# wen-yuan-zhang/MaterialRefGS

Hardware: AMD Instinct MI355X
Metric: full-render fwd+bwd views/sec at 800x800/300k surfels; grad max-rel-err vs ref (higher is better)
Workload: dtype f32; 1 GPU; C3 shell scene through render_surfel: P=300000, 800x800, S=8 + deferred BRDF shading, fwd+bwd; P=300000, H=800, W=800, S=8, sh_degree=3, num_rendered=1153468, cameras_cycled=2, parallelism=single GPU, glue_epilogue=True

## Files before the change

include/mrgs.h:

```cpp
#ifndef MRGS_H_INCLUDED
#define MRGS_H_INCLUDED

#include <stddef.h>
#include <stdint.h>

#ifdef __cplusplus
extern "C" {
#endif

#define MRGS_MAX_FEATURES 24
#define MRGS_TILE 16
#define MRGS_NUM_OTHERS 7

enum {
    MRGS_OK = 0,
    MRGS_E_BAD_ARG = 1,
    MRGS_E_TOO_MANY_FEATURES = 2,
    MRGS_E_NEED_COLORS = 3,
    MRGS_E_HIP = 4,
    MRGS_E_WORKSPACE = 5,
    MRGS_E_UNSUPPORTED = 6,
    MRGS_E_INTERNAL = 7
};

typedef struct MrgsRasterConfig {
    uint32_t struct_size;
    int32_t P;
    int32_t S;
    int32_t D;
    int32_t M;
    int32_t H, W;
    float tanfovx, tanfovy;
    float scale_modifier;
    int32_t prefiltered;
    int32_t debug;
} MrgsRasterConfig;

typedef struct MrgsRasterInputs {
    uint64_t struct_size;
    const float* bg;
    const float* means3D;
    const float* shs;
    const float* colors_precomp;
    const float* features;
    const float* opacities;
    const float* scales;
    const float* rotations;
    const float* transMat_precomp;
    const float* viewmatrix;
    const float* projmatrix;
    const float* campos;
    uint32_t* work_hint;
    const float* shs_rest;
    void* bwd_grad_ws;
    uint32_t hint_flags;
    uint32_t features_live;
} MrgsRasterInputs;
#define MRGS_HINT_REUSE_ORDER 1u
#define MRGS_HINT_VISIBLE_BYTES 2u

size_t mrgs_geom_bytes(int32_t P, int32_t H, int32_t W);
size_t mrgs_img_bytes(int32_t H, int32_t W);
size_t mrgs_binning_bytes(int64_t num_rendered);
size_t mrgs_work_hint_bytes(int32_t H, int32_t W);

int mrgs_rasterize_forward_geom(const MrgsRasterConfig* cfg, const MrgsRasterInputs* in, void* geom_ws, size_t geom_bytes,
                                int32_t* radii, int64_t* num_rendered_host, void* stream);

int mrgs_rasterize_forward_render(const MrgsRasterConfig* cfg, const MrgsRasterInputs* in, void* geom_ws, void* binning_ws,
                                  size_t binning_bytes, void* img_ws, int64_t num_rendered, float* out_color,
                                  float* out_feature, float* out_others, void* stream);

int mrgs_rasterize_forward(const MrgsRasterConfig* cfg, const MrgsRasterInputs* in, void* geom_ws, size_t geom_bytes,
                           void* binning_ws, size_t binning_bytes, int64_t capacity_pairs, void* img_ws, int32_t* radii,
                           float* out_color, float* out_feature, float* out_others, int64_t* num_rendered_host, void* stream);

typedef struct MrgsRasterTicket {
    int32_t device, slot;
    uint64_t seq;
    int64_t capacity_pairs;
} MrgsRasterTicket;
int mrgs_rasterize_forward_begin(const MrgsRasterConfig* cfg, const MrgsRasterInputs* in, void* geom_ws, size_t geom_bytes,
                                 void* binning_ws, size_t binning_bytes, int64_t capacity_pairs, void* img_ws, int32_t* radii,
                                 float* out_color, float* out_feature, float* out_others, MrgsRasterTicket* ticket, void* stream);
int mrgs_rasterize_forward_finish(const MrgsRasterTicket* ticket, int64_t* num_rendered_host);

typedef struct MrgsRasterGrads {
    uint64_t struct_size;
    float* dL_dmeans2D;
    float* dL_dcolors;
    float* dL_dfeatures;
    float* dL_dopacity;
    float* dL_dmeans3D;
    float* dL_dtransMat;
    float* dL_dsh;
    float* dL_dscales;
    float* dL_drotations;
    float* dL_dsh_rest;
    const struct MrgsSurfelParams* glue_params;
    const struct MrgsSurfelGrads* glue_grads;
} MrgsRasterGrads;

size_t mrgs_grad_bytes(int32_t P, int32_t S);
int mrgs_rasterize_backward(const MrgsRasterConfig* cfg, const MrgsRasterInputs* in, const int32_t* radii, const void* geom_ws,
                            const void* binning_ws, const void* img_ws, int64_t num_rendered, const float* dL_dout_color,
                            const float* dL_dout_feature, const float* dL_dout_others, void* grad_ws,
                            const MrgsRasterGrads* grads, void* stream);

int mrgs_rasterize_backward_blend(const MrgsRasterConfig* cfg, const MrgsRasterInputs* in, const int32_t* radii, const void* geom_ws,
                                  const void* binning_ws, const void* img_ws, int64_t num_rendered, const float* dL_dout_color,
                                  const float* dL_dout_feature, const float* dL_dout_others, void* grad_ws, float* dL_dRGB_masked,
                                  void* stream);
int mrgs_rasterize_backward_finish(const MrgsRasterConfig* cfg, const MrgsRasterInputs* in, const int32_t* radii, const void* geom_ws,
                                   const void* grad_ws, const MrgsRasterGrads* grads, void* stream);

int mrgs_mark_visible(int32_t P, const float* means3D, const float* viewmatrix, const float* projmatrix, uint8_t* present,
                      void* stream);

#define MRGS_MAX_MIPS 8
typedef struct MrgsEnvMips {
    int32_t n_levels;
    int32_t res[MRGS_MAX_MIPS];
    const float* tex[MRGS_MAX_MIPS];
    float* grad[MRGS_MAX_MIPS];
    int32_t grad_copies[MRGS_MAX_MIPS];
    float min_roughness, max_roughness;
} MrgsEnvMips;

int mrgs_envmap_lookup_forward(const MrgsEnvMips* mips, int64_t N, const float* dirs, const float* roughness, float* out, void* stream);
int mrgs_envmap_lookup_backward(const MrgsEnvMips* mips, int64_t N, const float* dirs, const float* roughness, const float* g_out,
                                float* g_dirs , float* g_roughness , void* stream);

typedef struct MrgsStridedMap { const float* ptr; int64_t stride_h, stride_w, stride_c; } MrgsStridedMap;
typedef struct MrgsShadeFrame {
    int32_t H, W;
    float Kinv[9];
    const float* R;
    const float* T;
    MrgsStridedMap albedo;
    MrgsStridedMap normal;
    MrgsStridedMap alpha;
// ... 335 lines not shown
```

materialrefgs_amd/_lib.py:

```python
import ctypes
import os
import subprocess

import torch

_CSRC = os.path.join(os.path.dirname(os.path.abspath(__file__)), "csrc")
LIB_PATH = os.environ.get("MRGS_LIB") or os.path.join(_CSRC, "libmrgs.so")

c_int32, c_int64, c_float, c_void_p, c_size_t = ctypes.c_int32, ctypes.c_int64, ctypes.c_float, ctypes.c_void_p, ctypes.c_size_t


class _Sized(ctypes.Structure):

    def __init__(self, *args, **kw):
        super().__init__(ctypes.sizeof(type(self)), *args, **kw)


class MrgsRasterConfig(_Sized):
    _fields_ = [("struct_size", ctypes.c_uint32), ("P", c_int32), ("S", c_int32), ("D", c_int32), ("M", c_int32), ("H", c_int32), ("W", c_int32),
                ("tanfovx", c_float), ("tanfovy", c_float), ("scale_modifier", c_float), ("prefiltered", c_int32),
                ("debug", c_int32)]


class MrgsRasterInputs(_Sized):
    _fields_ = [("struct_size", ctypes.c_uint64)] + [(n, c_void_p) for n in ("bg", "means3D", "shs", "colors_precomp", "features", "opacities", "scales",
                                        "rotations", "transMat_precomp", "viewmatrix", "projmatrix", "campos", "work_hint", "shs_rest",
                                        "bwd_grad_ws")] + [("hint_flags", ctypes.c_uint32), ("features_live", ctypes.c_uint32)]


MRGS_HINT_REUSE_ORDER = 1
MRGS_HINT_VISIBLE_BYTES = 2


class MrgsRasterGrads(_Sized):
    _fields_ = [("struct_size", ctypes.c_uint64)] + [(n, c_void_p) for n in ("dL_dmeans2D", "dL_dcolors", "dL_dfeatures", "dL_dopacity", "dL_dmeans3D",
                                        "dL_dtransMat", "dL_dsh", "dL_dscales", "dL_drotations", "dL_dsh_rest",
                                        "glue_params", "glue_grads")]


MRGS_MAX_MIPS = 8


class MrgsEnvMips(ctypes.Structure):
    _fields_ = [("n_levels", c_int32), ("res", c_int32 * MRGS_MAX_MIPS), ("tex", c_void_p * MRGS_MAX_MIPS),
                ("grad", c_void_p * MRGS_MAX_MIPS), ("grad_copies", c_int32 * MRGS_MAX_MIPS), ("min_roughness", c_float), ("max_roughness", c_float)]


class MrgsStridedMap(ctypes.Structure):
    _fields_ = [("ptr", c_void_p), ("stride_h", c_int64), ("stride_w", c_int64), ("stride_c", c_int64)]


class MrgsShadeFrame(ctypes.Structure):
    _fields_ = [("H", c_int32), ("W", c_int32), ("Kinv", c_float * 9), ("R", c_void_p), ("T", c_void_p),
                ("albedo", MrgsStridedMap), ("normal", MrgsStridedMap), ("alpha", MrgsStridedMap), ("refl", MrgsStridedMap),
                ("roughness", MrgsStridedMap), ("lut", c_void_p), ("lut_res", c_int32)]


class MrgsRasterTicket(ctypes.Structure):
    _fields_ = [("device", c_int32), ("slot", c_int32), ("seq", ctypes.c_uint64), ("capacity_pairs", c_int64)]


class MrgsSpmvDesc(ctypes.Structure):
    _fields_ = [("nrows", c_int32), ("lanes_per_row", c_int32), ("col_bytes", c_int32), ("val_bytes", c_int32), ("row_ptr", c_void_p),
                ("col", c_void_p), ("val", c_void_p), ("row_scale", c_void_p), ("x", c_void_p), ("y", c_void_p),
                ("image_rows", c_void_p), ("pre_scale", c_void_p), ("tile_ptr", c_void_p), ("panel_ptr", c_void_p), ("panel_src", c_void_p),
                ("res", c_int32), ("n_tiles", c_int32), ("max_panel", c_int32), ("reserved", c_int32)]


class MrgsSurfelParams(ctypes.Structure):
    _fields_ = [("P", c_int32)] + [(n, c_void_p) for n in ("xyz", "scaling_raw", "rotation_raw", "opacity_raw", "refl_raw", "rough_raw",
                                                             "ori_color_raw", "indirect_dc", "indirect_rest", "campos", "viewmatrix")]


class MrgsSurfelGrads(ctypes.Structure):
    _fields_ = [(n, c_void_p) for n in ("d_xyz", "d_scaling", "d_rotation", "d_opacity", "d_refl", "d_rough", "d_ori_color",
                                        "d_indirect_dc", "d_indirect_rest")]


class MrgsMapsFrame(ctypes.Structure):
    _fields_ = [("H", c_int32), ("W", c_int32), ("view_rot", c_float * 9), ("ray_matrix", c_float * 9), ("ray_origin", c_float * 3),
                ("depth_ratio", c_float), ("pgsr_fx", c_float), ("pgsr_fy", c_float), ("rend_distance", c_void_p), ("g_rend_distance", c_void_p)]


class MrgsLossConfig(ctypes.Structure):
    _fields_ = [("H", c_int32), ("W", c_int32), ("C", c_int32), ("lambda_dssim", c_float), ("lambda_normal", c_float),
                ("lambda_dist", c_float)]


MRGS_WARP_GEO, MRGS_WARP_MATERIAL, MRGS_WARP_METALLIC, MRGS_WARP_ROUGHNESS = 1, 2, 4, 8


class MrgsWarpConfig(_Sized):
    _fields_ = [("struct_size", ctypes.c_uint32), ("H", c_int32), ("W", c_int32), ("sample_num", c_int32), ("patch_half", c_int32),
                ("n_given", c_int32), ("flags", ctypes.c_uint32), ("seed_lo", ctypes.c_uint32), ("seed_hi", ctypes.c_uint32)] + \
               [(n, c_float) for n in ("fx_v", "fy_v", "cx_v", "cy_v", "fx_n", "fy_n", "cx_n", "cy_n", "pixel_noise_th", "geo_weight",
                                       "base_weight", "metallic_weight", "roughness_weight")]


class MrgsWarpMaps(ctypes.Structure):
    _fields_ = [(n, c_void_p) for n in ("depth_v", "depth_n", "normal_v", "distance_v", "base_v", "metal_v", "rough_v", "base_n", "metal_n",
                                        "rough_n", "fg_v", "keep_v", "cam_v", "cam_n")]


class MrgsAdamTensor(ctypes.Structure):
    _fields_ = [("param", c_void_p), ("grad", c_void_p), ("exp_avg", c_void_p), ("exp_avg_sq", c_void_p), ("numel", c_int64),
                ("lr", c_float), ("step", c_int32)]


class MrgsCompactTensor(ctypes.Structure):
    _fields_ = [("src", c_void_p), ("dst", c_void_p), ("row_floats", c_int32)]


MRGS_DENSIFY_COPY, MRGS_DENSIFY_MOMENT, MRGS_DENSIFY_XYZ, MRGS_DENSIFY_SCALING = 0, 1, 2, 3

# ... 250 lines not shown
```

materialrefgs_amd/csrc/mrgs_api.hip:

```cpp
#include <stdio.h>
#include <string.h>
#include <atomic>
#include <mutex>
#include <vector>
#include "mrgs_internal.h"

static thread_local char g_hip_err[256] = "";
static int g_profiling = 0;

int mrgs_hip_status(hipError_t e, const char* file, int line)
{
    if (e == hipSuccess) return MRGS_OK;
    snprintf(g_hip_err, sizeof(g_hip_err), "%s at %s:%d", hipGetErrorString(e), file, line);
    return MRGS_E_HIP;
}

#define STAGE_CHECK(cfg, stream)                                      \
    do {                                                              \
        if (int rc_ = MRGS_LAUNCH_STATUS()) return rc_;               \
        if ((cfg)->debug) MRGS_HIP_TRY(hipStreamSynchronize(stream)); \
    } while (0)

namespace {
enum { ST_PRE = 0, ST_SORT, ST_DUP, ST_FWD, ST_BWD, ST_PREB, ST_COUNT };
// ... 20 lines not shown
                std::lock_guard<std::mutex> lk(g_prof_mutex);
                if (!g_free.empty()) { p = g_free.back(); g_free.pop_back(); reuse = true; }
            }
            if (!reuse) { (void)hipEventCreate(&p.a); (void)hipEventCreate(&p.b); }
            p.stage = stage;
            (void)hipEventRecord(p.a, s);
        }
    }
    void stop()
    {
        if (on) {
            (void)hipEventRecord(p.b, s);
            std::lock_guard<std::mutex> lk(g_prof_mutex);
            g_pairs.push_back(p);
            on = false;
        }
    }
};

struct Carver {
    char* p;
    size_t used = 0;
    explicit Carver(void* base) : p((char*)base) {}
    template <typename T>
    T* take(size_t n)
    {
        used = mrgs_align_up(used, 256);
        T* r = p ? (T*)(p + used) : nullptr;
        used += sizeof(T) * n;
        return r;
    }
};
}

MrgsGeomWs mrgs_carve_geom(void* base, int P, int H, int W)
{
    Carver c(base);
    MrgsGeomWs g;
    const size_t n = (size_t)(P > 0 ? P : 1);
    g.rec = c.take<float4>(n * MRGS_REC_F4);
    g.cull = c.take<float4>(n * MRGS_CULL_F4);
    g.depth_key[0] = c.take<uint32_t>(n);
    g.depth_key[1] = c.take<uint32_t>(n);
    g.order[0] = c.take<uint32_t>(n);
    g.order[1] = c.take<uint32_t>(n);
    g.rect = c.take<uint2>(n);
    g.tiles_touched = c.take<uint32_t>(n);
    g.offsets = c.take<uint32_t>(n);
    g.clamped = c.take<uint8_t>(n);
    g.counters = c.take<uint32_t>(16 + MRGS_CENSUS_WORDS);
    const size_t clear_from = c.used - (16 + MRGS_CENSUS_WORDS) * sizeof(uint32_t);
    g.sort_ws = c.take<uint32_t>(mrgs_sort_ws_words((int64_t)n));
    g.scan_ws = c.take<uint32_t>(mrgs_scan_ws_words((int)n));
    g.clear_bytes = c.used - clear_from;
    const int T = ((W + MRGS_BLOCK_X - 1) / MRGS_BLOCK_X) * ((H + MRGS_BLOCK_Y - 1) / MRGS_BLOCK_Y);
    g.tile_mat = g.tile_cnt = g.tile_loc = g.chunk_tot = g.chunk_base = g.big_list = nullptr;
    if (mrgs_bin_supported(T)) {
        const size_t Tpad = (size_t)mrgs_bin_tpad(T);
        g.tile_mat = c.take<uint32_t>((size_t)mrgs_bin_groups(P) * Tpad);
        g.tile_cnt = c.take<uint32_t>(Tpad);
        g.tile_loc = c.take<uint32_t>(Tpad);
        g.chunk_tot = c.take<uint32_t>(Tpad / 64);
        g.chunk_base = c.take<uint32_t>(Tpad / 64);
        g.big_list = c.take<uint32_t>(Tpad);
    }
    g.total = mrgs_align_up(c.used, 256);
    return g;
}

MrgsImgWs mrgs_carve_img(void* base, int H, int W)
{
    Carver c(base);
    MrgsImgWs w;
    const size_t hw = (size_t)H * W;
    const size_t tiles = (size_t)((W + MRGS_BLOCK_X - 1) / MRGS_BLOCK_X) * ((H + MRGS_BLOCK_Y - 1) / MRGS_BLOCK_Y);
    const size_t nt = tiles > 0 ? tiles : 1;
    w.ranges = c.take<uint2>(nt);
    const size_t ranges_from = c.used - sizeof(uint2) * nt;
    c.used = mrgs_align_up(c.used, 256);
    w.item_est = c.take<uint32_t>(4 * nt);
    w.ranges_est_bytes = c.used - ranges_from;
    w.item_work = c.take<uint32_t>(4 * nt);
    const size_t per_list = (nt + 7) / 8 * 4;
    w.order_items = c.take<uint32_t>(8 * per_list);
    w.order_work = c.take<uint32_t>(8 * per_list);
    w.fwd_assign = c.take<uint32_t>(8 * (per_list + MRGS_MAX_SIMD_QUEUES));
    w.bwd_assign = c.take<uint32_t>(8 * (per_list + MRGS_MAX_SIMD_QUEUES));
    w.blend_state = c.take<uint32_t>(MRGS_BLEND_STATE_WORDS);
    w.q_bwd = w.blend_state + MRGS_QS_BWD;
    w.final_T = c.take<float>(3 * hw);
    w.n_contrib = c.take<uint32_t>(2 * hw);
    w.redo_list = c.take<uint32_t>(2 + hw);
    w.total = mrgs_align_up(c.used, 256);
    return w;
}

MrgsBinWs mrgs_carve_bin(void* base, int64_t R)
{
    Carver c(base);
    MrgsBinWs b;
    const size_t n = (size_t)(R > 0 ? R : 1);
    const size_t n64 = mrgs_align_up(n, 64);
    b.tile_key[0] = c.take<uint32_t>(2 * n64);
    b.tile_key[1] = b.tile_key[0] ? b.tile_key[0] + n64 : nullptr;
    b.plist[0] = c.take<uint32_t>(n);
    b.plist[1] = c.take<uint32_t>(n);
    b.sort_ws = c.take<uint32_t>(16 + mrgs_sort_ws_words((int64_t)n));
    b.sort_ws_bytes = sizeof(uint32_t) * (16 + mrgs_sort_ws_words((int64_t)n));
    b.qmask = c.take<uint8_t>(n);
    b.cflag = c.take<uint8_t>(4 * n);
    b.total = mrgs_align_up(c.used, 256);
    return b;
}

static int tile_bits(int ntiles)
{
    int bits = 1;
    while ((1 << bits) < ntiles) bits++;
    return bits;
}

static int sorted_buf(int bits) { return ((bits + 7) / 8) & 1; }
static int plist_buf(const MrgsGeomWs& g, int ntiles) { return g.tile_mat != nullptr ? 0 : sorted_buf(tile_bits(ntiles)); }

static int check_cfg(const MrgsRasterConfig* cfg, const MrgsRasterInputs* in)
{
    if (!cfg || !in) return MRGS_E_BAD_ARG;
    if (cfg->struct_size != sizeof(MrgsRasterConfig) || in->struct_size != sizeof(MrgsRasterInputs)) return MRGS_E_BAD_ARG;
    if (cfg->P < 0 || cfg->H <= 0 || cfg->W <= 0 || cfg->S < 0 || cfg->M < 0) return MRGS_E_BAD_ARG;
    if (cfg->S > MRGS_MAX_FEATURES) return MRGS_E_TOO_MANY_FEATURES;
    if (cfg->P > 0) {
        if (!in->means3D || !in->opacities || !in->viewmatrix || !in->projmatrix || !in->campos || !in->bg) return MRGS_E_BAD_ARG;
        if ((in->shs == nullptr) == (in->colors_precomp == nullptr)) return MRGS_E_NEED_COLORS;
        if (in->shs && cfg->M <= 0) return MRGS_E_BAD_ARG;
        if (in->shs_rest && (!in->shs || cfg->M < 2 || cfg->M > 16)) return MRGS_E_BAD_ARG;
        const bool have_sr = in->scales && in->rotations;
        if (have_sr == (in->transMat_precomp != nullptr)) return MRGS_E_BAD_ARG;
        if (cfg->S > 0 && !in->features) return MRGS_E_BAD_ARG;
        if ((cfg->W + 15) / 16 > 65535 || (cfg->H + 15) / 16 > 65535) return MRGS_E_UNSUPPORTED;
        if (cfg->P >= (1 << 28)) return MRGS_E_UNSUPPORTED;
        if ((uint64_t)cfg->P * MRGS_GRAD_STRIDE(cfg->S) * sizeof(float) >= (1ull << 32)) return MRGS_E_UNSUPPORTED;
    }
    return MRGS_OK;
}

MrgsHintLayout mrgs_hint_layout(int H, int W)
{
    const size_t tiles = (size_t)((W + MRGS_BLOCK_X - 1) / MRGS_BLOCK_X) * ((H + MRGS_BLOCK_Y - 1) / MRGS_BLOCK_Y);
    const size_t nt = tiles > 0 ? tiles : 1, per_list = (nt + 7) / 8 * 4;
    MrgsHintLayout l;
    l.work = 0;
    l.blend_state = mrgs_align_up(4 * nt, 64);
    l.fwd_assign = mrgs_align_up(l.blend_state + MRGS_BLEND_STATE_WORDS, 64);
    l.total_words = mrgs_align_up(l.fwd_assign + 8 * (per_list + MRGS_MAX_SIMD_QUEUES), 64);
    return l;
}
static void img_use_hint(MrgsImgWs& img, const MrgsRasterInputs* in, int H, int W)
{
    if (in->work_hint == nullptr) return;
    const MrgsHintLayout l = mrgs_hint_layout(H, W);
    img.blend_state = in->work_hint + l.blend_state;
    img.fwd_assign = in->work_hint + l.fwd_assign;
}

extern "C" {

size_t mrgs_geom_bytes(int32_t P, int32_t H, int32_t W) { return mrgs_carve_geom(nullptr, P, H, W).total; }
size_t mrgs_img_bytes(int32_t H, int32_t W) { return mrgs_carve_img(nullptr, H, W).total; }
size_t mrgs_binning_bytes(int64_t R) { return mrgs_carve_bin(nullptr, R).total; }
size_t mrgs_work_hint_bytes(int32_t H, int32_t W)
{
    if (H <= 0 || W <= 0) return 0;
    return mrgs_hint_layout(H, W).total_words * sizeof(uint32_t);
}
size_t mrgs_grad_bytes(int32_t P, int32_t S) { return mrgs_align_up((size_t)(P > 0 ? P : 1) * MRGS_GRAD_STRIDE(S) * sizeof(float), 256); }

static int enqueue_geom(const MrgsRasterConfig* cfg, const MrgsRasterInputs* in, MrgsGeomWs g, int32_t* radii, hipStream_t stream,
                        uint32_t* host_slot = nullptr, hipEvent_t slot_event = nullptr)
{
    StageTimer t0(stream, ST_PRE);
    mrgs_launch_preprocess_fwd(*cfg, *in, g, radii, stream);
    t0.stop();
    STAGE_CHECK(cfg, stream);

    StageTimer t1(stream, ST_SORT);
    if (g.tile_mat != nullptr) {
        mrgs_launch_tile_count_scan(*cfg, g, host_slot, stream);
        if (slot_event != nullptr) MRGS_HIP_TRY(hipEventRecord(slot_event, stream));
    } else {
        const int cur = mrgs_radix_sort_pairs(g.depth_key, g.order, g.sort_ws, g.counters + 1, cfg->P, nullptr, 0, 32, stream);
        STAGE_CHECK(cfg, stream);
        mrgs_scan_tiles(g.tiles_touched, g.order[cur], g.offsets, g.scan_ws, g.counters, g.counters + 1, cfg->P, stream);
    }
    t1.stop();
    STAGE_CHECK(cfg, stream);
    return MRGS_OK;
}

static int enqueue_render(const MrgsRasterConfig* cfg, const MrgsRasterInputs* in, MrgsGeomWs g, MrgsBinWs b,
                          const MrgsImgWs& img, int64_t R, const uint32_t* R_dev, float* out_color, float* out_feature,
                          float* out_others, hipStream_t stream, uint32_t* host_slot = nullptr, hipEvent_t slot_event = nullptr)
{
    const int tiles_x = (cfg->W + MRGS_BLOCK_X - 1) / MRGS_BLOCK_X, tiles_y = (cfg->H + MRGS_BLOCK_Y - 1) / MRGS_BLOCK_Y;
    const int ntiles = tiles_x * tiles_y;
    const int dcur = sorted_buf(32);

    StageTimer t0(stream, ST_DUP);
    int cur = 0;
    bool reuse_order = false;
    if (g.tile_mat != nullptr) {
        reuse_order = R > 0 && in->work_hint != nullptr && (in->hint_flags & MRGS_HINT_REUSE_ORDER) != 0u;
        if (R > 0) mrgs_launch_tile_emit_sort(*cfg, g, b, img, R, reuse_order, in->bwd_grad_ws, in->bwd_grad_ws ? mrgs_grad_bytes(cfg->P, cfg->S) : 0, stream);
        else MRGS_HIP_TRY(hipMemsetAsync(img.ranges, 0, img.ranges_est_bytes, stream));
        STAGE_CHECK(cfg, stream);
    } else {
        if (R > 0) {
            mrgs_launch_duplicate(*cfg, g, g.order[dcur], b.tile_key[0], b.plist[0], R, R_dev, b, img, host_slot, stream);
            if (slot_event != nullptr) MRGS_HIP_TRY(hipEventRecord(slot_event, stream));
        } else {
            MRGS_HIP_TRY(hipMemsetAsync(img.ranges, 0, img.ranges_est_bytes, stream));
        }
        STAGE_CHECK(cfg, stream);
        const int bits = tile_bits(ntiles);
        cur = mrgs_radix_sort_pairs(b.tile_key, b.plist, b.sort_ws + 16, b.sort_ws, R, R_dev, 0, bits, stream);
        STAGE_CHECK(cfg, stream);
        mrgs_launch_tile_ranges(b.tile_key[cur], b.plist[cur], R, R_dev, g.cull, b.qmask, img, tiles_x, ntiles, stream);
    }
    if (!reuse_order)
        mrgs_launch_blend_order(img, g.counters + 16, ntiles, 0, in->bwd_grad_ws, in->bwd_grad_ws ? mrgs_grad_bytes(cfg->P, cfg->S) : 0, in->work_hint,
                                stream);
    t0.stop();
    STAGE_CHECK(cfg, stream);

    StageTimer t1(stream, ST_FWD);
    mrgs_launch_render_fwd(*cfg, *in, g, b.plist[cur], b.qmask, b.cflag, img, out_color, out_feature, out_others, stream);
    t1.stop();
    STAGE_CHECK(cfg, stream);
    return MRGS_OK;
}

static int zero_outputs(const MrgsRasterConfig* cfg, float* out_color, float* out_feature, float* out_others, hipStream_t stream)
{
    const size_t hw = (size_t)cfg->H * cfg->W;
    MRGS_HIP_TRY(hipMemsetAsync(out_color, 0, sizeof(float) * 3 * hw, stream));
    if (cfg->S > 0) MRGS_HIP_TRY(hipMemsetAsync(out_feature, 0, sizeof(float) * cfg->S * hw, stream));
    MRGS_HIP_TRY(hipMemsetAsync(out_others, 0, sizeof(float) * MRGS_NUM_OTHERS * hw, stream));
    return MRGS_OK;
}

static int check_counters(const uint32_t host[2], int64_t* num_rendered_host)
{
    if (host[1] != 0) return MRGS_E_INTERNAL;
    if (host[0] >= (1u << 30)) return MRGS_E_UNSUPPORTED;
    *num_rendered_host = (int64_t)host[0];
    return MRGS_OK;
}

int mrgs_rasterize_forward_geom(const MrgsRasterConfig* cfg, const MrgsRasterInputs* in, void* geom_ws, size_t geom_bytes,
                                int32_t* radii, int64_t* num_rendered_host, void* stream_)
{
    hipStream_t stream = (hipStream_t)stream_;
    int rc = check_cfg(cfg, in);
    if (rc) return rc;
    if (!num_rendered_host) return MRGS_E_BAD_ARG;
    *num_rendered_host = 0;
    if (cfg->P == 0) return MRGS_OK;
    if (!geom_ws || !radii) return MRGS_E_BAD_ARG;
    MrgsGeomWs g = mrgs_carve_geom(geom_ws, cfg->P, cfg->H, cfg->W);
    if (geom_bytes < g.total) return MRGS_E_WORKSPACE;
    rc = enqueue_geom(cfg, in, g, radii, stream);
    if (rc) return rc;
    uint32_t host[2] = {0, 0};
    MRGS_HIP_TRY(hipMemcpyAsync(host, g.counters, 2 * sizeof(uint32_t), hipMemcpyDeviceToHost, stream));
    MRGS_HIP_TRY(hipStreamSynchronize(stream));
    return check_counters(host, num_rendered_host);
}

int mrgs_rasterize_forward_render(const MrgsRasterConfig* cfg, const MrgsRasterInputs* in, void* geom_ws, void* binning_ws,
                                  size_t binning_bytes, void* img_ws, int64_t R, float* out_color, float* out_feature,
                                  float* out_others, void* stream_)
{
    hipStream_t stream = (hipStream_t)stream_;
    int rc = check_cfg(cfg, in);
    if (rc) return rc;
    if (!out_color || !out_others || (cfg->S > 0 && !out_feature) || !img_ws) return MRGS_E_BAD_ARG;
    if (cfg->P == 0) return zero_outputs(cfg, out_color, out_feature, out_others, stream);
    if (!geom_ws || !binning_ws) return MRGS_E_BAD_ARG;
    MrgsImgWs img = mrgs_carve_img(img_ws, cfg->H, cfg->W);
    img_use_hint(img, in, cfg->H, cfg->W);
    MrgsGeomWs g = mrgs_carve_geom(geom_ws, cfg->P, cfg->H, cfg->W);
    MrgsBinWs b = mrgs_carve_bin(binning_ws, R);
    if (binning_bytes < b.total) return MRGS_E_WORKSPACE;
    return enqueue_render(cfg, in, g, b, img, R, nullptr, out_color, out_feature, out_others, stream);
}

namespace {
#define MRGS_MAX_DEVICES 64
#define MRGS_TICKET_RING 16
struct ReadbackRing {
    uint32_t* host = nullptr;
    uint32_t* dev = nullptr;
    hipEvent_t ev[MRGS_TICKET_RING] = {};
    uint64_t seq[MRGS_TICKET_RING] = {};
    uint64_t next = 1;
};
static thread_local ReadbackRing g_rings[MRGS_MAX_DEVICES];
}

int mrgs_rasterize_forward_begin(const MrgsRasterConfig* cfg, const MrgsRasterInputs* in, void* geom_ws, size_t geom_bytes,
                                 void* binning_ws, size_t binning_bytes, int64_t capacity_pairs, void* img_ws, int32_t* radii,
                                 float* out_color, float* out_feature, float* out_others, MrgsRasterTicket* ticket, void* stream_)
{
    hipStream_t stream = (hipStream_t)stream_;
    int rc = check_cfg(cfg, in);
    if (rc) return rc;
    if (!ticket || !out_color || !out_others || (cfg->S > 0 && !out_feature) || !img_ws) return MRGS_E_BAD_ARG;
    ticket->device = -1; ticket->slot = -1; ticket->seq = 0; ticket->capacity_pairs = capacity_pairs;
    if (cfg->P == 0) return zero_outputs(cfg, out_color, out_feature, out_others, stream);
// ... 7 lines not shown
    int device = 0;
    MRGS_HIP_TRY(hipGetDevice(&device));
    if (device < 0 || device >= MRGS_MAX_DEVICES) return MRGS_E_UNSUPPORTED;
    ReadbackRing& ring = g_rings[device];
    if (!ring.host) {
        MRGS_HIP_TRY(hipHostMalloc((void**)&ring.host, MRGS_TICKET_RING * 64, hipHostMallocMapped | hipHostMallocPortable));
        MRGS_HIP_TRY(hipHostGetDevicePointer((void**)&ring.dev, ring.host, 0));
        for (int i = 0; i < MRGS_TICKET_RING; ++i) MRGS_HIP_TRY(hipEventCreateWithFlags(&ring.ev[i], hipEventDisableTiming));
    }
    const int slot = (int)(ring.next % MRGS_TICKET_RING);
    ring.seq[slot] = ring.next;
    ticket->device = device; ticket->slot = slot; ticket->seq = ring.next++;
    uint32_t* slot_dev = ring.dev + 16 * slot;
    rc = enqueue_geom(cfg, in, g, radii, stream, slot_dev, ring.ev[slot]);
    if (rc) return rc;
    return enqueue_render(cfg, in, g, b, img, capacity_pairs, g.counters, out_color, out_feature, out_others, stream, slot_dev, ring.ev[slot]);
}

int mrgs_rasterize_forward_finish(const MrgsRasterTicket* ticket, int64_t* num_rendered_host)
{
    if (!ticket || !num_rendered_host) return MRGS_E_BAD_ARG;
    *num_rendered_host = 0;
    if (ticket->device < 0) return MRGS_OK;
    if (ticket->device >= MRGS_MAX_DEVICES || ticket->slot < 0 || ticket->slot >= MRGS_TICKET_RING) return MRGS_E_BAD_ARG;
    ReadbackRing& ring = g_rings[ticket->device];
    if (!ring.host || ring.seq[ticket->slot] != ticket->seq) return MRGS_E_BAD_ARG;
    MRGS_HIP_TRY(hipEventSynchronize(ring.ev[ticket->slot]));
    int rc = check_counters(ring.host + 16 * ticket->slot, num_rendered_host);
    if (rc) return rc;
    return *num_rendered_host > ticket->capacity_pairs ? MRGS_E_WORKSPACE : MRGS_OK;
}

int mrgs_rasterize_forward(const MrgsRasterConfig* cfg, const MrgsRasterInputs* in, void* geom_ws, size_t geom_bytes,
                           void* binning_ws, size_t binning_bytes, int64_t capacity_pairs, void* img_ws, int32_t* radii,
                           float* out_color, float* out_feature, float* out_others, int64_t* num_rendered_host, void* stream_)
{
    if (!num_rendered_host) return MRGS_E_BAD_ARG;
    *num_rendered_host = 0;
    MrgsRasterTicket ticket;
    int rc = mrgs_rasterize_forward_begin(cfg, in, geom_ws, geom_bytes, binning_ws, binning_bytes, capacity_pairs, img_ws, radii, out_color,
                                          out_feature, out_others, &ticket, stream_);
    if (rc) return rc;
    return mrgs_rasterize_forward_finish(&ticket, num_rendered_host);
}

static int grads_check(const MrgsRasterConfig* cfg, const MrgsRasterInputs* in, const MrgsRasterGrads* g)
{
    if (!g->dL_dmeans2D || (cfg->M > 0 && !g->dL_dsh) || ((in->shs_rest != nullptr) != (g->dL_dsh_rest != nullptr))) return MRGS_E_BAD_ARG;
    if ((g->glue_params != nullptr) != (g->glue_grads != nullptr)) return MRGS_E_BAD_ARG;
    if (g->glue_params == nullptr)
        return (g->dL_dcolors && g->dL_dopacity && g->dL_dmeans3D && g->dL_dtransMat && g->dL_dscales && g->dL_drotations && (cfg->S == 0 || g->dL_dfeatures))
                   ? MRGS_OK : MRGS_E_BAD_ARG;
    const MrgsSurfelParams* p = g->glue_params;
    const MrgsSurfelGrads* o = g->glue_grads;
    const bool rows8 = cfg->S == 8 && p->viewmatrix == nullptr, rows12 = cfg->S == 12 && in->features_live == 9u && p->viewmatrix != nullptr;
    if (!(rows8 || rows12) || !in->scales || !in->rotations || in->transMat_precomp) return MRGS_E_UNSUPPORTED;
    if (cfg->P != p->P || !p->scaling_raw || !p->rotation_raw || !p->opacity_raw || !p->refl_raw || !p->rough_raw || !p->ori_color_raw) return MRGS_E_BAD_ARG;
    return (o->d_xyz && o->d_scaling && o->d_rotation && o->d_opacity && o->d_refl && o->d_rough && o->d_ori_color && o->d_indirect_dc && o->d_indirect_rest)
               ? MRGS_OK : MRGS_E_BAD_ARG;
}

int mrgs_rasterize_backward_blend(const MrgsRasterConfig* cfg, const MrgsRasterInputs* in, const int32_t* radii, const void* geom_ws,
                                  const void* binning_ws, const void* img_ws, int64_t R, const float* dL_dout_color,
                                  const float* dL_dout_feature, const float* dL_dout_others, void* grad_ws, float* dL_dRGB_masked,
                                  void* stream_)
{
    hipStream_t stream = (hipStream_t)stream_;
    int rc = check_cfg(cfg, in);
    if (rc) return rc;
    if (cfg->P == 0) return MRGS_OK;
    if (!radii || !geom_ws || !binning_ws || !img_ws || !grad_ws || !dL_dout_color || !dL_dout_others) return MRGS_E_BAD_ARG;
    if (cfg->S > 0 && !dL_dout_feature) return MRGS_E_BAD_ARG;
    const int tiles_x = (cfg->W + MRGS_BLOCK_X - 1) / MRGS_BLOCK_X, tiles_y = (cfg->H + MRGS_BLOCK_Y - 1) / MRGS_BLOCK_Y;
    MrgsGeomWs g = mrgs_carve_geom(const_cast<void*>(geom_ws), cfg->P, cfg->H, cfg->W);
    MrgsBinWs b = mrgs_carve_bin(const_cast<void*>(binning_ws), R);
    MrgsImgWs img = mrgs_carve_img(const_cast<void*>(img_ws), cfg->H, cfg->W);
    img_use_hint(img, in, cfg->H, cfg->W);
    const int cur = plist_buf(g, tiles_x * tiles_y);
    float* grad_rec = (float*)grad_ws;

    StageTimer t0(stream, ST_BWD);
    const bool prepared = in->bwd_grad_ws != nullptr && in->bwd_grad_ws == grad_ws;
    if (R > 0) {
        if (!prepared) mrgs_launch_blend_order(img, g.counters + 16, tiles_x * tiles_y, 1, grad_rec, mrgs_grad_bytes(cfg->P, cfg->S), nullptr, stream);
        mrgs_launch_render_bwd(*cfg, *in, g, b.plist[cur], b.cflag, img, dL_dout_color, dL_dout_feature, dL_dout_others, grad_rec, prepared, stream);
    } else if (!prepared) {
        MRGS_HIP_TRY(hipMemsetAsync(grad_rec, 0, mrgs_grad_bytes(cfg->P, cfg->S), stream));
    }
    t0.stop();
    if (dL_dRGB_masked) mrgs_launch_color_grad_extract(*cfg, g, radii, grad_rec, in->shs != nullptr, dL_dRGB_masked, stream);
    STAGE_CHECK(cfg, stream);
    return MRGS_OK;
}

int mrgs_rasterize_backward_finish(const MrgsRasterConfig* cfg, const MrgsRasterInputs* in, const int32_t* radii, const void* geom_ws,
                                   const void* grad_ws, const MrgsRasterGrads* grads, void* stream_)
{
    hipStream_t stream = (hipStream_t)stream_;
    int rc = check_cfg(cfg, in);
    if (rc) return rc;
    if (!grads || grads->struct_size != sizeof(MrgsRasterGrads)) return MRGS_E_BAD_ARG;
    if (cfg->P == 0) return MRGS_OK;
    rc = grads_check(cfg, in, grads);
    if (rc) return rc;
    if (!radii || !geom_ws || !grad_ws) return MRGS_E_BAD_ARG;
    MrgsGeomWs g = mrgs_carve_geom(const_cast<void*>(geom_ws), cfg->P, cfg->H, cfg->W);
    StageTimer t1(stream, ST_PREB);
    mrgs_launch_preprocess_bwd(*cfg, *in, g, radii, (const float*)grad_ws, *grads, stream);
    t1.stop();
    STAGE_CHECK(cfg, stream);
    return MRGS_OK;
}

int mrgs_rasterize_backward(const MrgsRasterConfig* cfg, const MrgsRasterInputs* in, const int32_t* radii, const void* geom_ws,
                            const void* binning_ws, const void* img_ws, int64_t R, const float* dL_dout_color,
                            const float* dL_dout_feature, const float* dL_dout_others, void* grad_ws, const MrgsRasterGrads* grads,
                            void* stream_)
{
    int rc = check_cfg(cfg, in);
    if (rc) return rc;
    if (!grads || grads->struct_size != sizeof(MrgsRasterGrads)) return MRGS_E_BAD_ARG;
    if (cfg->P == 0) return MRGS_OK;
    rc = grads_check(cfg, in, grads);
    if (rc) return rc;
    if (!radii || !geom_ws || !binning_ws || !img_ws || !grad_ws || !dL_dout_color || !dL_dout_others) return MRGS_E_BAD_ARG;
    if (cfg->S > 0 && !dL_dout_feature) return MRGS_E_BAD_ARG;
    rc = mrgs_rasterize_backward_blend(cfg, in, radii, geom_ws, binning_ws, img_ws, R, dL_dout_color, dL_dout_feature, dL_dout_others, grad_ws,
                                       nullptr, stream_);
    if (rc) return rc;
    return mrgs_rasterize_backward_finish(cfg, in, radii, geom_ws, grad_ws, grads, stream_);
}

int mrgs_mark_visible(int32_t P, const float* means3D, const float* viewmatrix, const float* projmatrix, uint8_t* present,
                      void* stream_)
{
    (void)projmatrix;
    if (P < 0) return MRGS_E_BAD_ARG;
    if (P == 0) return MRGS_OK;
    if (!means3D || !viewmatrix || !present) return MRGS_E_BAD_ARG;
    mrgs_launch_mark_visible(P, means3D, viewmatrix, present, (hipStream_t)stream_);
    return MRGS_LAUNCH_STATUS();
}

#define MRGS_MESH_ENTRY(call) do { bool launched = false; if (int rc = (call)) return rc; return launched ? MRGS_LAUNCH_STATUS() : MRGS_OK; } while (0)
int mrgs_tsdf_fuse(const MrgsTsdfConfig* cfg, const MrgsTsdfView* views_dev, float* field, float* weight_debug, void* stream_)
{
    MRGS_MESH_ENTRY(mrgs_tsdf_fuse_launch(cfg, views_dev, field, weight_debug, stream_, &launched));
}
int mrgs_mesh_count(const MrgsMeshConfig* cfg, const float* field, void* ws, size_t ws_bytes, int64_t* totals_dev, void* stream_)
{
    MRGS_MESH_ENTRY(mrgs_mesh_count_launch(cfg, field, ws, ws_bytes, totals_dev, stream_, &launched));
}
int mrgs_mesh_emit(const MrgsMeshConfig* cfg, const float* field, void* ws, size_t ws_bytes, const int64_t* totals_host, float* vertices,
                   int32_t* triangles, void* stream_)
{
    MRGS_MESH_ENTRY(mrgs_mesh_emit_launch(cfg, field, ws, ws_bytes, totals_host, vertices, triangles, stream_, &launched));
}
int mrgs_mesh_clusters(int64_t V, int64_t T, const int32_t* triangles, int32_t* labels, int32_t* counts, void* stream_)
{
    MRGS_MESH_ENTRY(mrgs_mesh_clusters_launch(V, T, triangles, labels, counts, stream_, &launched));
}
int mrgs_mesh_select(int64_t V, int64_t T, const int32_t* triangles, const int32_t* labels, const int32_t* counts, int32_t threshold,
                     uint8_t* keep_vertex, uint8_t* keep_triangle, void* stream_)
{
    MRGS_MESH_ENTRY(mrgs_mesh_select_launch(V, T, triangles, labels, counts, threshold, keep_vertex, keep_triangle, stream_, &launched));
}
int mrgs_mesh_reindex(int64_t V_old, int64_t V_new, const int32_t* new_to_old, int32_t* remap_ws, int64_t T, int32_t* triangles, void* stream_)
{
// ... 116 lines not shown
```

materialrefgs_amd/csrc/mrgs_blend_math.h:

```cpp
#pragma once
#include "mrgs_internal.h"
#include "mrgs_wave.h"

#define MRGS_ALPHA_MIN (1.0f / 255.0f)
#define MRGS_T_MIN 0.0001f
#define MRGS_CHUNK 64

template <auto KERNEL> static int mrgs_waves_per_simd()
{
    static const int n = [] {
        int per_cu = 0;
        if (hipOccupancyMaxActiveBlocksPerMultiprocessor(&per_cu, KERNEL, 64, 0) != hipSuccess || per_cu < 4) return 1;
        return per_cu / 4;
    }();
    return n;
}


__device__ __forceinline__ uint32_t mrgs_pull_item(uint32_t* __restrict__ qstate, const uint32_t* __restrict__ cu_state,
                                                   const uint32_t* __restrict__ assign_ws, int ntiles, int xcd, int wv, int lane,
                                                   int slots, unsigned long long* dbg = nullptr)
{
    const uint32_t pw = qstate[MRGS_QS_PASSES + xcd];
    const int passes = (int)(pw & 0xFFFFu), NQ = (int)(pw >> 16);
    if (wv >= passes * NQ) return 0xFFFFFFFFu;
    const int per_list = ((ntiles + 7) >> 3) * 4;
    const uint32_t hw_id = __builtin_amdgcn_s_getreg((4 << 0) | (0 << 6) | (31 << 11));
    const uint32_t xcc = __builtin_amdgcn_s_getreg((20 << 0) | (0 << 6) | (3 << 11)) & 7u;
    const uint32_t dense = cu_state[MRGS_CS_DENSE + xcc * 256 + mrgs_cu_key(hw_id)];
    const int q0 = (int)((dense * 4u + ((hw_id >> 4) & 3u)) % (uint32_t)NQ);
    const uint32_t* assign = assign_ws + (size_t)xcd * (per_list + MRGS_MAX_SIMD_QUEUES);
    uint32_t* tickets = qstate + MRGS_QS_TICKET + xcd * MRGS_MAX_SIMD_QUEUES;
    uint32_t item = 0xFFFFFFFFu;
    int t = 0;
    if (lane == 0) {
        t = (int)atomicAdd(&tickets[q0], 1u);
        if (t < passes) item = assign[t * NQ + q0];
    }
    item = __builtin_amdgcn_readfirstlane(item);
    t = __builtin_amdgcn_readfirstlane(t);
    if (dbg) { dbg[0] = dbg[2] = wall_clock64(); dbg[1] = 0; }
    if (item != 0xFFFFFFFFu) return item;
    if (t < passes && passes <= slots) __builtin_amdgcn_s_sleep(127);
    for (int base = 1; item == 0xFFFFFFFFu && base < NQ;) {
        const int d = base + lane;
        const int q = d < NQ ? (q0 + d < NQ ? q0 + d : q0 + d - NQ) : q0;
        const uint32_t tk = __hip_atomic_load(&tickets[q], __ATOMIC_RELAXED, __HIP_MEMORY_SCOPE_AGENT);
        const uint32_t last = assign[(passes - 1) * NQ + q];
        const bool has = d < NQ && (int)tk < passes - (last == 0xFFFFFFFFu ? 1 : 0);
        const unsigned long long m = __ballot(has);
        if (dbg) dbg[1] += 1 + (m == 0ull ? 256 : 0);
        if (m == 0ull) { base += 64; continue; }
        const int qs = __builtin_amdgcn_readlane(q, (int)__builtin_ctzll(m));
        if (lane == 0) {
            const int ts = (int)atomicAdd(&tickets[qs], 1u);
            if (ts < passes) item = assign[ts * NQ + qs];
        }
        item = __builtin_amdgcn_readfirstlane(item);
    }
    if (dbg) dbg[2] = wall_clock64();
    return item;
}

__device__ __forceinline__ float mrgs_rcp(float x) { return __builtin_amdgcn_rcpf(x); }

__device__ __forceinline__ float mrgs_exp(float x)
{
    const float L2E_HI = 1.44269502162933349609375f, L2E_LO = 1.925963033500011e-8f, LN2 = 0.693147182464599609375f;
    const float t = x * L2E_HI;
    float e = fmaf(x, L2E_HI, -t);
    e = fmaf(x, L2E_LO, e);
    const float r = __builtin_amdgcn_exp2f(t);
    return fmaf(r, e * LN2, r);
}

struct SurfelGeom { float4 g0, g1, g2; };

struct Hit {
    float kx, ky, kz, lx, ly, lz;
    float inv_pz, sx, sy;
    float rho3d, rho2d, dx, dy;
    float depth, G, alpha;
    bool use3d;
};

#define MRGS_ALPHA_LO (MRGS_ALPHA_MIN * (1.0f - 4e-6f))
#define MRGS_ALPHA_HI (MRGS_ALPHA_MIN * (1.0f + 4e-6f))
#define MRGS_NEAR_LO (MRGS_NEAR_N - 1e-4f)
#define MRGS_NEAR_HI (MRGS_NEAR_N + 1e-4f)
#define MRGS_RHO_EPS 2e-5f
#define MRGS_T_STEP_ERR 4.1e-7f
#define MRGS_T1_SLACK 1.25f
#define MRGS_T1_ABS 1e-11f
#ifndef MRGS_T2_EPS
#define MRGS_T2_EPS (0.5f * 4e-6f)
#endif

struct HitTest { float ppz, d3, power; };
__device__ __forceinline__ HitTest mrgs_intersect_fast(const SurfelGeom& s, float px, float py, Hit& h)
{
    const float Twx = s.g1.z, Twy = s.g1.w, Twz = s.g2.x;
    h.kx = fmaf(px, Twx, -s.g0.x); h.ky = fmaf(px, Twy, -s.g0.y); h.kz = fmaf(px, Twz, -s.g0.z);
    h.lx = fmaf(py, Twx, -s.g0.w); h.ly = fmaf(py, Twy, -s.g1.x); h.lz = fmaf(py, Twz, -s.g1.y);
    const float ppx = fmaf(h.ky, h.lz, -(h.kz * h.ly));
    const float ppy = fmaf(h.kz, h.lx, -(h.kx * h.lz));
    const float ppz = fmaf(h.kx, h.ly, -(h.ky * h.lx));
    h.inv_pz = mrgs_rcp(ppz);
    h.sx = ppx * h.inv_pz;
    h.sy = ppy * h.inv_pz;
    h.rho3d = fmaf(h.sx, h.sx, h.sy * h.sy);
    h.dx = s.g2.y - px;
    h.dy = s.g2.z - py;
    h.rho2d = MRGS_FILTER_INV_SQUARE * fmaf(h.dx, h.dx, h.dy * h.dy);
    const float rho = fminf(h.rho3d, h.rho2d);
    const float d3 = fmaf(h.sx, Twx, fmaf(h.sy, Twy, Twz));
    h.use3d = h.rho3d <= h.rho2d;
    h.depth = h.use3d ? d3 : Twz;
    const float power = -0.5f * rho;
    h.G = mrgs_exp(power);
    h.alpha = fminf(0.99f, s.g2.w * h.G);
    return HitTest{ppz, d3, power};
}

__device__ __forceinline__ bool mrgs_intersect(const SurfelGeom& s, float px, float py, Hit& h)
{
    const HitTest t = mrgs_intersect_fast(s, px, py, h);
    return (t.ppz != 0.0f) & (!(t.d3 < MRGS_NEAR_LO) | !(s.g2.x < MRGS_NEAR_LO)) & !(t.power > 0.0f) & !(h.alpha < MRGS_ALPHA_LO);
}

__device__ __forceinline__ bool mrgs_hit_decide(const Hit& h, bool may_hit, bool& ambiguous)
{
    const bool hit = may_hit & !(h.depth < MRGS_NEAR_LO);
    ambiguous = (hit & ((h.alpha < MRGS_ALPHA_HI) | (h.depth < MRGS_NEAR_HI))) | (may_hit & (fabsf(h.rho3d - h.rho2d) < MRGS_RHO_EPS));
    return hit;
}

#define MRGS_BALLOT(cond) __builtin_amdgcn_ballot_w64(cond)
#define MRGS_LANES(mask) __builtin_amdgcn_inverse_ballot_w64(mask)
__device__ __forceinline__ uint64_t mrgs_intersect_mask(const SurfelGeom& s, float px, float py, Hit& h)
{
    const HitTest t = mrgs_intersect_fast(s, px, py, h);
    const uint64_t tw_ok = s.g2.x < MRGS_NEAR_LO ? 0ull : ~0ull;
    return MRGS_BALLOT(t.ppz != 0.0f) & (~MRGS_BALLOT(t.d3 < MRGS_NEAR_LO) | tw_ok) & ~MRGS_BALLOT(t.power > 0.0f) & ~MRGS_BALLOT(h.alpha < MRGS_ALPHA_LO);
}
__device__ __forceinline__ uint64_t mrgs_hit_decide_mask(const Hit& h, uint64_t may_hit, uint64_t& ambiguous)
{
    const uint64_t hit = may_hit & ~MRGS_BALLOT(h.depth < MRGS_NEAR_LO);
    ambiguous = (hit & (MRGS_BALLOT(h.alpha < MRGS_ALPHA_HI) | MRGS_BALLOT(h.depth < MRGS_NEAR_HI))) |
                (may_hit & MRGS_BALLOT(fabsf(h.rho3d - h.rho2d) < MRGS_RHO_EPS));
    return hit;
}

__device__ const double mrgs_exp_cr_tab[16] = {1.4426950408889634074, 0.69314718055994530942, 1.0 / 6227020800.0, 1.0 / 479001600.0,
                                               1.0 / 39916800.0, 1.0 / 3628800.0, 1.0 / 362880.0, 1.0 / 40320.0, 1.0 / 5040.0, 1.0 / 720.0,
                                               1.0 / 120.0, 1.0 / 24.0, 1.0 / 6.0, 0.5, 1.0, 1.0};
__device__ __forceinline__ float mrgs_exp_cr_finish(double p, double n)
{
    const int e = n < -1000.0 ? -1000 : (int)n;
    return (float)__builtin_ldexp(p, e);
}
template <bool TABLE>
__device__ __forceinline__ float mrgs_exp_cr(float x)
{
    if (TABLE) {
        const volatile double* c = mrgs_exp_cr_tab;
        const double t = (double)x * c[0];
        const double n = __builtin_rint(t);
        const double z = (t - n) * c[1];
        double p = c[2];
#pragma unroll
        for (int i = 3; i < 16; i++) p = __builtin_fma(p, z, c[i]);
        return mrgs_exp_cr_finish(p, n);
    }
    const double t = (double)x * 1.4426950408889634074;
    const double n = __builtin_rint(t);
    const double z = (t - n) * 0.69314718055994530942;
    double p = 1.0 / 6227020800.0;
    p = __builtin_fma(p, z, 1.0 / 479001600.0);
    p = __builtin_fma(p, z, 1.0 / 39916800.0);
    p = __builtin_fma(p, z, 1.0 / 3628800.0);
    p = __builtin_fma(p, z, 1.0 / 362880.0);
    p = __builtin_fma(p, z, 1.0 / 40320.0);
    p = __builtin_fma(p, z, 1.0 / 5040.0);
    p = __builtin_fma(p, z, 1.0 / 720.0);
    p = __builtin_fma(p, z, 1.0 / 120.0);
    p = __builtin_fma(p, z, 1.0 / 24.0);
    p = __builtin_fma(p, z, 1.0 / 6.0);
    p = __builtin_fma(p, z, 0.5);
    p = __builtin_fma(p, z, 1.0);
    p = __builtin_fma(p, z, 1.0);
    return mrgs_exp_cr_finish(p, n);
}

template <bool COLD = false>
__device__ __forceinline__ bool mrgs_intersect_exact(const SurfelGeom& s, float px, float py, Hit& h)
{
    const float Twx = s.g1.z, Twy = s.g1.w, Twz = s.g2.x;
    h.kx = fmaf(px, Twx, -s.g0.x); h.ky = fmaf(px, Twy, -s.g0.y); h.kz = fmaf(px, Twz, -s.g0.z);
    h.lx = fmaf(py, Twx, -s.g0.w); h.ly = fmaf(py, Twy, -s.g1.x); h.lz = fmaf(py, Twz, -s.g1.y);
    const float ppx = fmaf(h.ky, h.lz, -(h.kz * h.ly));
    const float ppy = fmaf(h.kz, h.lx, -(h.kx * h.lz));
    const float ppz = fmaf(h.kx, h.ly, -(h.ky * h.lx));
    h.inv_pz = 1.0f / ppz;
    h.sx = ppx * h.inv_pz;
    h.sy = ppy * h.inv_pz;
    h.rho3d = fmaf(h.sx, h.sx, h.sy * h.sy);
    h.dx = s.g2.y - px;
    h.dy = s.g2.z - py;
    h.rho2d = MRGS_FILTER_INV_SQUARE * fmaf(h.dx, h.dx, h.dy * h.dy);
    const float rho = fminf(h.rho3d, h.rho2d);
    h.use3d = h.rho3d <= h.rho2d;
    h.depth = h.use3d ? fmaf(h.sx, Twx, fmaf(h.sy, Twy, Twz)) : Twz;
    const float power = -0.5f * rho;
    h.G = mrgs_exp_cr<COLD>(power);
    h.alpha = fminf(0.99f, s.g2.w * h.G);
    return (ppz != 0.0f) & !(h.depth < MRGS_NEAR_N) & !(power > 0.0f) & !(h.alpha < MRGS_ALPHA_MIN);
}

__device__ __forceinline__ void mrgs_block_pixel(int block_x, int block_y, int lane, int& pxi, int& pyi)
{
    pxi = block_x * 8 + (lane & 7);
    pyi = block_y * 8 + (lane >> 3);
}

struct CullConic { float4 a, b, c; };
__device__ __forceinline__ float mrgs_edge_min(float D, float Q, float slope, float X, float lo, float hi, float errX)
{
// ... 85 lines not shown
```

materialrefgs_amd/csrc/mrgs_internal.h:

```cpp
#pragma once
#include <hip/hip_runtime.h>
#include <stdint.h>
#include "../../include/mrgs.h"

#define MRGS_BLOCK_X 16
#define MRGS_BLOCK_Y 16
#define MRGS_NEAR_N 0.2f
#define MRGS_FAR_N 100.0f
#define MRGS_FILTER_INV_SQUARE 2.0f

#define MRGS_REC_F4 5
#define MRGS_CULL_F4 3

#define MRGS_SMAX(S) ((S) == 0 ? 0 : (S) <= 8 ? 8 : (S) <= 12 ? 12 : 24)
#define MRGS_G_DT 0
#define MRGS_G_OPA 9
#define MRGS_G_NRM 10
#define MRGS_G_COL 13
#define MRGS_G_FEAT 16
#define MRGS_G_M2(SMAX) (16 + (SMAX))
#define MRGS_GRAD_STRIDE(S) ((18 + MRGS_SMAX(S) + 3) & ~3)

int mrgs_hip_status(hipError_t e, const char* file, int line);
#define MRGS_HIP_TRY(expr) do { if (int rc_ = mrgs_hip_status((expr), __FILE__, __LINE__)) return rc_; } while (0)
#define MRGS_LAUNCH_STATUS() mrgs_hip_status(hipGetLastError(), __FILE__, __LINE__)

static inline size_t mrgs_align_up(size_t v, size_t a) { return (v + a - 1) / a * a; }

struct MrgsGeomWs {
    float4* rec;
    float4* cull;
    uint32_t* depth_key[2];
    uint32_t* order[2];
    uint2* rect;
    uint32_t* tiles_touched;
    uint32_t* offsets;
    uint8_t* clamped;
    uint32_t* counters;
    uint32_t* sort_ws;
    uint32_t* scan_ws;
    size_t clear_bytes;
    uint32_t* tile_mat;
    uint32_t* tile_cnt;
    uint32_t* tile_loc;
    uint32_t* chunk_tot;
    uint32_t* chunk_base;
    uint32_t* big_list;
    size_t total;
};

struct MrgsImgWs {
    uint2* ranges;
    uint32_t* item_est;
    size_t ranges_est_bytes;
    uint32_t* item_work;
    uint32_t* order_items, *order_work;
    uint32_t* fwd_assign, *bwd_assign;
    uint32_t* blend_state;
    uint32_t* q_bwd;
    float* final_T;
    uint32_t* n_contrib;
    uint32_t* redo_list;
    size_t total;
};

struct MrgsBinWs {
    uint32_t* tile_key[2];
    uint32_t* plist[2];
    uint32_t* sort_ws;
    size_t sort_ws_bytes;
    uint8_t* qmask;
    uint8_t* cflag;
    size_t total;
};

struct MrgsHintLayout { size_t work, blend_state, fwd_assign, total_words; };
MrgsHintLayout mrgs_hint_layout(int H, int W);
MrgsGeomWs mrgs_carve_geom(void* base, int P, int H, int W);
MrgsImgWs mrgs_carve_img(void* base, int H, int W);
MrgsBinWs mrgs_carve_bin(void* base, int64_t R);


#define MRGS_SORT_WS_HEADER 16
#define MRGS_MAX_SIMD_QUEUES 128
#define MRGS_QS_COUNT 0
#define MRGS_QS_PASSES 8
#define MRGS_QS_TICKET 16
#define MRGS_QS_WORDS (16 + 8 * MRGS_MAX_SIMD_QUEUES)
#define MRGS_QS_FWD 0
#define MRGS_QS_BWD MRGS_QS_WORDS
#define MRGS_CS_BASE (2 * MRGS_QS_WORDS)
#define MRGS_CS_NCU 0
#define MRGS_CS_DENSE 8
#define MRGS_BLEND_STATE_WORDS (2 * MRGS_QS_WORDS + 8 + 2048)
#define MRGS_CENSUS_WORDS 2048
__device__ __forceinline__ uint32_t mrgs_cu_key(uint32_t hw_id) { return ((hw_id >> 8) & 0xFFu); }
__device__ __forceinline__ void mrgs_census_mark(uint32_t* __restrict__ census)
{
    const uint32_t key = mrgs_cu_key(__builtin_amdgcn_s_getreg((4 << 0) | (0 << 6) | (31 << 11)));
    const uint32_t xcc = __builtin_amdgcn_s_getreg((20 << 0) | (0 << 6) | (3 << 11)) & 7u;
    census[xcc * 256 + key] = 1u;
}
size_t mrgs_sort_ws_words(int64_t n);
int mrgs_radix_sort_pairs(uint32_t* key[2], uint32_t* val[2], uint32_t* ws, uint32_t* error_flag, int64_t n, const uint32_t* n_dev,
                          int bit_lo, int bit_hi, hipStream_t stream);
size_t mrgs_scan_ws_words(int n);
void mrgs_scan_tiles(const uint32_t* tiles_touched, const uint32_t* order, uint32_t* offsets, uint32_t* ws, uint32_t* total_out,
                     uint32_t* error_flag, int n, hipStream_t stream);

int mrgs_bin_groups(int P);
int mrgs_bin_tpad(int T);
bool mrgs_bin_supported(int T);
void mrgs_launch_tile_count_scan(const MrgsRasterConfig& cfg, const MrgsGeomWs& g, uint32_t* host_slot, hipStream_t stream);
void mrgs_launch_tile_emit_sort(const MrgsRasterConfig& cfg, const MrgsGeomWs& g, const MrgsBinWs& b, const MrgsImgWs& img, int64_t capacity,
                                bool reuse_order, void* bulk_zero, size_t bulk_zero_bytes, hipStream_t stream);

void mrgs_launch_preprocess_fwd(const MrgsRasterConfig& cfg, const MrgsRasterInputs& in, const MrgsGeomWs& g, int32_t* radii,
                                hipStream_t stream);
void mrgs_launch_preprocess_bwd(const MrgsRasterConfig& cfg, const MrgsRasterInputs& in, const MrgsGeomWs& g,
                                const int32_t* radii, const float* grad_rec, const MrgsRasterGrads& out, hipStream_t stream);
void mrgs_launch_color_grad_extract(const MrgsRasterConfig& cfg, const MrgsGeomWs& g, const int32_t* radii, const float* grad_rec, bool from_sh,
                                    float* out, hipStream_t stream);
void mrgs_launch_mark_visible(int P, const float* means3D, const float* viewmatrix, uint8_t* present, hipStream_t stream);

void mrgs_launch_duplicate(const MrgsRasterConfig& cfg, const MrgsGeomWs& g, const uint32_t* order, uint32_t* tile_key,
                           uint32_t* plist, int64_t capacity, const uint32_t* R_dev, const MrgsBinWs& b, const MrgsImgWs& img, uint32_t* host_slot,
                           hipStream_t stream);
void mrgs_launch_tile_ranges(const uint32_t* tile_key, const uint32_t* plist, int64_t R, const uint32_t* R_dev, const float4* rec,
                             uint8_t* qmask, const MrgsImgWs& img, int tiles_x, int ntiles, hipStream_t stream);
void mrgs_launch_blend_order(const MrgsImgWs& img, const uint32_t* census, int ntiles, int backward, void* bulk_zero, size_t bulk_zero_bytes,
                             const uint32_t* fwd_hint,
                             hipStream_t stream);

void mrgs_launch_render_fwd(const MrgsRasterConfig& cfg, const MrgsRasterInputs& in, const MrgsGeomWs& g, const uint32_t* plist,
                            const uint8_t* qmask, uint8_t* cflag, const MrgsImgWs& img, float* out_color, float* out_feature, float* out_others, hipStream_t stream);
void mrgs_launch_render_bwd(const MrgsRasterConfig& cfg, const MrgsRasterInputs& in, const MrgsGeomWs& g, const uint32_t* plist,
                            const uint8_t* cflag, const MrgsImgWs& img, const float* dL_dpix, const float* dL_dpix_f, const float* dL_dothers,
                            float* grad_rec, bool forward_queues, hipStream_t stream);

int mrgs_tsdf_fuse_launch(const MrgsTsdfConfig* cfg, const MrgsTsdfView* views, float* field, float* weight_debug, void* stream, bool* launched);
int mrgs_mesh_count_launch(const MrgsMeshConfig* cfg, const float* field, void* ws, size_t ws_bytes, int64_t* totals_dev, void* stream, bool* launched);
int mrgs_mesh_emit_launch(const MrgsMeshConfig* cfg, const float* field, void* ws, size_t ws_bytes, const int64_t* totals_host, float* vertices,
                          int32_t* triangles, void* stream, bool* launched);
int mrgs_mesh_clusters_launch(int64_t V, int64_t T, const int32_t* triangles, int32_t* labels, int32_t* counts, void* stream, bool* launched);
int mrgs_mesh_select_launch(int64_t V, int64_t T, const int32_t* triangles, const int32_t* labels, const int32_t* counts, int32_t threshold,
                            uint8_t* keep_vertex, uint8_t* keep_triangle, void* stream, bool* launched);
int mrgs_mesh_reindex_launch(int64_t V_old, int64_t V_new, const int32_t* new_to_old, int32_t* remap_ws, int64_t T, int32_t* triangles,
                             void* stream, bool* launched);

#ifndef MRGS_EXP
#define MRGS_EXP(x) expf(x)
#endif
```

materialrefgs_amd/csrc/mrgs_render_bwd.hip:

```cpp
#include "mrgs_blend_math.h"
#include "mrgs_wave.h"

#ifndef MRGS_BWD_STAGES
#define MRGS_BWD_STAGES 1
#endif


__device__ __forceinline__ void swap32_add(float& a, float b)
{
    typedef unsigned u2 __attribute__((ext_vector_type(2)));
    const u2 r = __builtin_amdgcn_permlane32_swap(__float_as_uint(a), __float_as_uint(b), false, false);
    a = __uint_as_float(r.x) + __uint_as_float(r.y);
}
__device__ __forceinline__ void swap16_add(float& a, float b)
{
    typedef unsigned u2 __attribute__((ext_vector_type(2)));
    const u2 r = __builtin_amdgcn_permlane16_swap(__float_as_uint(a), __float_as_uint(b), false, false);
    a = __uint_as_float(r.x) + __uint_as_float(r.y);
}

__device__ __forceinline__ float rows_reduce4(float a0, float a1, float a2, float a3)
{
    float t0, t1, u;
    asm volatile(
// ... 55 lines not shown
}

__device__ __forceinline__ void atomic_add_at(float* __restrict__ base, uint32_t byte_off, float v)
{
    atomicAdd((float*)((char*)base + byte_off), v);
}

template <int K>
__device__ __forceinline__ void wave_reduce_atomic_add(float (&v)[K], float* __restrict__ base, uint32_t row_off, const ReduceLane& rl)
{
    static_assert(K % 4 == 0, "pad the value count to a multiple of 4");
#pragma unroll
    for (int i = 0; i < K / 2; i++) swap32_add(v[2 * i], v[2 * i + 1]);
#pragma unroll
    for (int i = 0; i < K / 4; i++) swap16_add(v[4 * i], v[4 * i + 2]);
    constexpr int N4 = K / 4;
    constexpr int NB4 = N4 / 4;
    constexpr int REM = N4 - 4 * NB4;
#pragma unroll
    for (int t = 0; t < NB4; t++) {
        const float u = rows_reduce4(v[16 * t], v[16 * t + 4], v[16 * t + 8], v[16 * t + 12]);
        if (rl.w16) atomic_add_at(base, row_off + (64u * t + rl.off16), u);
    }
    if (REM >= 2) {
        const float u = rows_reduce2(v[16 * NB4], v[16 * NB4 + 4]);
        if (rl.w8) atomic_add_at(base, row_off + (64u * NB4 + rl.off8), u);
    }
    if (REM == 1 || REM == 3) {
        constexpr int vbase = 16 * NB4 + (REM == 3 ? 8 : 0);
        const float u = rows_reduce1(v[vbase]);
        if (rl.w4) atomic_add_at(base, row_off + (4u * vbase + rl.off4), u);
    }
}

__device__ __forceinline__ void wave_reduce_atomic_add2(float a, float b, float* __restrict__ base, uint32_t byte_off, int lane)
{
    swap32_add(a, b);
    a = rows_reduce1(a);
    a += __int_as_float(__builtin_amdgcn_update_dpp(0, __float_as_int(a), 0x142, 0xa, 0xf, false));
    if ((lane & 31) == 16) atomic_add_at(base, byte_off + 4u * (uint32_t)(lane >> 5), a);
}

__device__ __forceinline__ void wave_reduce_atomic_add1(float a, float* __restrict__ base, uint32_t byte_off, int lane)
{
    float z = 0.0f;
    swap32_add(a, z);
    a = rows_reduce1(a);
    a += __int_as_float(__builtin_amdgcn_update_dpp(0, __float_as_int(a), 0x142, 0xa, 0xf, false));
    if (lane == 16) atomic_add_at(base, byte_off, a);
}

#ifdef MRGS_WAVE_STATS
__device__ unsigned long long g_wave_stats[8 * 65536];
extern "C" int mrgs_wave_stats(unsigned long long* host, int n)
{
    return (int)hipMemcpyFromSymbol(host, HIP_SYMBOL(g_wave_stats), sizeof(unsigned long long) * n);
}
#define WS_ENTRY() const unsigned long long ws_te = wall_clock64(); unsigned long long ws_dbg[3];
#define WS_DBG , ws_dbg
#define WS_BEGIN() const unsigned long long ws_t0 = wall_clock64(), ws_c0 = __builtin_amdgcn_s_memtime(); unsigned ws_iters = 0, ws_act = 0, ws_chunks = 0;
#define WS_ITER(a) { ws_iters++; ws_act += (a) ? 1 : 0; }
#define WS_CHUNK() ws_chunks++;
#define WS_END() if (lane == 0 && b < 65536) { unsigned long long* w = g_wave_stats + 8 * (size_t)b; w[6] = ((ws_dbg[0] - ws_te) << 40) | ((ws_dbg[2] - ws_te) << 16) | ws_dbg[1]; w[7] = ws_te; w[0] = ws_t0; w[1] = wall_clock64(); \
        w[2] = __builtin_amdgcn_s_memtime() - ws_c0; w[3] = ((unsigned long long)ws_iters << 32) | ws_act; w[4] = ((unsigned long long)ws_chunks << 32) | (unsigned)max_contrib; \
        w[5] = (unsigned long long)__builtin_amdgcn_s_getreg((4 << 0) | (0 << 6) | (31 << 11)) | ((unsigned long long)__builtin_amdgcn_s_getreg((20 << 0) | (0 << 6) | (31 << 11)) << 32); }
#else
#define WS_ENTRY()
#define WS_DBG
#define WS_BEGIN()
#define WS_ITER(a)
#define WS_CHUNK()
#define WS_END()
#endif

#ifndef MRGS_BWD_WPE0
#define MRGS_BWD_WPE0 5
#endif
#ifndef MRGS_BWD_WPE8
#define MRGS_BWD_WPE8 4
#endif
template <int S_MAX, bool FV, int S_LIVE>
__global__ void __launch_bounds__(64) __attribute__((amdgpu_waves_per_eu(S_MAX == 0 ? MRGS_BWD_WPE0 : S_MAX <= 8 ? MRGS_BWD_WPE8 : 2, 8))) render_bwd_kernel(
    const uint2* __restrict__ ranges, const uint32_t* __restrict__ bwd_assign, uint32_t* __restrict__ q_bwd, const uint32_t* __restrict__ cu_state, const uint32_t* __restrict__ point_list,
    const uint8_t* __restrict__ cflag, int S, int W, int H, int tiles_x, int ntiles,
    const float4* __restrict__ rec, const float* __restrict__ features, const float* __restrict__ bg,
    const float* __restrict__ final_Ts, const uint32_t* __restrict__ n_contrib, const float* __restrict__ dL_dpixels,
    const float* __restrict__ dL_dpixels_f, const float* __restrict__ dL_dothers, float* __restrict__ grad_rec, int gstride, int slots)
{
    constexpr int SF = S_MAX > 0 ? S_MAX : 1;
    constexpr bool XREC = S_LIVE > S_MAX;
    static_assert(!XREC || (S_MAX == 8 && S_LIVE == 9 && FV), "one record channel: rows of twelve floats, eight staged");
    constexpr int S_ROW = XREC ? 12 : S_MAX;
    constexpr int S_STAGED = S_LIVE < S_MAX ? S_LIVE : S_MAX;
    constexpr int SFA = S_LIVE > SF ? S_LIVE : SF;
    constexpr int K = 16 + S_LIVE;
    constexpr int KT = K & ~3;
    __shared__ StageBuf<SF> stage[MRGS_BWD_STAGES];

    const int lane = threadIdx.x;
    const int b = blockIdx.x;
    WS_ENTRY();
    const uint32_t item = mrgs_pull_item(q_bwd, cu_state, bwd_assign, ntiles, b & 7, b >> 3, lane, slots WS_DBG);
    if (item == 0xFFFFFFFFu) return;
    const int tile = (int)((item & 0x1FFFFFFFu) >> 2), quad = (int)(item & 3u);
    const uint32_t prio = (item >> 29) & 3u;
    const uint2 range = ranges[tile];
    const int tx = tile % tiles_x, ty = tile / tiles_x;
    const int bx = tx * 2 + (quad & 1), by = ty * 2 + (quad >> 1);
    const int pxi = bx * 8 + (lane & 7), pyi = by * 8 + (lane >> 3);
    const bool inside = pxi < W && pyi < H;
    const float px = (float)pxi, py = (float)pyi;
    const int HW = H * W;
    const int pix = inside ? W * pyi + pxi : 0;

    const int last_contributor = inside ? (int)n_contrib[pix] : 0;
    int max_contrib = last_contributor;
#pragma unroll
    for (int d = 32; d >= 1; d >>= 1) max_contrib = max(max_contrib, __shfl_xor(max_contrib, d, 64));
    if (max_contrib == 0) return;
    WS_BEGIN();
    if (prio == 3u) __builtin_amdgcn_s_setprio(3);
    else if (prio == 2u) __builtin_amdgcn_s_setprio(2);
    else if (prio == 1u) __builtin_amdgcn_s_setprio(1);
    const int median_contributor = inside ? (int)n_contrib[pix + HW] : 0;

    const float T_final = inside ? final_Ts[pix] : 0.f;
    float T = T_final;
    float dL_dpixel[3] = {0.f, 0.f, 0.f};
    float dL_dpixel_f[SFA];
#pragma unroll
    for (int i = 0; i < SFA; i++) dL_dpixel_f[i] = 0.f;
    float accum_dot = 0.f;
    float dL_dreg = 0.f, dL_ddepth = 0.f, dL_daccum = 0.f, dL_dnormal2D[3] = {0.f, 0.f, 0.f}, dL_dmedian_depth = 0.f;
    if (inside && last_contributor > 0) {
        dL_ddepth = dL_dothers[0 * HW + pix];
        dL_daccum = dL_dothers[1 * HW + pix];
        dL_dnormal2D[0] = dL_dothers[2 * HW + pix];
        dL_dnormal2D[1] = dL_dothers[3 * HW + pix];
        dL_dnormal2D[2] = dL_dothers[4 * HW + pix];
        dL_dmedian_depth = dL_dothers[5 * HW + pix];
        dL_dreg = dL_dothers[6 * HW + pix];
#pragma unroll
        for (int i = 0; i < 3; i++) dL_dpixel[i] = dL_dpixels[i * HW + pix];
        if (S_MAX > 0) {
#pragma unroll
            for (int i = 0; i < S_LIVE; i++)
                if (i < S) dL_dpixel_f[i] = dL_dpixels_f[(size_t)i * HW + pix];
        }
    }
    const float final_D = inside ? final_Ts[pix + HW] : 0.f;
    const float final_D2 = inside ? final_Ts[pix + 2 * HW] : 0.f;
    const float mscale = MRGS_FAR_N / (MRGS_FAR_N - MRGS_NEAR_N);
    const float dmd_scale = (MRGS_FAR_N * MRGS_NEAR_N) / (MRGS_FAR_N - MRGS_NEAR_N);
    const float bg_dot_dpixel = fmaf(bg[2], dL_dpixel[2], fmaf(bg[1], dL_dpixel[1], bg[0] * dL_dpixel[0]));

    const uint32_t* plist = point_list + range.x;
    const uint8_t* qm = cflag + (size_t)range.x * 4 + quad;
    const ReduceLane rl = mrgs_reduce_lane(lane);
    const uint32_t row_bytes = (uint32_t)gstride * 4u;
    const int c_top = (max_contrib - 1) / MRGS_CHUNK;
    uint32_t idq1 = 0, idq2 = 0;
    uint64_t mask_cur, exact_cur;
    {
        uint32_t id0 = 0, q0 = 0;
        if (c_top * MRGS_CHUNK + lane < max_contrib) { id0 = plist[c_top * MRGS_CHUNK + lane]; q0 = qm[(size_t)(c_top * MRGS_CHUNK + lane) * 4]; }
        if (c_top >= 1) idq1 = plist[(c_top - 1) * MRGS_CHUNK + lane] | ((uint32_t)qm[(size_t)((c_top - 1) * MRGS_CHUNK + lane) * 4] << 28);
        if (c_top >= 2) idq2 = plist[(c_top - 2) * MRGS_CHUNK + lane] | ((uint32_t)qm[(size_t)((c_top - 2) * MRGS_CHUNK + lane) * 4] << 28);
        const bool cand0 = q0 & 1u;
        mask_cur = __builtin_amdgcn_ballot_w64(cand0);
        exact_cur = __builtin_amdgcn_ballot_w64((q0 & 2u) != 0u);
        mrgs_stage_async<S_MAX, SF, FV, S_LIVE, S_ROW>(stage[c_top % MRGS_BWD_STAGES], rec, features, S, id0, cand0);
        if (cand0) stage[c_top % MRGS_BWD_STAGES].id[lane] = id0 * row_bytes;
    }

    for (int c = c_top; c >= 0; c--) {
        const int base = c * MRGS_CHUNK;
        mrgs_stage_wait();
        WS_CHUNK();
        uint64_t mask_nxt = 0ull, exact_nxt = 0ull;
        auto stage_next = [&]() {
            const bool cand1 = (idq1 >> 28) & 1u;
            exact_nxt = __builtin_amdgcn_ballot_w64(((idq1 >> 29) & 1u) != 0u);
            const uint32_t id1 = idq1 & 0x0FFFFFFFu;
            mask_nxt = __builtin_amdgcn_ballot_w64(cand1);
            mrgs_stage_async<S_MAX, SF, FV, S_LIVE, S_ROW>(stage[(c + 1) % MRGS_BWD_STAGES], rec, features, S, id1, cand1);
            if (cand1) stage[(c + 1) % MRGS_BWD_STAGES].id[lane] = id1 * row_bytes;
            idq1 = idq2;
            idq2 = 0;
            if (c >= 3) idq2 = plist[(c - 3) * MRGS_CHUNK + lane] | ((uint32_t)qm[(size_t)((c - 3) * MRGS_CHUNK + lane) * 4] << 28);
        };
        if (MRGS_BWD_STAGES == 2) stage_next();

        uint64_t mask = mask_cur;
        const uint64_t exact_mask = exact_cur;
        const StageBuf<SF>& sb = stage[c % MRGS_BWD_STAGES];

        auto blend_entry = [&](const SurfelGeom& sg, int j) {
            const int contributor = base + j;
            Hit h;
            bool active;
            active = mrgs_intersect(sg, px, py, h) & !(h.depth < MRGS_NEAR_LO);
            if (__builtin_expect((exact_mask >> j) & 1ull, 0)) active = mrgs_intersect_exact<true>(sg, px, py, h);
            active = active & inside & (contributor < last_contributor);
            const uint64_t amask = __builtin_amdgcn_ballot_w64(active);
            WS_ITER(amask != 0ull);
            if (amask == 0ull) return;
            const bool use3d = h.use3d;
            const bool a3 = active & use3d;
            const float4 a0 = sb.rec[3][j], a1 = sb.rec[4][j];
            const float normal[3] = {a0.x, a0.y, a0.z};
            const float col[3] = {a0.w, a1.x, a1.y};
            const float alpha = active ? h.alpha : 0.0f;
            const float G = active ? h.G : 0.0f;
            const float c_d = active ? h.depth : 1.0f;
            const float sx = a3 ? h.sx : 0.0f, sy = a3 ? h.sy : 0.0f;
            const float inv_pz = a3 ? h.inv_pz : 0.0f;

            float g[K];
            const float inv_1ma = mrgs_rcp(1.0f - alpha);
            T = T * inv_1ma;
            const float w = alpha * T;
            const float one_m_a = 1.0f - alpha;
            float q = 0.0f;
#pragma unroll
            for (int ch = 0; ch < 3; ch++) {
                q = fmaf(col[ch], dL_dpixel[ch], q);
                g[MRGS_G_COL + ch] = w * dL_dpixel[ch];
            }
            if (S_MAX > 0) {
#pragma unroll
                for (int ch = 0; ch < S_STAGED; ch++) {
                    const float f = (FV || ch < S) ? mrgs_staged_feature<FV>(sb, ch, j) : 0.0f;
                    q = fmaf(f, dL_dpixel_f[ch], q);
                    g[MRGS_G_FEAT + ch] = w * dL_dpixel_f[ch];
                }
                if (XREC) {
                    q = fmaf(a1.w, dL_dpixel_f[S_MAX], q);
                    g[MRGS_G_FEAT + S_MAX] = w * dL_dpixel_f[S_MAX];
                }
            }
#pragma unroll
            for (int ch = 0; ch < 3; ch++) {
                q = fmaf(normal[ch], dL_dnormal2D[ch], q);
                g[MRGS_G_NRM + ch] = w * dL_dnormal2D[ch];
            }
            const float inv_cd = mrgs_rcp(c_d);
            const float m_d = mscale * (1.0f - MRGS_NEAR_N * inv_cd);
            const float dmd_dd = dmd_scale * inv_cd * inv_cd;
            float dL_dz = (active & (contributor == median_contributor - 1)) ? dL_dmedian_depth : 0.0f;
            const float final_A = 1.0f - T_final;
            const float dL_dweight = fmaf(-2.0f * m_d, final_D, fmaf(m_d * m_d, final_A, final_D2)) * dL_dreg;
            const float dL_dmd = 2.0f * w * fmaf(m_d, final_A, -final_D) * dL_dreg;
            dL_dz = fmaf(dL_dmd, dmd_dd, dL_dz);
            q = fmaf(c_d, dL_ddepth, q);
            q += dL_daccum;
            q += dL_dweight;
            float dL_dalpha = q - accum_dot;
            accum_dot = fmaf(alpha, q, one_m_a * accum_dot);
            dL_dalpha *= T;
            dL_dalpha = fmaf(-T_final * inv_1ma, bg_dot_dpixel, dL_dalpha);
            dL_dalpha = active ? dL_dalpha : 0.0f;
            const float dL_dG = sg.g2.w * dL_dalpha;
            dL_dz = fmaf(w, dL_ddepth, dL_dz);
            {
                const float Twx = sg.g1.z, Twy = sg.g1.w;
                const float dGn = dL_dG * -G;
                const float dL_dsx = fmaf(dGn, sx, dL_dz * Twx);
                const float dL_dsy = fmaf(dGn, sy, dL_dz * Twy);
                const float dpx = dL_dsx * inv_pz, dpy = dL_dsy * inv_pz;
                const float dpz = -fmaf(dpx, sx, dpy * sy);
                const float ndkx = fmaf(-h.ly, dpz, h.lz * dpy);
                const float ndky = fmaf(-h.lz, dpx, h.lx * dpz);
                const float ndkz = fmaf(-h.lx, dpy, h.ly * dpx);
                const float ndlx = fmaf(-dpy, h.kz, dpz * h.ky);
                const float ndly = fmaf(-dpz, h.kx, dpx * h.kz);
                const float ndlz = fmaf(-dpx, h.ky, dpy * h.kx);
                g[0] = ndkx; g[1] = ndky; g[2] = ndkz;
                g[3] = ndlx; g[4] = ndly; g[5] = ndlz;
                g[6] = fmaf(px, -ndkx, fmaf(py, -ndlx, dL_dz * sx));
                g[7] = fmaf(px, -ndky, fmaf(py, -ndly, dL_dz * sy));
                g[8] = fmaf(px, -ndkz, fmaf(py, -ndlz, dL_dz));
            }
            g[MRGS_G_OPA] = G * dL_dalpha;
            const uint32_t row_off = sb.id[j];
            if constexpr (KT == K) {
                wave_reduce_atomic_add<K>(g, grad_rec, row_off, rl);
            } else {
                float gt[KT];
#pragma unroll
                for (int k = 0; k < KT; k++) gt[k] = g[k];
                wave_reduce_atomic_add<KT>(gt, grad_rec, row_off, rl);
#pragma unroll
                for (int k = KT; k < K; k++) wave_reduce_atomic_add1(g[k], grad_rec, row_off + 4u * (uint32_t)k, lane);
            }
            const bool a2 = active & !use3d;
            if (__builtin_amdgcn_ballot_w64(a2) != 0ull) {
                const float dL_dG2 = a2 ? dL_dG : 0.0f;
                const float dGf = -G * MRGS_FILTER_INV_SQUARE;
                wave_reduce_atomic_add2(dL_dG2 * (dGf * h.dx), dL_dG2 * (dGf * h.dy), grad_rec, row_off + 4u * MRGS_G_M2(S_ROW), lane);
            }
        };

        if (mask != 0ull) {
            int j = 63 - __builtin_clzll(mask);
            SurfelGeom sA, sB;
            sA.g0 = sb.rec[0][j]; sA.g1 = sb.rec[1][j]; sA.g2 = sb.rec[2][j];
            while (true) {
                mask &= ~(1ull << j);
                bool more = mask != 0ull;
                int jn = more ? 63 - __builtin_clzll(mask) : j;
                sB.g0 = sb.rec[0][jn]; sB.g1 = sb.rec[1][jn]; sB.g2 = sb.rec[2][jn];
                blend_entry(sA, j);
                if (!more) break;
                j = jn;
                mask &= ~(1ull << j);
                more = mask != 0ull;
                jn = more ? 63 - __builtin_clzll(mask) : j;
                sA.g0 = sb.rec[0][jn]; sA.g1 = sb.rec[1][jn]; sA.g2 = sb.rec[2][jn];
                blend_entry(sB, j);
                if (!more) break;
                j = jn;
            }
        }
        if (MRGS_BWD_STAGES == 1) stage_next();
        mask_cur = mask_nxt;
        exact_cur = exact_nxt;
    }
    mrgs_stage_wait();
    WS_END();
}

#define MRGS_BWD_KERNEL render_bwd_kernel

void mrgs_launch_render_bwd(const MrgsRasterConfig& cfg, const MrgsRasterInputs& in, const MrgsGeomWs& g, const uint32_t* plist,
                            const uint8_t* cflag, const MrgsImgWs& img, const float* dL_dpix, const float* dL_dpix_f, const float* dL_dothers,
                            float* grad_rec, bool forward_queues, hipStream_t stream)
{
    const uint32_t* assign = forward_queues ? img.fwd_assign : img.bwd_assign;
    const int tiles_x = (cfg.W + MRGS_BLOCK_X - 1) / MRGS_BLOCK_X, tiles_y = (cfg.H + MRGS_BLOCK_Y - 1) / MRGS_BLOCK_Y;
    const int ntiles = tiles_x * tiles_y;
    const int nblocks = (((ntiles + 7) / 8) * 4 + MRGS_MAX_SIMD_QUEUES) * 8;
    const dim3 grid(nblocks), block(64);
#define LAUNCH(GS, SM, ...)                                                                                                       \
    hipLaunchKernelGGL((MRGS_BWD_KERNEL<SM, __VA_ARGS__>), grid, block, 0, stream, img.ranges, assign, img.q_bwd, img.blend_state + MRGS_CS_BASE, plist, cflag, cfg.S, cfg.W, cfg.H, tiles_x, ntiles, \
                       g.rec, in.features, in.bg, img.final_T, img.n_contrib, dL_dpix, dL_dpix_f, dL_dothers, grad_rec, GS, mrgs_waves_per_simd<MRGS_BWD_KERNEL<SM, __VA_ARGS__>>())
    const int gs = MRGS_GRAD_STRIDE(cfg.S);
    const bool fv_ok = ((uintptr_t)in.features & 15u) == 0;
    if (cfg.S == 0) LAUNCH(gs, 0, false, 0);
    else if (cfg.S == 8 && fv_ok) LAUNCH(gs, 8, true, 8);
    else if (cfg.S <= 8) LAUNCH(gs, 8, false, 8);
    else if (cfg.S == 12 && fv_ok && in.features_live == 9u) LAUNCH(gs, 8, true, 9);
    else if (cfg.S == 12 && fv_ok) LAUNCH(gs, 12, true, 12);
    else if (cfg.S <= 12) LAUNCH(gs, 12, false, 12);
    else if (cfg.S == 24 && fv_ok) LAUNCH(gs, 24, true, 24);
    else LAUNCH(gs, 24, false, 24);
#undef LAUNCH
}
```

materialrefgs_amd/csrc/mrgs_render_fwd.hip:

```cpp
#include <type_traits>

#include "mrgs_blend_math.h"
#include "mrgs_wave.h"

#ifndef MRGS_FWD_REFINE_LIVE
#define MRGS_FWD_REFINE_LIVE 24
#endif
#ifndef MRGS_FWD_STAGES
#define MRGS_FWD_STAGES 1
#endif

#ifdef MRGS_WAVE_STATS
__device__ unsigned long long g_wave_stats_fwd[8 * 65536];
extern "C" int mrgs_wave_stats_fwd(unsigned long long* host, int n)
{
    return (int)hipMemcpyFromSymbol(host, HIP_SYMBOL(g_wave_stats_fwd), sizeof(unsigned long long) * n);
}
__device__ int g_ws_min_total = 0;
extern "C" int mrgs_wave_stats_min_total(int n) { return (int)hipMemcpyToSymbol(HIP_SYMBOL(g_ws_min_total), &n, sizeof(int)); }
#endif

__device__ __forceinline__ float wave_inclusive_sum(float v)
{
    v = dpp_add<0x111, 0xf>(v);
// ... 100 lines not shown
        const float depth = bl ? h.depth : 1.0f;
        const float m_ = mscale * (1.0f - MRGS_NEAR_N * (1.0f / depth));
        const float mw = m_ * w, mmw = m_ * m_ * w;
        const float i1 = wave_inclusive_sum(mw), i2 = wave_inclusive_sum(mmw);
        const float pM1 = xM1 + (i1 - mw), pM2 = xM2 + (i2 - mmw);
        xM1 += __uint_as_float(__builtin_amdgcn_readlane(__float_as_uint(i1), 63));
        xM2 += __uint_as_float(__builtin_amdgcn_readlane(__float_as_uint(i2), 63));
        sDist = fmaf(fmaf(-2.0f * m_, pM1, fmaf(m_ * m_, 1.0f - Tb, pM2)), w, sDist);
        sD = fmaf(depth, w, sD);
        const float4 a0 = r3, a1 = r4;
        sN0 = fmaf(a0.x, w, sN0); sN1 = fmaf(a0.y, w, sN1); sN2 = fmaf(a0.z, w, sN2);
        sC0 = fmaf(a0.w, w, sC0); sC1 = fmaf(a1.x, w, sC1); sC2 = fmaf(a1.y, w, sC2);
        if (S_MAX > 0 && __builtin_amdgcn_ballot_w64(bl) != 0ull) {
            const float* fsrc = features + (size_t)gid * S;
#pragma unroll
            for (int ch = 0; ch < S_MAX; ch++)
                if (ch < S) sF[ch] = fmaf(fsrc[ch], w, sF[ch]);
        }
        if (bm != 0ull) xlast = (uint32_t)__builtin_amdgcn_readlane(e, 63 - __builtin_clzll(bm)) + 1u;
        const uint64_t medm = __builtin_amdgcn_ballot_w64(bl & (Tb > 0.5f));
        if (medm != 0ull) {
            const int jm = 63 - __builtin_clzll(medm);
            xmedc = (uint32_t)__builtin_amdgcn_readlane(e, jm) + 1u;
            xmed = __uint_as_float(__builtin_amdgcn_readlane(__float_as_uint(h.depth), jm));
        }
        if (valid) {
            Hit hf;
            bool amb;
            const bool mh = mrgs_intersect(sg, qx, qy, hf);
            (void)mrgs_hit_decide(hf, mh, amb);
            const bool in_reach = tm == 0ull || lane <= __builtin_ctzll(tm);
            const uint32_t fl = (bl ? 1u : 0u) | ((amb && in_reach) ? 3u : 0u);
            if (fl) atomicOr(reinterpret_cast<uint32_t*>(cflag) + range.x + e, fl << (8 * quad));
        }
        ended = tm != 0ull;
        qh += n;
        nq -= n;
    }
    auto wave_sum = [&](float v) {
#pragma unroll
        for (int d = 32; d >= 1; d >>= 1) v += __shfl_xor(v, d, 64);
        return v;
    };
    sC0 = wave_sum(sC0); sC1 = wave_sum(sC1); sC2 = wave_sum(sC2);
    sN0 = wave_sum(sN0); sN1 = wave_sum(sN1); sN2 = wave_sum(sN2);
    sD = wave_sum(sD); sDist = wave_sum(sDist);
    if (S_MAX > 0) {
#pragma unroll
        for (int ch = 0; ch < S_MAX; ch++) sF[ch] = wave_sum(sF[ch]);
    }
    if (lane == 0) {
        final_T[pix] = xT;
        final_T[pix + HW] = xM1;
        final_T[pix + 2 * HW] = xM2;
        n_contrib[pix] = xlast;
        n_contrib[pix + HW] = xmedc;
        out_color[pix] = fmaf(xT, bg[0], sC0);
        out_color[pix + HW] = fmaf(xT, bg[1], sC1);
        out_color[pix + 2 * HW] = fmaf(xT, bg[2], sC2);
        if (S_MAX > 0) {
#pragma unroll
            for (int ch = 0; ch < S_MAX; ch++)
                if (ch < S) out_feature[(size_t)ch * HW + pix] = sF[ch];
        }
        out_others[pix + 0 * HW] = sD;
        out_others[pix + 1 * HW] = 1.0f - xT;
        out_others[pix + 2 * HW] = sN0;
        out_others[pix + 3 * HW] = sN1;
        out_others[pix + 4 * HW] = sN2;
        out_others[pix + 5 * HW] = xmed;
        out_others[pix + 6 * HW] = sDist;
    }
}

template <int S_MAX, bool FV, int S_LIVE>
#ifndef MRGS_FWD_WAVES_S0
#define MRGS_FWD_WAVES_S0 5
#endif
#ifndef MRGS_FWD_WAVES_S8
#define MRGS_FWD_WAVES_S8 4
#endif
__global__ void __launch_bounds__(64) __attribute__((amdgpu_waves_per_eu(S_MAX == 0 ? MRGS_FWD_WAVES_S0 : S_MAX <= 12 ? MRGS_FWD_WAVES_S8 : 4, 8))) render_fwd_kernel(
    const uint2* __restrict__ ranges, const uint32_t* __restrict__ fwd_assign, uint32_t* __restrict__ blend_state, const uint32_t* __restrict__ point_list,
    const uint8_t* __restrict__ qmask, uint8_t* __restrict__ cflag, int S, int W, int H, int tiles_x, int ntiles,
    const float4* __restrict__ rec, const float4* __restrict__ cull, const float* __restrict__ features, const float* __restrict__ bg, float* __restrict__ final_T,
    uint32_t* __restrict__ n_contrib, float* __restrict__ out_color, float* __restrict__ out_feature, float* __restrict__ out_others,
    uint32_t* __restrict__ item_work, const uint32_t* __restrict__ item_est ,
    uint32_t* __restrict__ work_hint, int slots, uint32_t* __restrict__ redo_list)
{
    constexpr int SF = S_MAX > 0 ? S_MAX : 1;
    constexpr bool XREC = S_LIVE > S_MAX;
    static_assert(!XREC || (S_MAX == 8 && S_LIVE == 9 && FV), "one record channel: rows of twelve floats, eight staged");
    constexpr int S_ROW = XREC ? 12 : S_MAX;
    constexpr int S_STAGED = S_LIVE < S_MAX ? S_LIVE : S_MAX;
    using RecTail = typename std::conditional<XREC, float4, float2>::type;
    __shared__ StageBuf<SF> stage[MRGS_FWD_STAGES];

    const int lane = threadIdx.x;
    const int b = blockIdx.x;
    const uint32_t item = mrgs_pull_item(blend_state + MRGS_QS_FWD, blend_state + MRGS_CS_BASE, fwd_assign, ntiles, b & 7, b >> 3, lane, slots);
    if (item == 0xFFFFFFFFu) return;
    const int tile = (int)((item & 0x1FFFFFFFu) >> 2), quad = (int)(item & 3u);
    const uint32_t prio = (item >> 29) & 3u;
    const uint2 range = ranges[tile];
    const int tx = tile % tiles_x, ty = tile / tiles_x;
    const int bx = tx * 2 + (quad & 1), by = ty * 2 + (quad >> 1);
    const int pxi = bx * 8 + (lane & 7), pyi = by * 8 + (lane >> 3);
    const bool inside = pxi < W && pyi < H;
    const float px = (float)pxi, py = (float)pyi;
    const int HW = H * W;
    const int pix = W * pyi + pxi;

#ifdef MRGS_WAVE_STATS
    const int total = (int)(range.y - range.x) >= g_ws_min_total ? (int)(range.y - range.x) : 0;
#else
    const int total = (int)(range.y - range.x);
#endif
#ifdef MRGS_WAVE_STATS
    const unsigned long long ws_t0 = wall_clock64(), ws_c0 = __builtin_amdgcn_s_memtime();
    unsigned ws_blend = 0, ws_le4 = 0, ws_le8 = 0, ws_le16 = 0, ws_blend_le8 = 0;
#endif
    if (prio == 3u) __builtin_amdgcn_s_setprio(3);
    else if (prio == 2u) __builtin_amdgcn_s_setprio(2);
    else if (prio == 1u) __builtin_amdgcn_s_setprio(1);

    uint64_t done = ~__builtin_amdgcn_ballot_w64(inside);
    uint64_t redo = 0ull;
    int cf_end = 0;
    uint32_t work = 0;
    float T = 1.0f;
    float Terr = 0.0f;
    float C0 = 0.f, C1 = 0.f, C2 = 0.f, N0 = 0.f, N1 = 0.f, N2 = 0.f;
    float F[SF];
#pragma unroll
    for (int i = 0; i < SF; i++) F[i] = 0.f;
    float Fx = 0.f;
    float Dp = 0.f, M1 = 0.f, M2 = 0.f, distortion = 0.f, median_depth = 0.f;
    uint32_t last_contributor = 0, median_contributor = 0;
    const float mscale = MRGS_FAR_N / (MRGS_FAR_N - MRGS_NEAR_N);

    const uint32_t* plist = point_list + range.x;
    const uint8_t* qm = qmask + range.x;
    uint8_t* cf = cflag + (size_t)range.x * 4 + quad;
    uint32_t id1 = 0, id2 = 0, q1 = 0, q2 = 0;
    uint32_t idc = 0, idn = 0;

    uint64_t mask_cur;
    {
        uint32_t id0 = 0, q0 = 0;
        if (lane < total) { id0 = plist[lane]; q0 = qm[lane]; }
        idc = id0;
        if (MRGS_CHUNK + lane < total) { id1 = plist[MRGS_CHUNK + lane]; q1 = qm[MRGS_CHUNK + lane]; }
        if (2 * MRGS_CHUNK + lane < total) { id2 = plist[2 * MRGS_CHUNK + lane]; q2 = qm[2 * MRGS_CHUNK + lane]; }
        const bool cand0 = (q0 >> quad) & 1u;
        mask_cur = __builtin_amdgcn_ballot_w64(cand0);
        mrgs_stage_async<S_MAX, SF, FV, S_LIVE, S_ROW>(stage[0], rec, features, S, id0, cand0);
    }

    for (int base = 0, c = 0; base < total; base += MRGS_CHUNK, c++) {
        if (~done == 0ull) break;
        mrgs_stage_wait();
        uint64_t mask_nxt = 0ull;
        auto stage_next = [&]() {
            const bool cand1 = (q1 >> quad) & 1u;
            mask_nxt = __builtin_amdgcn_ballot_w64(cand1);
            mrgs_stage_async<S_MAX, SF, FV, S_LIVE, S_ROW>(stage[(c + 1) % MRGS_FWD_STAGES], rec, features, S, id1, cand1);
            idn = id1;
            id1 = id2; q1 = q2;
            id2 = 0; q2 = 0;
            if (base + 3 * MRGS_CHUNK + lane < total) { id2 = plist[base + 3 * MRGS_CHUNK + lane]; q2 = qm[base + 3 * MRGS_CHUNK + lane]; }
        };
        if (MRGS_FWD_STAGES == 2) stage_next();

        uint64_t m = mask_cur;
        {
            const uint64_t live = ~done;
            if (m != 0ull && __builtin_popcountll(live) <= MRGS_FWD_REFINE_LIVE) {
                const int r0 = __builtin_ctzll(live) >> 3, r1 = (63 - __builtin_clzll(live)) >> 3;
                uint32_t cols = (uint32_t)(live | (live >> 32));
                cols |= cols >> 16; cols |= cols >> 8; cols &= 0xFFu;
                const int c0 = __builtin_ctz(cols), c1 = 31 - __builtin_clz(cols);
                const CullConic cc = mrgs_cull_load(cull, idc);
                const bool touch = mrgs_block_may_touch(cc, (float)(bx * 8 + c0), (float)(by * 8 + r0), (float)(c1 - c0), (float)(r1 - r0));
                m &= __builtin_amdgcn_ballot_w64(touch);
            }
        }
        work += (uint32_t)__builtin_popcountll(m);
        const StageBuf<SF>& sb = stage[c % MRGS_FWD_STAGES];
        uint64_t contributed = 0ull;
        uint64_t unsure = 0ull;

        const bool median_live = (MRGS_BALLOT(T > 0.5f - MRGS_T2_EPS) & ~done) != 0ull;
        auto blend_entry = [&](const SurfelGeom& sg, const float4& a0, const RecTail& a1, int j) {
            Hit h;
            const uint64_t may_hit = mrgs_intersect_mask(sg, px, py, h) & ~done;
#ifdef MRGS_WAVE_STATS
            const int ws_live = __builtin_popcountll(~done);
            ws_le4 += ws_live <= 4; ws_le8 += ws_live <= 8; ws_le16 += ws_live <= 16;
#endif
            if (may_hit == 0ull) return;
#ifdef MRGS_WAVE_STATS
            ws_blend++; ws_blend_le8 += ws_live <= 8;
#endif
            work += 3u;
            contributed |= 1ull << j;
            uint64_t ambiguous;
            const uint64_t ok = mrgs_hit_decide_mask(h, may_hit, ambiguous);
            if (ambiguous != 0ull) unsure |= 1ull << j;
            const float oma = 1.0f - h.alpha;
            const float test_T = T * oma;
            const float Terr_new = fmaf(Terr, oma, (MRGS_T1_SLACK * MRGS_T_STEP_ERR) * T);
            const uint64_t below = MRGS_BALLOT(test_T < (MRGS_T_MIN - MRGS_T1_ABS) - Terr_new);
            redo |= ambiguous;
            done |= ok & below;
            const uint64_t upd_mask = ok & ~below;
            const bool upd = MRGS_LANES(upd_mask);
            const float alpha = upd ? h.alpha : 0.0f;
            const float depth = upd ? h.depth : 1.0f;
            const float w = alpha * T;
            const float A = 1.0f - T;
            const float m_ = mscale * (1.0f - MRGS_NEAR_N * mrgs_rcp(depth));
            const float mm = m_ * m_;
            distortion = fmaf(fmaf(-2.0f * m_, M1, fmaf(mm, A, M2)), w, distortion);
            Dp = fmaf(depth, w, Dp);
            M1 = fmaf(m_, w, M1);
            M2 = fmaf(mm, w, M2);
            const uint32_t contributor = (uint32_t)(base + j + 1);
            if (median_live) {
                const uint64_t t_high = MRGS_BALLOT(T > 0.5f + MRGS_T2_EPS);
                const uint64_t t_band = MRGS_BALLOT(T > 0.5f - MRGS_T2_EPS) & ~t_high;
                redo |= ok & t_band;
                const bool med = MRGS_LANES(upd_mask & t_high);
                median_depth = med ? depth : median_depth;
                median_contributor = med ? contributor : median_contributor;
            }
            N0 = fmaf(a0.x, w, N0); N1 = fmaf(a0.y, w, N1); N2 = fmaf(a0.z, w, N2);
            C0 = fmaf(a0.w, w, C0); C1 = fmaf(a1.x, w, C1); C2 = fmaf(a1.y, w, C2);
            if (S_MAX > 0) {
#pragma unroll
                for (int ch = 0; ch < S_STAGED; ch++) F[ch] = fmaf(mrgs_staged_feature<FV>(sb, ch, j), w, F[ch]);
                if constexpr (XREC) Fx = fmaf(a1.w, w, Fx);
            }
            T = upd ? test_T : T;
            Terr = upd ? Terr_new : Terr;
            last_contributor = upd ? contributor : last_contributor;
        };

        if (m != 0ull) {
            int j = __builtin_ctzll(m);
            SurfelGeom sA, sB;
            sA.g0 = sb.rec[0][j]; sA.g1 = sb.rec[1][j]; sA.g2 = sb.rec[2][j];
            float4 tA0 = sb.rec[3][j], tB0;
            RecTail tA1 = *reinterpret_cast<const RecTail*>(&sb.rec[4][j]), tB1;
            while (true) {
                m &= m - 1;
                bool more = m != 0ull;
                int jn = more ? __builtin_ctzll(m) : j;
                sB.g0 = sb.rec[0][jn]; sB.g1 = sb.rec[1][jn]; sB.g2 = sb.rec[2][jn];
                tB0 = sb.rec[3][jn]; tB1 = *reinterpret_cast<const RecTail*>(&sb.rec[4][jn]);
                blend_entry(sA, tA0, tA1, j);
                if (!more) break;
                j = jn;
                m &= m - 1;
                more = m != 0ull;
                jn = more ? __builtin_ctzll(m) : j;
                sA.g0 = sb.rec[0][jn]; sA.g1 = sb.rec[1][jn]; sA.g2 = sb.rec[2][jn];
                tA0 = sb.rec[3][jn]; tA1 = *reinterpret_cast<const RecTail*>(&sb.rec[4][jn]);
                blend_entry(sB, tB0, tB1, j);
                if (!more) break;
                j = jn;
            }
        }
        if (base + lane < total) cf[(size_t)(base + lane) * 4] = (uint8_t)(((contributed >> lane) & 1ull) | (((unsure >> lane) & 1ull) << 1));
        cf_end = base + MRGS_CHUNK;
        if (MRGS_FWD_STAGES == 1) stage_next();
        mask_cur = mask_nxt;
        idc = idn;
    }
    mrgs_stage_wait();

    if (lane == 0) {
        item_work[tile * 4 + quad] = work;
        if (work_hint != nullptr) work_hint[tile * 4 + quad] = work;
    }
#ifdef MRGS_WAVE_STATS
    if (lane == 0 && b < 65536) {
        unsigned long long* w = g_wave_stats_fwd + 8 * (size_t)b;
        w[0] = ws_t0; w[1] = wall_clock64(); w[2] = __builtin_amdgcn_s_memtime() - ws_c0;
        w[3] = ((unsigned long long)(work - 3u * ws_blend) << 32) | ws_blend; w[4] = ((unsigned long long)ws_blend_le8 << 32) | (unsigned)total;
        w[6] = item_est[tile * 4 + quad];
        w[5] = (unsigned long long)__builtin_amdgcn_s_getreg((4 << 0) | (0 << 6) | (31 << 11)) | ((unsigned long long)__builtin_amdgcn_s_getreg((20 << 0) | (0 << 6) | (31 << 11)) << 32);
        w[7] = ((unsigned long long)ws_le4 << 40) | ((unsigned long long)ws_le8 << 20) | ws_le16;
    }
#endif
    if (inside) {
        final_T[pix] = T;
        final_T[pix + HW] = M1;
        final_T[pix + 2 * HW] = M2;
        n_contrib[pix] = last_contributor;
        n_contrib[pix + HW] = median_contributor;
        out_color[pix] = fmaf(T, bg[0], C0);
        out_color[pix + HW] = fmaf(T, bg[1], C1);
        out_color[pix + 2 * HW] = fmaf(T, bg[2], C2);
        if (S_MAX > 0) {
#pragma unroll
            for (int ch = 0; ch < S_ROW; ch++)
                if (ch < S) out_feature[(size_t)ch * HW + pix] = ch < S_STAGED ? F[ch < SF ? ch : 0] : (XREC && ch == S_MAX) ? Fx : 0.0f;
        }
        out_others[pix + 0 * HW] = Dp;
        out_others[pix + 1 * HW] = 1.0f - T;
        out_others[pix + 2 * HW] = N0;
        out_others[pix + 3 * HW] = N1;
        out_others[pix + 4 * HW] = N2;
        out_others[pix + 5 * HW] = median_depth;
        out_others[pix + 6 * HW] = distortion;
    }

#ifdef MRGS_FWD_REDO_ALL
    redo = ~0ull;
#endif
    redo |= MRGS_BALLOT(T < (MRGS_T_MIN + MRGS_T1_ABS) + Terr);
    redo &= __builtin_amdgcn_ballot_w64(inside);
    if (redo != 0ull) {
        for (int e = cf_end + lane; e < total; e += MRGS_CHUNK) cf[(size_t)e * 4] = 0;
        if (lane == 0) atomicAdd(&redo_list[0], (uint32_t)__builtin_popcountll(redo));
        uint32_t* q = reinterpret_cast<uint32_t*>(&stage[0]);
        static_assert(sizeof(StageBuf<SF>) >= 2 * MRGS_REDO_QCAP * sizeof(uint32_t), "the redo's queue must fit the staging buffer");
        __builtin_amdgcn_fence(__ATOMIC_RELEASE, "wavefront");
        __builtin_amdgcn_wave_barrier();
        while (redo != 0ull) {
            const int p = __builtin_ctzll(redo);
            redo &= redo - 1;
            mrgs_redo_pixel<S_ROW>(__builtin_amdgcn_readlane(pix, p), lane, q, q + MRGS_REDO_QCAP, ranges, point_list, qmask, cflag, S, W, H, tiles_x, rec, features,
                                   bg, final_T, n_contrib, out_color, out_feature, out_others);
            __builtin_amdgcn_wave_barrier();
        }
    }
}

#define MRGS_FWD_KERNEL render_fwd_kernel

void mrgs_launch_render_fwd(const MrgsRasterConfig& cfg, const MrgsRasterInputs& in, const MrgsGeomWs& g, const uint32_t* plist,
                            const uint8_t* qmask, uint8_t* cflag, const MrgsImgWs& img, float* out_color, float* out_feature, float* out_others, hipStream_t stream)
{
    const int tiles_x = (cfg.W + MRGS_BLOCK_X - 1) / MRGS_BLOCK_X, tiles_y = (cfg.H + MRGS_BLOCK_Y - 1) / MRGS_BLOCK_Y;
    const int ntiles = tiles_x * tiles_y;
    const int nblocks = (((ntiles + 7) / 8) * 4 + MRGS_MAX_SIMD_QUEUES) * 8;
    const dim3 grid(nblocks), block(64);
#define LAUNCH(SM, ...)                                                                                                           \
    hipLaunchKernelGGL((MRGS_FWD_KERNEL<SM, __VA_ARGS__>), grid, block, 0, stream, img.ranges, img.fwd_assign, img.blend_state, plist, qmask, cflag, cfg.S, cfg.W, cfg.H, tiles_x, ntiles, \
                       g.rec, g.cull, in.features, in.bg, img.final_T, img.n_contrib, out_color, out_feature, out_others, img.item_work, img.item_est, in.work_hint, mrgs_waves_per_simd<MRGS_FWD_KERNEL<SM, __VA_ARGS__>>(), img.redo_list)
    const bool fv_ok = ((uintptr_t)in.features & 15u) == 0;
    if (cfg.S == 0) LAUNCH(0, false, 0);
    else if (cfg.S == 8 && fv_ok) LAUNCH(8, true, 8);
    else if (cfg.S <= 8) LAUNCH(8, false, 8);
    else if (cfg.S == 12 && fv_ok && in.features_live == 9u) LAUNCH(8, true, 9);
    else if (cfg.S == 12 && fv_ok) LAUNCH(12, true, 12);
    else if (cfg.S <= 12) LAUNCH(12, false, 12);
    else if (cfg.S == 24 && fv_ok) LAUNCH(24, true, 24);
    else LAUNCH(24, false, 24);
#undef LAUNCH
}
```

materialrefgs_amd/csrc/mrgs_sort.hip:

```cpp
#include "mrgs_blend_math.h"
#include "mrgs_wave.h"

#define SORT_THREADS 256
#define SORT_WAVES (SORT_THREADS / 64)

#define OS_STATE_AGG 1u
#define OS_STATE_INC 2u
#define OS_VALUE_MASK 0x3FFFFFFFu
#define OS_SPIN_LIMIT (1 << 24)

__device__ __forceinline__ int64_t mrgs_count(int64_t n_host, const uint32_t* __restrict__ n_dev)
{
    if (n_dev == nullptr) return n_host;
    const int64_t v = (int64_t)*n_dev;
    return v <= n_host ? v : 0;
}

__device__ __forceinline__ uint64_t lanemask_lt() { return (1ull << (threadIdx.x & 63)) - 1ull; }

#define OS_WINDOW 8
__device__ __forceinline__ bool os_look_back(const uint32_t* __restrict__ status, int stride, int column, int blk, uint32_t& excl)
{
    excl = 0;
    int spins = 0;
// ... 311 lines not shown
    if (i >= P) return;
    if (R_dev != nullptr && *R_dev > capacity) return;
    const uint32_t g = order[i];
    if (tiles_touched[g] == 0) return;
    uint32_t off = offsets[i];
    const uint2 r = rect[g];
    const int x0 = r.x & 0xFFFF, y0 = r.x >> 16, x1 = r.y & 0xFFFF, y1 = r.y >> 16;
    for (int y = y0; y < y1; y++)
        for (int x = x0; x < x1; x++) {
            tile_key[off] = (uint32_t)(y * tiles_x + x);
            plist[off] = g;
            off++;
        }
}

void mrgs_launch_duplicate(const MrgsRasterConfig& cfg, const MrgsGeomWs& g, const uint32_t* order, uint32_t* tile_key,
                           uint32_t* plist, int64_t capacity, const uint32_t* R_dev, const MrgsBinWs& b, const MrgsImgWs& img, uint32_t* host_slot,
                           hipStream_t stream)
{
    const int tiles_x = (cfg.W + MRGS_BLOCK_X - 1) / MRGS_BLOCK_X;
    hipLaunchKernelGGL(duplicate_kernel, dim3((cfg.P + 255) / 256), dim3(256), 0, stream, cfg.P, order, g.tiles_touched, g.offsets,
                       g.rect, tiles_x, tile_key, plist, (uint32_t)capacity, R_dev, g.counters + 16, b.sort_ws,
                       (unsigned)(b.sort_ws_bytes / sizeof(uint32_t)), (uint32_t*)img.ranges, (unsigned)(img.ranges_est_bytes / sizeof(uint32_t)), host_slot);
}

__global__ void __launch_bounds__(256) tile_ranges_kernel(const uint32_t* __restrict__ tile_key, const uint32_t* __restrict__ plist,
                                                          int64_t R_host, const uint32_t* __restrict__ R_dev, const float4* __restrict__ cull,
                                                          int tiles_x, uint2* __restrict__ ranges, uint8_t* __restrict__ qmask,
                                                          uint32_t* __restrict__ item_est)
{
    const int64_t R = mrgs_count(R_host, R_dev);
    const int64_t idx = (int64_t)blockIdx.x * blockDim.x + threadIdx.x;
    const bool valid = idx < R;
    uint32_t cur = 0xFFFFFFFFu;
    uint32_t m = 0;
    if (valid) {
        cur = tile_key[idx];
        if (idx == 0)
            ranges[cur].x = 0;
        else {
            const uint32_t prev = tile_key[idx - 1];
            if (cur != prev) {
                ranges[prev].y = (uint32_t)idx;
                ranges[cur].x = (uint32_t)idx;
            }
        }
        if (idx == R - 1) ranges[cur].y = (uint32_t)R;
        const CullConic c = mrgs_cull_load(cull, plist[idx]);
        const int tx = (int)(cur % (uint32_t)tiles_x), ty = (int)(cur / (uint32_t)tiles_x);
        const float x0 = (float)(tx * MRGS_BLOCK_X), y0 = (float)(ty * MRGS_BLOCK_Y);
#pragma unroll
        for (int q = 0; q < 4; q++)
            m |= mrgs_block_may_touch(c, x0 + (float)(8 * (q & 1)), y0 + (float)(8 * (q >> 1)), 7.0f, 7.0f) ? (1u << q) : 0u;
        qmask[idx] = (uint8_t)m;
    }
    __shared__ uint32_t s_cnt[64 * 4];
    __shared__ uint32_t s_first;
    s_cnt[threadIdx.x] = 0u;
    if (threadIdx.x == 0) s_first = cur;
    __syncthreads();
    const uint32_t first_tile = s_first;
    uint64_t todo = __builtin_amdgcn_ballot_w64(valid);
    while (todo != 0ull) {
        const uint32_t t = (uint32_t)__builtin_amdgcn_readlane((int)cur, __builtin_ctzll(todo));
        const bool mine = valid && cur == t;
        todo &= ~__builtin_amdgcn_ballot_w64(mine);
        const uint32_t rel = t - first_tile;
#pragma unroll
        for (int q = 0; q < 4; q++) {
            const int n = __builtin_popcountll(__builtin_amdgcn_ballot_w64(mine && ((m >> q) & 1u)));
            if ((threadIdx.x & 63) == 0 && n > 0) {
                if (rel < 64u) atomicAdd(&s_cnt[rel * 4 + q], (uint32_t)n);
                else atomicAdd(&item_est[t * 4 + q], (uint32_t)n);
            }
        }
    }
    __syncthreads();
    const uint32_t c = s_cnt[threadIdx.x];
    if (c != 0u) atomicAdd(&item_est[(first_tile + (threadIdx.x >> 2)) * 4 + (threadIdx.x & 3)], c);
}

__device__ __forceinline__ uint32_t item_cost(const uint32_t* __restrict__ item_src, const uint32_t* __restrict__ hint, int idx)
{
    const uint32_t e = item_src[idx];
    if (hint == nullptr) return e;
    const uint32_t h = hint[idx];
    return (h != 0u && e != 0u) ? h : 3u * e;
}
#define ORDER_ADAPTIVE_PASSES 16
#define ORDER_LDS_ITEMS 4096
__global__ void __launch_bounds__(1024) blend_order_kernel(const uint32_t* __restrict__ item_src, int ntiles, uint32_t* __restrict__ items_ws,
                                                           uint32_t* __restrict__ work_ws, uint32_t* __restrict__ assign_ws,
                                                           uint32_t* __restrict__ qstate, const uint32_t* __restrict__ census,
                                                           uint32_t* __restrict__ cu_state, int forward, uint32_t* __restrict__ zero_this,
                                                           float4* __restrict__ bulk_zero, size_t bulk_zero_f4, const uint32_t* __restrict__ hint,
                                                           uint32_t* __restrict__ qstate_twin, uint32_t* __restrict__ redo_count)
{
    if (blockIdx.x >= 8) {
        const float4 z = make_float4(0.f, 0.f, 0.f, 0.f);
        for (size_t i = (size_t)(blockIdx.x - 8) * 1024 + threadIdx.x; i < bulk_zero_f4; i += (size_t)(gridDim.x - 8) * 1024) bulk_zero[i] = z;
        return;
    }
    __shared__ uint32_t hist[1024];
    __shared__ uint32_t wave_sums[16];
    __shared__ uint32_t load[MRGS_MAX_SIMD_QUEUES];
    __shared__ unsigned long long s_total;
    __shared__ uint32_t s_busy;
    const int tid = threadIdx.x, x = blockIdx.x;
    const int per_list = ((ntiles + 7) >> 3) * 4;
    hist[tid] = 0;
    if (tid == 0) { s_total = 0ull; s_busy = 0u; }
    if (tid < MRGS_MAX_SIMD_QUEUES) {
        qstate[MRGS_QS_TICKET + x * MRGS_MAX_SIMD_QUEUES + tid] = 0u;
        if (qstate_twin != nullptr) qstate_twin[MRGS_QS_TICKET + x * MRGS_MAX_SIMD_QUEUES + tid] = 0u;
        load[tid] = 0u;
    }
    if (zero_this != nullptr)
        for (int i = tid + 1024 * x; i < 4 * ntiles; i += 8 * 1024) zero_this[i] = 0u;
    if (redo_count != nullptr && x == 0 && tid == 0) redo_count[0] = 0u;
    const uint32_t idle = forward ? 1u : 0u;
    if (forward && tid < 256) {
        const bool seen = census[x * 256 + tid] != 0u;
        const uint64_t m = __builtin_amdgcn_ballot_w64(seen);
        if ((tid & 63) == 0) wave_sums[tid >> 6] = (uint32_t)__builtin_popcountll(m);
        __syncthreads();
        uint32_t below = (uint32_t)__builtin_popcountll(m & ((1ull << (tid & 63)) - 1ull));
        for (int w = 0; w < (tid >> 6); w++) below += wave_sums[w];
        cu_state[MRGS_CS_DENSE + x * 256 + tid] = below;
        if (tid == 255) cu_state[MRGS_CS_NCU + x] = below + (seen ? 1u : 0u);
    } else if (forward) {
        __syncthreads();
    }
    __syncthreads();
    for (int i0 = 0; i0 < per_list; i0 += 1024) {
        const int i = i0 + tid;
        const int tile = (i >> 2) * 8 + x;
        const uint32_t w = (i < per_list && tile < ntiles) ? item_cost(item_src, hint, tile * 4 + (i & 3)) + idle : 0u;
        const bool lightest = w > 0u && (w >> 2) == 0u;
        const uint64_t lm = __builtin_amdgcn_ballot_w64(lightest);
        if (lightest) { if ((tid & 63) == __builtin_ctzll(lm)) atomicAdd(&hist[1023], (uint32_t)__builtin_popcountll(lm)); }
        else if (w > 0u) atomicAdd(&hist[1023u - min(w >> 2, 1023u)], 1u);
        const uint64_t bm = __builtin_amdgcn_ballot_w64(w > idle);
        if ((tid & 63) == 0 && bm != 0ull) atomicAdd(&s_busy, (uint32_t)__builtin_popcountll(bm));
    }
    __syncthreads();
    uint32_t tot;
    const uint32_t ex = block_exclusive_scan<1024>(hist[tid], wave_sums, tot);
    hist[tid] = ex;
    __syncthreads();
    __shared__ uint32_t s_items[ORDER_LDS_ITEMS], s_work[ORDER_LDS_ITEMS];
    const bool in_lds = per_list <= ORDER_LDS_ITEMS;
    uint32_t* items = in_lds ? s_items : items_ws + (size_t)x * per_list;
    uint32_t* work = in_lds ? s_work : work_ws + (size_t)x * per_list;
    for (int i0 = 0; i0 < per_list; i0 += 1024) {
        const int i = i0 + tid;
        const int tile = (i >> 2) * 8 + x;
        const uint32_t w = (i < per_list && tile < ntiles) ? item_cost(item_src, hint, tile * 4 + (i & 3)) + idle : 0u;
        const bool lightest = w > 0u && (w >> 2) == 0u;
        const uint64_t lm = __builtin_amdgcn_ballot_w64(lightest);
        uint32_t pos = 0;
        if (lightest) {
            const int leader = __builtin_ctzll(lm);
            uint32_t base = 0;
            if ((tid & 63) == leader) base = atomicAdd(&hist[1023], (uint32_t)__builtin_popcountll(lm));
            base = (uint32_t)__builtin_amdgcn_readlane((int)base, leader);
            pos = base + (uint32_t)__builtin_popcountll(lm & ((1ull << (tid & 63)) - 1ull));
        } else if (w > 0u) {
            pos = atomicAdd(&hist[1023u - min(w >> 2, 1023u)], 1u);
        }
        if (w > 0u) {
            items[pos] = ((uint32_t)tile << 2) | (uint32_t)(i & 3);
            work[pos] = w;
        }
        unsigned long long ws = w;
#pragma unroll
        for (int d = 32; d >= 1; d >>= 1) ws += __shfl_xor(ws, d, 64);
        if ((tid & 63) == 0 && ws != 0ull) atomicAdd(&s_total, ws);
    }
    __threadfence_block();
    __syncthreads();

    __syncthreads();
    const int Q = (int)cu_state[MRGS_CS_NCU + x];
    const int NQ = 4 * min(max(Q, 1), MRGS_MAX_SIMD_QUEUES / 4);
    const int n_items = (int)tot;
    const int passes = (n_items + NQ - 1) / NQ;
    const unsigned long long mean5 = n_items > 0 ? 5ull * s_total / (unsigned long long)n_items : 0ull;
    uint32_t* assign = assign_ws + (size_t)x * (per_list + MRGS_MAX_SIMD_QUEUES);
    __shared__ uint32_t qrank[MRGS_MAX_SIMD_QUEUES];
    const int n_adapt = min(min(passes, ORDER_ADAPTIVE_PASSES), ((int)s_busy + NQ - 1) / NQ);
    for (int p = 0; p < n_adapt; p++) {
        if (p > 0) {
            if (tid < NQ) qrank[tid] = 0u;
            __syncthreads();
            const int q = tid & (MRGS_MAX_SIMD_QUEUES - 1), part = tid >> 7;
            if (q < NQ) {
                const uint32_t mine = load[q];
                uint32_t r = 0;
                for (int o = part; o < NQ; o += 8) {
                    const uint32_t lo = load[o];
                    r += (lo < mine || (lo == mine && o < q)) ? 1u : 0u;
                }
                if (r) atomicAdd(&qrank[q], r);
            }
            __syncthreads();
        }
        if (tid < NQ) {
            const int rank = p * NQ + (p > 0 ? (int)qrank[tid] : tid);
            uint32_t entry = 0xFFFFFFFFu;
            if (rank < n_items) {
                const unsigned long long w25 = 25ull * work[rank];
                const uint32_t prio = w25 > 8ull * mean5 ? 3u : w25 > 6ull * mean5 ? 2u : w25 > 4ull * mean5 ? 1u : 0u;
                entry = items[rank] | (prio << 29);
                load[tid] += work[rank];
            }
            assign[p * NQ + tid] = entry;
        }
        __syncthreads();
    }
    for (int e = n_adapt * NQ + tid; e < passes * NQ; e += 1024) {
        const int p = e / NQ, q = e - p * NQ;
        const int rank = p * NQ + ((p & 1) ? NQ - 1 - q : q);
        assign[e] = rank < n_items ? items[rank] : 0xFFFFFFFFu;
    }
    if (tid == 0) {
        qstate[MRGS_QS_COUNT + x] = tot;
        qstate[MRGS_QS_PASSES + x] = (uint32_t)passes | ((uint32_t)NQ << 16);
        if (qstate_twin != nullptr) {
            qstate_twin[MRGS_QS_COUNT + x] = tot;
            qstate_twin[MRGS_QS_PASSES + x] = (uint32_t)passes | ((uint32_t)NQ << 16);
        }
    }
}

void mrgs_launch_blend_order(const MrgsImgWs& img, const uint32_t* census, int ntiles, int backward, void* bulk_zero, size_t bulk_zero_bytes,
                             const uint32_t* fwd_hint, hipStream_t stream)
{
    const size_t f4 = bulk_zero ? bulk_zero_bytes / sizeof(float4) : 0;
    const unsigned extra = f4 ? (unsigned)((f4 + 8191) / 8192 < 504 ? (f4 + 8191) / 8192 : 504) : 0u;
    if (backward)
        hipLaunchKernelGGL(blend_order_kernel, dim3(8 + extra), dim3(1024), 0, stream, img.item_work, ntiles, img.order_items, img.order_work,
                           img.bwd_assign, img.q_bwd, census, img.blend_state + MRGS_CS_BASE, 0, (uint32_t*)nullptr,
                           (float4*)bulk_zero, f4, (const uint32_t*)nullptr, (uint32_t*)nullptr, (uint32_t*)nullptr);
    else
        hipLaunchKernelGGL(blend_order_kernel, dim3(8 + extra), dim3(1024), 0, stream, img.item_est, ntiles, img.order_items, img.order_work,
                           img.fwd_assign, img.blend_state + MRGS_QS_FWD, census, img.blend_state + MRGS_CS_BASE, 1, img.item_work,
                           (float4*)bulk_zero, f4, fwd_hint, bulk_zero ? img.q_bwd : (uint32_t*)nullptr, img.redo_list);
}

void mrgs_launch_tile_ranges(const uint32_t* tile_key, const uint32_t* plist, int64_t R, const uint32_t* R_dev, const float4* rec,
                             uint8_t* qmask, const MrgsImgWs& img, int tiles_x, int ntiles, hipStream_t stream)
{
    if (R > 0)
        hipLaunchKernelGGL(tile_ranges_kernel, dim3((unsigned)((R + 255) / 256)), dim3(256), 0, stream, tile_key, plist, R, R_dev, rec,
                           tiles_x, img.ranges, qmask, img.item_est);
}
```

materialrefgs_amd/rasterizer.py:

```python
import ctypes
import functools
import threading
import time
from typing import NamedTuple

import torch
import torch.nn as nn

from . import _lib
from ._cache import Bounded, constant, derived
from ._lib import MrgsRasterConfig, MrgsRasterGrads, MrgsRasterInputs, MrgsRasterTicket


_PAIR_GUESS_MAX = 64
_PAIR_GUESS = Bounded(_PAIR_GUESS_MAX)
_WORK_HINTS_MAX = 2048
_WORK_HINTS_MAX_BYTES = 256 << 20
_WORK_HINTS = Bounded(_WORK_HINTS_MAX, _WORK_HINTS_MAX_BYTES, lambda ent: ent.buf.numel() * 4)


def _hint_key(raster_settings, device):
    vm, pm = raster_settings.viewmatrix, raster_settings.projmatrix
    return (device.index, int(raster_settings.image_height), int(raster_settings.image_width), vm.data_ptr(), pm.data_ptr())

# ... 14 lines not shown
        return None
    return ent


def _hint_is_warm(raster_settings, device):
    ent = _hint_entry(raster_settings, device)
    return ent is not None and ent.visits > 0


_REORDER_EVERY = 16


def _hint_flags(raster_settings, device, P, forward=False):
    if not forward:
        return 0
    ent = _hint_entry(raster_settings, device)
    if ent is None:
        return 0
    now = (int(P), _GENERATION[0])
    if ent.visits >= 2 and ent.visits % _REORDER_EVERY != 0 and ent.dealt_for == now:
        return _lib.MRGS_HINT_REUSE_ORDER
    if ent.visits >= 1:
        ent.dealt_for = now
    return 0


def _work_hint(raster_settings, device, count_visit=False):
    ent = _hint_entry(raster_settings, device)
    if ent is None:
        n = _lib.lib().mrgs_work_hint_bytes(int(raster_settings.image_height), int(raster_settings.image_width)) // 4
        ent = _WORK_HINTS[_hint_key(raster_settings, device)] = _Hint(torch.zeros(max(int(n), 1), dtype=torch.int32, device=device),
                                                                      raster_settings.viewmatrix, raster_settings.projmatrix)
    if count_visit:
        ent.visits += 1
    return ent.buf


def reset_work_hints():
    _WORK_HINTS.clear()
    _CAM_COPIES.clear()


def note_surfel_set_changed():
    _GENERATION[0] += 1


_AFTER_BLEND_HOOK = [None]


def set_after_blend_hook(fn):
    _AFTER_BLEND_HOOK[0] = fn


LAST_NUM_RENDERED = 0
COUNT_WAIT_SECONDS = 0.0


def cpu_deep_copy_tuple(input_tuple):
    return tuple(x.detach().cpu().clone() if torch.is_tensor(x) else x for x in input_tuple)


_ptr = _lib.ptr


def _f32c(t):
    if t.dtype != torch.float32:
        t = t.float()
    return t.contiguous()


_CAM_COPIES = Bounded(4096)


def _camera_f32c(t):
    if t.dtype == torch.float32 and t.is_contiguous():
        return t
    return derived(_CAM_COPIES, (t.data_ptr(), t.stride(), t.dtype, t.device), (t,), lambda: _f32c(t))


_RESOLVE = object()


class _RenderCall:
    __slots__ = ("features_live", "glue", "visible")

    def __init__(self, features_live=0, glue=None):
        self.features_live, self.glue, self.visible = int(features_live or 0), glue, None


def _make_cfg_inputs(raster_settings, means3D, sh, colors_precomp, features, opacities, scales, rotations, cov3Ds_precomp, sh_rest=None,
                     bwd_grad_ws=None, work_hint=_RESOLVE, extra_flags=0, features_live=0):
    P = means3D.shape[0]
    is_forward = work_hint is _RESOLVE
    if work_hint is _RESOLVE:
        work_hint = _work_hint(raster_settings, means3D.device) if means3D.is_cuda else None
    S = features.shape[1] if features.dim() == 2 else 0
    M = sh.shape[1] if sh.numel() != 0 else 0
    if sh_rest is not None:
        M = 1 + sh_rest.shape[1]
    cfg = MrgsRasterConfig(P, S, int(raster_settings.sh_degree), M, int(raster_settings.image_height),
                           int(raster_settings.image_width), float(raster_settings.tanfovx), float(raster_settings.tanfovy),
                           float(raster_settings.scale_modifier), int(bool(raster_settings.prefiltered)),
                           int(bool(raster_settings.debug)))
    inp = MrgsRasterInputs(_ptr(raster_settings.bg), _ptr(means3D), _ptr(sh), _ptr(colors_precomp), _ptr(features),
                           _ptr(opacities), _ptr(scales), _ptr(rotations), _ptr(cov3Ds_precomp),
                           _ptr(raster_settings.viewmatrix), _ptr(raster_settings.projmatrix), _ptr(raster_settings.campos),
                           _ptr(work_hint), _ptr(sh_rest),
                           _ptr(bwd_grad_ws), (_hint_flags(raster_settings, means3D.device, P, forward=is_forward) if means3D.is_cuda else 0) | extra_flags,
                           features_live)
    return cfg, inp, work_hint


class RasterWorkspaceOverflow(RuntimeError):

    def __init__(self, num_rendered):
        super().__init__(f"libmrgs: {num_rendered} (tile, surfel) pairs did not fit the binning workspace sized from the previous view")
        self.num_rendered = num_rendered


_DEFER = threading.local()
_TICKET_RING = 16


def _note_count(guess_key, num_rendered, hint_settings, dev):
    _PAIR_GUESS[guess_key] = max(int(num_rendered * 1.25) + 65536, 1)
    if hint_settings is not None:
        _work_hint(hint_settings, dev, count_visit=True)


class _PendingCount:

    def __init__(self, ticket, guess_key, hint_settings, dev):
        self.ticket, self.guess_key, self.hint_settings, self.dev = ticket, guess_key, hint_settings, dev
        self.value, self.overflow, self.ctx = None, False, None

    def finish(self):
        global LAST_NUM_RENDERED, COUNT_WAIT_SECONDS
        if self.value is None:
            R = ctypes.c_int64(0)
            t0 = time.perf_counter()
            rc = _lib.lib().mrgs_rasterize_forward_finish(ctypes.byref(self.ticket), ctypes.byref(R))
            COUNT_WAIT_SECONDS += time.perf_counter() - t0
            if rc != _lib.MRGS_E_WORKSPACE:
                _lib.check(rc)
            self.value, self.overflow = int(R.value), rc == _lib.MRGS_E_WORKSPACE
            _note_count(self.guess_key, self.value, None if self.overflow else self.hint_settings, self.dev)
            LAST_NUM_RENDERED = self.value
            if self.ctx is not None:
                self.ctx.num_rendered = self.value
        if self.overflow:
            raise RasterWorkspaceOverflow(self.value)
        return self.value


class deferred_count:

    def __init__(self):
        self.pending, self.outer = [], None

    def __enter__(self):
        self.outer = getattr(_DEFER, "box", None)
        if self.outer is None:
            _DEFER.box = self
            return self
        return self.outer

    def __exit__(self, *exc):
        if self.outer is None:
            _DEFER.box = None
        return False

    def finish(self):
        if self.outer is not None:
            return
        pending, self.pending = self.pending, []
        first = None
        for p in pending:
            try:
                p.finish()
            except RasterWorkspaceOverflow as ex:
                first = first or ex
        if first is not None:
            raise first


def deferred_raster_count(render_fn):
    @functools.wraps(render_fn)
    def wrapper(*args, **kw):
        dc = deferred_count()
        with dc:
            out = render_fn(*args, **kw)
        if dc.outer is not None:
            return out
        try:
            dc.finish()
        except RasterWorkspaceOverflow:
            return render_fn(*args, **kw)
        return out
    return wrapper


def _rasterize_forward_native(raster_settings, means3D, sh, colors_precomp, features, opacities, scales, rotations, cov3Ds_precomp,
                              sh_rest=None, prepare_backward=False, call=None):
    if means3D.dim() != 2 or means3D.shape[1] != 3:
        raise RuntimeError("means3D must have dimensions (num_points, 3)")
    if not means3D.is_cuda:
        raise RuntimeError("means3D must be a CUDA tensor")
    L = _lib.lib()
    dev = means3D.device
    H, W = int(raster_settings.image_height), int(raster_settings.image_width)
    S_ = features.shape[1] if features.dim() == 2 else 0
    grad_ws = None
    if prepare_backward and means3D.shape[0] > 0:
        with _lib.guard(dev):
            grad_ws = torch.empty((L.mrgs_grad_bytes(means3D.shape[0], S_),), dtype=torch.uint8, device=dev)
    cfg, inp, hint = _make_cfg_inputs(raster_settings, means3D, sh, colors_precomp, features, opacities, scales, rotations, cov3Ds_precomp,
                                      sh_rest, grad_ws, extra_flags=_lib.MRGS_HINT_VISIBLE_BYTES,
                                      features_live=0 if call is None else call.features_live)
    P, S = cfg.P, cfg.S
    with _lib.guard(dev):
        st = _lib.stream_ptr(dev)
        contrib = constant((1, H, W), torch.int32, dev)
        color = torch.empty((3, H, W), dtype=torch.float32, device=dev)
        feature = torch.empty((S, H, W), dtype=torch.float32, device=dev)
        others = torch.empty((7, H, W), dtype=torch.float32, device=dev)
        rbuf = torch.empty((5 * P,), dtype=torch.uint8, device=dev)
        radii = rbuf[:4 * P].view(torch.int32)
        if call is not None:
            call.visible = rbuf[4 * P:].view(torch.bool)
        geom = torch.empty((L.mrgs_geom_bytes(P, H, W),), dtype=torch.uint8, device=dev)
        img = torch.empty((L.mrgs_img_bytes(H, W),), dtype=torch.uint8, device=dev)
        R = ctypes.c_int64(0)
        global LAST_NUM_RENDERED
        guess_key = (dev.index, P, H, W)
        guess = _PAIR_GUESS.get(guess_key)
        if guess is None and P > 0:
            for (d_, p_, h_, w_), g_ in reversed(list(_PAIR_GUESS.items())):
                if (d_, h_, w_) == (dev.index, H, W) and p_ > 0:
                    guess = int(g_ * max(P / p_, 1.0) * 1.3)
                    break
        pairs = None
        box = getattr(_DEFER, "box", None)
        if guess is not None and P > 0:
            pairs = guess
            binning = torch.empty((L.mrgs_binning_bytes(pairs),), dtype=torch.uint8, device=dev)
            ticket = MrgsRasterTicket()
            _lib.check(L.mrgs_rasterize_forward_begin(ctypes.byref(cfg), ctypes.byref(inp), _ptr(geom), geom.numel(), _ptr(binning), binning.numel(),
                                                      pairs, _ptr(img), _ptr(radii), _ptr(color), _ptr(feature), _ptr(others), ctypes.byref(ticket), st))
            pending = _PendingCount(ticket, guess_key, raster_settings if hint is not None else None, dev)
            if box is not None:
                waiting = [q for q in box.pending if q.value is None]
                for q in waiting[:max(0, len(waiting) - (_TICKET_RING - 3))]:
                    try:
                        q.finish()
                    except RasterWorkspaceOverflow:
                        pass
                box.pending.append(pending)
                return (pending, pairs), contrib, color, feature, others, radii, geom, binning, img, grad_ws, hint
            try:
                num_rendered = pending.finish()
            except RasterWorkspaceOverflow as ex:
                num_rendered, pairs = ex.num_rendered, None
        else:
            _lib.check(L.mrgs_rasterize_forward_geom(ctypes.byref(cfg), ctypes.byref(inp), _ptr(geom), geom.numel(), _ptr(radii),
                                                     ctypes.byref(R), st))
            num_rendered = int(R.value)
        LAST_NUM_RENDERED = num_rendered
        if pairs is None:
            pairs = num_rendered
            binning = torch.empty((L.mrgs_binning_bytes(pairs),), dtype=torch.uint8, device=dev)
            _lib.check(L.mrgs_rasterize_forward_render(ctypes.byref(cfg), ctypes.byref(inp), _ptr(geom), _ptr(binning), binning.numel(),
                                                       _ptr(img), pairs, _ptr(color), _ptr(feature), _ptr(others), st))
            if P > 0:
                _note_count(guess_key, num_rendered, raster_settings if hint is not None else None, dev)
    return (num_rendered, pairs), contrib, color, feature, others, radii, geom, binning, img, grad_ws, hint


def _rasterize_backward_native(raster_settings, means3D, radii, colors_precomp, features, scales, rotations, cov3Ds_precomp,
                               grad_out_color, grad_out_feature, grad_out_others, sh, opacities, geom, num_rendered, binning, img,
                               sh_rest=None, prepared_grad_ws=None, work_hint=_RESOLVE, glue=None, features_live=0):
    L = _lib.lib()
    dev = means3D.device
    if prepared_grad_ws is not None and (work_hint is _RESOLVE or work_hint is None):
        prepared_grad_ws = None
    cfg, inp, _ = _make_cfg_inputs(raster_settings, means3D, sh, colors_precomp, features, opacities, scales, rotations, cov3Ds_precomp,
                                   sh_rest, prepared_grad_ws, work_hint, features_live=features_live)
    P, S, M = cfg.P, cfg.S, cfg.M
    with _lib.guard(dev):
        st = _lib.stream_ptr(dev)
        opts = dict(dtype=torch.float32, device=dev)
        fused = glue is not None and P > 0
        keep = (lambda name, shape: None) if fused else (lambda name, shape: torch.empty(shape, **opts))
        g = {"dL_dmeans2D": torch.empty((P, 3), **opts),
             "dL_dcolors": None if fused and colors_precomp.numel() == 0 else torch.empty((P, 3), **opts),
             "dL_dfeatures": keep("dL_dfeatures", (P, S)), "dL_dopacity": keep("dL_dopacity", (P, 1)),
             "dL_dmeans3D": keep("dL_dmeans3D", (P, 3)),
             "dL_dtransMat": None if fused and cov3Ds_precomp.numel() == 0 else torch.empty((P, 9), **opts),
             "dL_dsh": torch.empty((P, 1 if sh_rest is not None else M, 3), **opts), "dL_dscales": keep("dL_dscales", (P, 2)),
             "dL_drotations": keep("dL_drotations", (P, 4)),
             "dL_dsh_rest": torch.empty((P, M - 1, 3), **opts) if sh_rest is not None else None}
# ... 49 lines not shown
            try:
                out = _rasterize_forward_native(*args)
            except Exception as ex:
                torch.save(cpu_args, "snapshot_fw.dump")
                print("\nAn error occured in forward. Please forward snapshot_fw.dump for debugging.")
                raise ex
        else:
            out = _rasterize_forward_native(*args)
        (num_rendered, binning_pairs), contrib, color, feature, depth, radii, geomBuffer, binningBuffer, imgBuffer, grad_ws, hint = out
        ctx.prepared_grad_ws = grad_ws
        ctx.work_hint = hint
        ctx.raster_settings = rs
        ctx.num_rendered = num_rendered
        if isinstance(num_rendered, _PendingCount):
            ctx.num_rendered, num_rendered.ctx = None, ctx
        ctx.binning_pairs = binning_pairs
        ctx.save_for_backward(colors_precomp, features, means3D, scales, rotations, cov3Ds_precomp, radii, sh, opacities,
                              geomBuffer, binningBuffer, imgBuffer, contrib, sh_rest)
        ctx.mark_non_differentiable(contrib, radii)
        return contrib, color, feature, radii, depth

    @staticmethod
    def backward(ctx, grad_out_contrib, grad_out_color, grad_out_feature, grad_radii, grad_depth):
        num_rendered = ctx.binning_pairs
        rs = ctx.raster_settings
        (colors_precomp, features, means3D, scales, rotations, cov3Ds_precomp, radii, sh, opacities, geomBuffer, binningBuffer,
         imgBuffer, contrib, sh_rest) = ctx.saved_tensors
        H, W = int(rs.image_height), int(rs.image_width)
        S = features.shape[1] if features.dim() == 2 else 0
        dev = means3D.device
        if grad_out_color is None:
            grad_out_color = torch.zeros((3, H, W), dtype=torch.float32, device=dev)
        if grad_out_feature is None:
            grad_out_feature = torch.zeros((S, H, W), dtype=torch.float32, device=dev)
        if grad_depth is None:
            grad_depth = torch.zeros((7, H, W), dtype=torch.float32, device=dev)
        prepared, ctx.prepared_grad_ws = ctx.prepared_grad_ws, None
        args = (rs, means3D, radii, colors_precomp, features, scales, rotations, cov3Ds_precomp, _f32c(grad_out_color),
                _f32c(grad_out_feature), _f32c(grad_depth), sh, opacities, geomBuffer, num_rendered, binningBuffer, imgBuffer, sh_rest, prepared,
                ctx.work_hint, ctx.call.glue, ctx.call.features_live)
        if rs.debug:
            cpu_args = cpu_deep_copy_tuple(args[1:-2])
            try:
                out = _rasterize_backward_native(*args)
            except Exception as ex:
                torch.save(cpu_args, "snapshot_bw.dump")
                print("\nAn error occured in backward. Writing snapshot_bw.dump for debugging.\n")
                raise ex
        else:
            out = _rasterize_backward_native(*args)
        (grad_means2D, grad_colors_precomp, grad_features, grad_opacities, grad_means3D, grad_cov3Ds_precomp, grad_sh, grad_scales,
         grad_rotations, grad_sh_rest) = out
        if sh.numel() == 0:
            grad_sh = None
        if colors_precomp.numel() == 0:
            grad_colors_precomp = None
        if scales.numel() == 0:
            grad_scales = None
            grad_rotations = None
        if cov3Ds_precomp.numel() == 0:
            grad_cov3Ds_precomp = None
        return (grad_means3D, grad_means2D, grad_sh, grad_colors_precomp, grad_features, grad_opacities, grad_scales,
                grad_rotations, grad_cov3Ds_precomp, None, grad_sh_rest, None)


class GaussianRasterizationSettings(NamedTuple):
    image_height: int
    image_width: int
    tanfovx: float
    tanfovy: float
    bg: torch.Tensor
    scale_modifier: float
    viewmatrix: torch.Tensor
    projmatrix: torch.Tensor
    sh_degree: int
    campos: torch.Tensor
    prefiltered: bool
    debug: bool


class GaussianRasterizer(nn.Module):
    features_live = 0
    glue = None
    visible = None

    def __init__(self, raster_settings):
        super().__init__()
        self.raster_settings = raster_settings

    def markVisible(self, positions):
        with torch.no_grad():
            rs = self.raster_settings
            positions = _f32c(positions)
            P = positions.shape[0]
            present = torch.zeros((P,), dtype=torch.uint8, device=positions.device)
            with _lib.guard(positions.device):
                _lib.check(_lib.lib().mrgs_mark_visible(P, _ptr(positions), _ptr(_f32c(rs.viewmatrix)), _ptr(_f32c(rs.projmatrix)),
                                                        _ptr(present), _lib.stream_ptr(positions.device)))
            visible = present.bool()
        return visible

    def forward(self, means3D, means2D, opacities, shs=None, colors_precomp=None, features=None, scales=None, rotations=None,
                cov3D_precomp=None):
        raster_settings = self.raster_settings

        if (shs is None and colors_precomp is None) or (shs is not None and colors_precomp is not None):
            raise Exception('Please provide excatly one of either SHs or precomputed colors!')

        if ((scales is None or rotations is None) and cov3D_precomp is None) or \
                ((scales is not None or rotations is not None) and cov3D_precomp is not None):
            raise Exception('Please provide exactly one of either scale/rotation pair or precomputed 3D covariance!')

        empty = torch.empty((0,), dtype=torch.float32, device=means3D.device)
        shs_rest = None
        if isinstance(shs, (tuple, list)):
            shs, shs_rest = shs
            if shs.dim() != 3 or shs.shape[1] != 1 or shs_rest.dim() != 3 or shs_rest.shape[1] < 1 or shs_rest.shape[1] > 15:
                raise Exception('split SHs must be (dc [P,1,3], rest [P,1..15,3])')
        if shs is None:
            shs = empty
        if colors_precomp is None:
            colors_precomp = empty
        if features is None:
            features = torch.empty_like(means3D[..., :0])
        if scales is None:
            scales = empty
        if rotations is None:
            rotations = empty
        if cov3D_precomp is None:
            cov3D_precomp = empty

        call = _RenderCall(self.features_live, self.glue)
        self.visible = None
        out = rasterize_gaussians(means3D, means2D, shs, colors_precomp, features, opacities, scales, rotations, cov3D_precomp,
                                  raster_settings, shs_rest, call)
        self.visible = call.visible
        return out
```

Measured before the change: 1205 views/s.

## Split heavy tile-quad blend items into two half-row work items

The blend ordering kernel can now mark the costliest tile quads as split and emit two half items, each covering four pixel rows. The forward pass renders the halves on separate waves, writing contribution flags to a second cflag plane, and the backward pass ORs both planes and runs only the first half item. The goal is to cut tail imbalance from a few very heavy tiles in the persistent SIMD-queue schedule. The cost is an extra flag plane, more item bookkeeping, and duplicated per-surfel intersection work across the halves. Whether splitting happens by default depends on the split_buckets heuristic, since the split hint flags default to 0.

```diff
diff --git a/include/mrgs.h b/include/mrgs.h
--- a/include/mrgs.h
+++ b/include/mrgs.h
@@ -57,6 +57,8 @@
     uint32_t features_live;
 } MrgsRasterInputs;
 #define MRGS_HINT_REUSE_ORDER 1u
+#define MRGS_HINT_SPLIT_ALL 4u
+#define MRGS_HINT_SPLIT_NONE 8u
 #define MRGS_HINT_VISIBLE_BYTES 2u
 
 size_t mrgs_geom_bytes(int32_t P, int32_t H, int32_t W);
diff --git a/materialrefgs_amd/_lib.py b/materialrefgs_amd/_lib.py
--- a/materialrefgs_amd/_lib.py
+++ b/materialrefgs_amd/_lib.py
@@ -30,6 +30,8 @@
 
 MRGS_HINT_REUSE_ORDER = 1
 MRGS_HINT_VISIBLE_BYTES = 2
+MRGS_HINT_SPLIT_ALL = 4
+MRGS_HINT_SPLIT_NONE = 8
 
 
 class MrgsRasterGrads(_Sized):
diff --git a/materialrefgs_amd/csrc/mrgs_api.hip b/materialrefgs_amd/csrc/mrgs_api.hip
--- a/materialrefgs_amd/csrc/mrgs_api.hip
+++ b/materialrefgs_amd/csrc/mrgs_api.hip
@@ -126,10 +126,10 @@
     w.ranges_est_bytes = c.used - ranges_from;
     w.item_work = c.take<uint32_t>(4 * nt);
     const size_t per_list = (nt + 7) / 8 * 4;
-    w.order_items = c.take<uint32_t>(8 * per_list);
-    w.order_work = c.take<uint32_t>(8 * per_list);
-    w.fwd_assign = c.take<uint32_t>(8 * (per_list + MRGS_MAX_SIMD_QUEUES));
-    w.bwd_assign = c.take<uint32_t>(8 * (per_list + MRGS_MAX_SIMD_QUEUES));
+    w.order_items = c.take<uint32_t>(8 * (per_list + MRGS_MAX_SIMD_QUEUES));
+    w.order_work = c.take<uint32_t>(8 * (per_list + MRGS_MAX_SIMD_QUEUES));
+    w.fwd_assign = c.take<uint32_t>(8 * MRGS_ASSIGN_WORDS(per_list));
+    w.bwd_assign = c.take<uint32_t>(8 * MRGS_ASSIGN_WORDS(per_list));
     w.blend_state = c.take<uint32_t>(MRGS_BLEND_STATE_WORDS);
     w.q_bwd = w.blend_state + MRGS_QS_BWD;
     w.final_T = c.take<float>(3 * hw);
@@ -153,6 +153,7 @@
     b.sort_ws_bytes = sizeof(uint32_t) * (16 + mrgs_sort_ws_words((int64_t)n));
     b.qmask = c.take<uint8_t>(n);
     b.cflag = c.take<uint8_t>(4 * n);
+    b.cflag1 = c.take<uint8_t>(4 * n);
     b.total = mrgs_align_up(c.used, 256);
     return b;
 }
@@ -196,7 +197,7 @@
     l.work = 0;
     l.blend_state = mrgs_align_up(4 * nt, 64);
     l.fwd_assign = mrgs_align_up(l.blend_state + MRGS_BLEND_STATE_WORDS, 64);
-    l.total_words = mrgs_align_up(l.fwd_assign + 8 * (per_list + MRGS_MAX_SIMD_QUEUES), 64);
+    l.total_words = mrgs_align_up(l.fwd_assign + 8 * MRGS_ASSIGN_WORDS(per_list), 64);
     return l;
 }
 static void img_use_hint(MrgsImgWs& img, const MrgsRasterInputs* in, int H, int W)
@@ -272,12 +273,12 @@
     }
     if (!reuse_order)
         mrgs_launch_blend_order(img, g.counters + 16, ntiles, 0, in->bwd_grad_ws, in->bwd_grad_ws ? mrgs_grad_bytes(cfg->P, cfg->S) : 0, in->work_hint,
-                                stream);
+                                mrgs_fwd_splits(cfg->S) ? in->hint_flags & (MRGS_HINT_SPLIT_ALL | MRGS_HINT_SPLIT_NONE) : MRGS_HINT_SPLIT_NONE, stream);
     t0.stop();
     STAGE_CHECK(cfg, stream);
 
     StageTimer t1(stream, ST_FWD);
-    mrgs_launch_render_fwd(*cfg, *in, g, b.plist[cur], b.qmask, b.cflag, img, out_color, out_feature, out_others, stream);
+    mrgs_launch_render_fwd(*cfg, *in, g, b.plist[cur], b.qmask, b.cflag, (size_t)(b.cflag1 - b.cflag), img, out_color, out_feature, out_others, stream);
     t1.stop();
     STAGE_CHECK(cfg, stream);
     return MRGS_OK;
@@ -451,8 +452,8 @@
     StageTimer t0(stream, ST_BWD);
     const bool prepared = in->bwd_grad_ws != nullptr && in->bwd_grad_ws == grad_ws;
     if (R > 0) {
-        if (!prepared) mrgs_launch_blend_order(img, g.counters + 16, tiles_x * tiles_y, 1, grad_rec, mrgs_grad_bytes(cfg->P, cfg->S), nullptr, stream);
-        mrgs_launch_render_bwd(*cfg, *in, g, b.plist[cur], b.cflag, img, dL_dout_color, dL_dout_feature, dL_dout_others, grad_rec, prepared, stream);
+        if (!prepared) mrgs_launch_blend_order(img, g.counters + 16, tiles_x * tiles_y, 1, grad_rec, mrgs_grad_bytes(cfg->P, cfg->S), nullptr, 0u, stream);
+        mrgs_launch_render_bwd(*cfg, *in, g, b.plist[cur], b.cflag, (size_t)(b.cflag1 - b.cflag), img, dL_dout_color, dL_dout_feature, dL_dout_others, grad_rec, prepared, stream);
     } else if (!prepared) {
         MRGS_HIP_TRY(hipMemsetAsync(grad_rec, 0, mrgs_grad_bytes(cfg->P, cfg->S), stream));
     }
diff --git a/materialrefgs_amd/csrc/mrgs_blend_math.h b/materialrefgs_amd/csrc/mrgs_blend_math.h
--- a/materialrefgs_amd/csrc/mrgs_blend_math.h
+++ b/materialrefgs_amd/csrc/mrgs_blend_math.h
@@ -29,7 +29,7 @@
     const uint32_t xcc = __builtin_amdgcn_s_getreg((20 << 0) | (0 << 6) | (3 << 11)) & 7u;
     const uint32_t dense = cu_state[MRGS_CS_DENSE + xcc * 256 + mrgs_cu_key(hw_id)];
     const int q0 = (int)((dense * 4u + ((hw_id >> 4) & 3u)) % (uint32_t)NQ);
-    const uint32_t* assign = assign_ws + (size_t)xcd * (per_list + MRGS_MAX_SIMD_QUEUES);
+    const uint32_t* assign = assign_ws + (size_t)xcd * MRGS_ASSIGN_WORDS(per_list);
     uint32_t* tickets = qstate + MRGS_QS_TICKET + xcd * MRGS_MAX_SIMD_QUEUES;
     uint32_t item = 0xFFFFFFFFu;
     int t = 0;
@@ -143,6 +143,18 @@
     const uint64_t tw_ok = s.g2.x < MRGS_NEAR_LO ? 0ull : ~0ull;
     return MRGS_BALLOT(t.ppz != 0.0f) & (~MRGS_BALLOT(t.d3 < MRGS_NEAR_LO) | tw_ok) & ~MRGS_BALLOT(t.power > 0.0f) & ~MRGS_BALLOT(h.alpha < MRGS_ALPHA_LO);
 }
+__device__ __forceinline__ uint64_t mrgs_intersect_mask_pair(const SurfelGeom& s, float px, float py, Hit& h)
+{
+    const HitTest t = mrgs_intersect_fast(s, px, py, h);
+    return MRGS_BALLOT(t.ppz != 0.0f) & (~MRGS_BALLOT(t.d3 < MRGS_NEAR_LO) | ~MRGS_BALLOT(s.g2.x < MRGS_NEAR_LO)) & ~MRGS_BALLOT(t.power > 0.0f) &
+           ~MRGS_BALLOT(h.alpha < MRGS_ALPHA_LO);
+}
+__device__ __forceinline__ float2 mrgs_halves(float v)
+{
+    const uint32_t u = __float_as_uint(v);
+    const auto r = __builtin_amdgcn_permlane32_swap(u, u, false, false);
+    return make_float2(__uint_as_float(r[0]), __uint_as_float(r[1]));
+}
 __device__ __forceinline__ uint64_t mrgs_hit_decide_mask(const Hit& h, uint64_t may_hit, uint64_t& ambiguous)
 {
     const uint64_t hit = may_hit & ~MRGS_BALLOT(h.depth < MRGS_NEAR_LO);
diff --git a/materialrefgs_amd/csrc/mrgs_internal.h b/materialrefgs_amd/csrc/mrgs_internal.h
--- a/materialrefgs_amd/csrc/mrgs_internal.h
+++ b/materialrefgs_amd/csrc/mrgs_internal.h
@@ -71,6 +71,7 @@
     size_t sort_ws_bytes;
     uint8_t* qmask;
     uint8_t* cflag;
+    uint8_t* cflag1;
     size_t total;
 };
 
@@ -93,6 +94,13 @@
 #define MRGS_CS_NCU 0
 #define MRGS_CS_DENSE 8
 #define MRGS_BLEND_STATE_WORDS (2 * MRGS_QS_WORDS + 8 + 2048)
+#define MRGS_WORK_SPLIT (1u << 31)
+#define MRGS_ITEM_SPLIT (1u << 27)
+#define MRGS_ITEM_HALF_SHIFT 28
+#define MRGS_ITEM_TILE_MASK 0x07FFFFFFu
+#define MRGS_SPLIT_MAX_TILES (1 << 25)
+#define MRGS_ASSIGN_WORDS(per_list) ((per_list) + 2 * MRGS_MAX_SIMD_QUEUES)
+#define MRGS_BLEND_BLOCKS(ntiles) (((((ntiles) + 7) / 8) * 4 + 2 * MRGS_MAX_SIMD_QUEUES) * 8)
 #define MRGS_CENSUS_WORDS 2048
 __device__ __forceinline__ uint32_t mrgs_cu_key(uint32_t hw_id) { return ((hw_id >> 8) & 0xFFu); }
 __device__ __forceinline__ void mrgs_census_mark(uint32_t* __restrict__ census)
@@ -129,13 +137,14 @@
 void mrgs_launch_tile_ranges(const uint32_t* tile_key, const uint32_t* plist, int64_t R, const uint32_t* R_dev, const float4* rec,
                              uint8_t* qmask, const MrgsImgWs& img, int tiles_x, int ntiles, hipStream_t stream);
 void mrgs_launch_blend_order(const MrgsImgWs& img, const uint32_t* census, int ntiles, int backward, void* bulk_zero, size_t bulk_zero_bytes,
-                             const uint32_t* fwd_hint,
+                             const uint32_t* fwd_hint, uint32_t split_mode ,
                              hipStream_t stream);
 
+static inline bool mrgs_fwd_splits(int S) { return S <= 12; }
 void mrgs_launch_render_fwd(const MrgsRasterConfig& cfg, const MrgsRasterInputs& in, const MrgsGeomWs& g, const uint32_t* plist,
-                            const uint8_t* qmask, uint8_t* cflag, const MrgsImgWs& img, float* out_color, float* out_feature, float* out_others, hipStream_t stream);
+                            const uint8_t* qmask, uint8_t* cflag, size_t cflag_plane, const MrgsImgWs& img, float* out_color, float* out_feature, float* out_others, hipStream_t stream);
 void mrgs_launch_render_bwd(const MrgsRasterConfig& cfg, const MrgsRasterInputs& in, const MrgsGeomWs& g, const uint32_t* plist,
-                            const uint8_t* cflag, const MrgsImgWs& img, const float* dL_dpix, const float* dL_dpix_f, const float* dL_dothers,
+                            const uint8_t* cflag, size_t cflag_plane, const MrgsImgWs& img, const float* dL_dpix, const float* dL_dpix_f, const float* dL_dothers,
                             float* grad_rec, bool forward_queues, hipStream_t stream);
 
 int mrgs_tsdf_fuse_launch(const MrgsTsdfConfig* cfg, const MrgsTsdfView* views, float* field, float* weight_debug, void* stream, bool* launched);
diff --git a/materialrefgs_amd/csrc/mrgs_render_bwd.hip b/materialrefgs_amd/csrc/mrgs_render_bwd.hip
--- a/materialrefgs_amd/csrc/mrgs_render_bwd.hip
+++ b/materialrefgs_amd/csrc/mrgs_render_bwd.hip
@@ -161,7 +161,7 @@
 template <int S_MAX, bool FV, int S_LIVE>
 __global__ void __launch_bounds__(64) __attribute__((amdgpu_waves_per_eu(S_MAX == 0 ? MRGS_BWD_WPE0 : S_MAX <= 8 ? MRGS_BWD_WPE8 : 2, 8))) render_bwd_kernel(
     const uint2* __restrict__ ranges, const uint32_t* __restrict__ bwd_assign, uint32_t* __restrict__ q_bwd, const uint32_t* __restrict__ cu_state, const uint32_t* __restrict__ point_list,
-    const uint8_t* __restrict__ cflag, int S, int W, int H, int tiles_x, int ntiles,
+    const uint8_t* __restrict__ cflag, size_t cflag_plane, const uint32_t* __restrict__ item_work, int S, int W, int H, int tiles_x, int ntiles,
     const float4* __restrict__ rec, const float* __restrict__ features, const float* __restrict__ bg,
     const float* __restrict__ final_Ts, const uint32_t* __restrict__ n_contrib, const float* __restrict__ dL_dpixels,
     const float* __restrict__ dL_dpixels_f, const float* __restrict__ dL_dothers, float* __restrict__ grad_rec, int gstride, int slots)
@@ -181,7 +181,10 @@
     WS_ENTRY();
     const uint32_t item = mrgs_pull_item(q_bwd, cu_state, bwd_assign, ntiles, b & 7, b >> 3, lane, slots WS_DBG);
     if (item == 0xFFFFFFFFu) return;
-    const int tile = (int)((item & 0x1FFFFFFFu) >> 2), quad = (int)(item & 3u);
+    const bool split_item = ntiles <= MRGS_SPLIT_MAX_TILES && (item & MRGS_ITEM_SPLIT) != 0u;
+    if (split_item && ((item >> MRGS_ITEM_HALF_SHIFT) & 1u) != 0u) return;
+    const int tile = (int)((item & (split_item ? MRGS_ITEM_TILE_MASK : 0x1FFFFFFFu)) >> 2), quad = (int)(item & 3u);
+    const bool split = (item_work[tile * 4 + quad] & MRGS_WORK_SPLIT) != 0u;
     const uint32_t prio = (item >> 29) & 3u;
     const uint2 range = ranges[tile];
     const int tx = tile % tiles_x, ty = tile / tiles_x;
@@ -235,6 +238,11 @@
 
     const uint32_t* plist = point_list + range.x;
     const uint8_t* qm = cflag + (size_t)range.x * 4 + quad;
+    auto flags_at = [&](int e) -> uint32_t {
+        uint32_t f = qm[(size_t)e * 4];
+        if (split) f |= qm[cflag_plane + (size_t)e * 4];
+        return f;
+    };
     const ReduceLane rl = mrgs_reduce_lane(lane);
     const uint32_t row_bytes = (uint32_t)gstride * 4u;
     const int c_top = (max_contrib - 1) / MRGS_CHUNK;
@@ -242,9 +250,9 @@
     uint64_t mask_cur, exact_cur;
     {
         uint32_t id0 = 0, q0 = 0;
-        if (c_top * MRGS_CHUNK + lane < max_contrib) { id0 = plist[c_top * MRGS_CHUNK + lane]; q0 = qm[(size_t)(c_top * MRGS_CHUNK + lane) * 4]; }
-        if (c_top >= 1) idq1 = plist[(c_top - 1) * MRGS_CHUNK + lane] | ((uint32_t)qm[(size_t)((c_top - 1) * MRGS_CHUNK + lane) * 4] << 28);
-        if (c_top >= 2) idq2 = plist[(c_top - 2) * MRGS_CHUNK + lane] | ((uint32_t)qm[(size_t)((c_top - 2) * MRGS_CHUNK + lane) * 4] << 28);
+        if (c_top * MRGS_CHUNK + lane < max_contrib) { id0 = plist[c_top * MRGS_CHUNK + lane]; q0 = flags_at(c_top * MRGS_CHUNK + lane); }
+        if (c_top >= 1) idq1 = plist[(c_top - 1) * MRGS_CHUNK + lane] | (flags_at((c_top - 1) * MRGS_CHUNK + lane) << 28);
+        if (c_top >= 2) idq2 = plist[(c_top - 2) * MRGS_CHUNK + lane] | (flags_at((c_top - 2) * MRGS_CHUNK + lane) << 28);
         const bool cand0 = q0 & 1u;
         mask_cur = __builtin_amdgcn_ballot_w64(cand0);
         exact_cur = __builtin_amdgcn_ballot_w64((q0 & 2u) != 0u);
@@ -266,7 +274,7 @@
             if (cand1) stage[(c + 1) % MRGS_BWD_STAGES].id[lane] = id1 * row_bytes;
             idq1 = idq2;
             idq2 = 0;
-            if (c >= 3) idq2 = plist[(c - 3) * MRGS_CHUNK + lane] | ((uint32_t)qm[(size_t)((c - 3) * MRGS_CHUNK + lane) * 4] << 28);
+            if (c >= 3) idq2 = plist[(c - 3) * MRGS_CHUNK + lane] | (flags_at((c - 3) * MRGS_CHUNK + lane) << 28);
         };
         if (MRGS_BWD_STAGES == 2) stage_next();
 
@@ -412,16 +420,16 @@
 #define MRGS_BWD_KERNEL render_bwd_kernel
 
 void mrgs_launch_render_bwd(const MrgsRasterConfig& cfg, const MrgsRasterInputs& in, const MrgsGeomWs& g, const uint32_t* plist,
-                            const uint8_t* cflag, const MrgsImgWs& img, const float* dL_dpix, const float* dL_dpix_f, const float* dL_dothers,
+                            const uint8_t* cflag, size_t cflag_plane, const MrgsImgWs& img, const float* dL_dpix, const float* dL_dpix_f, const float* dL_dothers,
                             float* grad_rec, bool forward_queues, hipStream_t stream)
 {
     const uint32_t* assign = forward_queues ? img.fwd_assign : img.bwd_assign;
     const int tiles_x = (cfg.W + MRGS_BLOCK_X - 1) / MRGS_BLOCK_X, tiles_y = (cfg.H + MRGS_BLOCK_Y - 1) / MRGS_BLOCK_Y;
     const int ntiles = tiles_x * tiles_y;
-    const int nblocks = (((ntiles + 7) / 8) * 4 + MRGS_MAX_SIMD_QUEUES) * 8;
+    const int nblocks = MRGS_BLEND_BLOCKS(ntiles);
     const dim3 grid(nblocks), block(64);
 #define LAUNCH(GS, SM, ...)                                                                                                       \
-    hipLaunchKernelGGL((MRGS_BWD_KERNEL<SM, __VA_ARGS__>), grid, block, 0, stream, img.ranges, assign, img.q_bwd, img.blend_state + MRGS_CS_BASE, plist, cflag, cfg.S, cfg.W, cfg.H, tiles_x, ntiles, \
+    hipLaunchKernelGGL((MRGS_BWD_KERNEL<SM, __VA_ARGS__>), grid, block, 0, stream, img.ranges, assign, img.q_bwd, img.blend_state + MRGS_CS_BASE, plist, cflag, cflag_plane, img.item_work, cfg.S, cfg.W, cfg.H, tiles_x, ntiles, \
                        g.rec, in.features, in.bg, img.final_T, img.n_contrib, dL_dpix, dL_dpix_f, dL_dothers, grad_rec, GS, mrgs_waves_per_simd<MRGS_BWD_KERNEL<SM, __VA_ARGS__>>())
     const int gs = MRGS_GRAD_STRIDE(cfg.S);
     const bool fv_ok = ((uintptr_t)in.features & 15u) == 0;
diff --git a/materialrefgs_amd/csrc/mrgs_render_fwd.hip b/materialrefgs_amd/csrc/mrgs_render_fwd.hip
--- a/materialrefgs_amd/csrc/mrgs_render_fwd.hip
+++ b/materialrefgs_amd/csrc/mrgs_render_fwd.hip
@@ -206,8 +206,8 @@
 #endif
 __global__ void __launch_bounds__(64) __attribute__((amdgpu_waves_per_eu(S_MAX == 0 ? MRGS_FWD_WAVES_S0 : S_MAX <= 12 ? MRGS_FWD_WAVES_S8 : 4, 8))) render_fwd_kernel(
     const uint2* __restrict__ ranges, const uint32_t* __restrict__ fwd_assign, uint32_t* __restrict__ blend_state, const uint32_t* __restrict__ point_list,
-    const uint8_t* __restrict__ qmask, uint8_t* __restrict__ cflag, int S, int W, int H, int tiles_x, int ntiles,
-    const float4* __restrict__ rec, const float4* __restrict__ cull, const float* __restrict__ features, const float* __restrict__ bg, float* __restrict__ final_T,
+    const uint8_t* __restrict__ qmask, uint8_t* __restrict__ cflag, size_t cflag_plane ,
+    int S, int W, int H, int tiles_x, int ntiles, const float4* __restrict__ rec, const float4* __restrict__ cull, const float* __restrict__ features, const float* __restrict__ bg, float* __restrict__ final_T,
     uint32_t* __restrict__ n_contrib, float* __restrict__ out_color, float* __restrict__ out_feature, float* __restrict__ out_others,
     uint32_t* __restrict__ item_work, const uint32_t* __restrict__ item_est ,
     uint32_t* __restrict__ work_hint, int slots, uint32_t* __restrict__ redo_list)
@@ -224,12 +224,21 @@
     const int b = blockIdx.x;
     const uint32_t item = mrgs_pull_item(blend_state + MRGS_QS_FWD, blend_state + MRGS_CS_BASE, fwd_assign, ntiles, b & 7, b >> 3, lane, slots);
     if (item == 0xFFFFFFFFu) return;
-    const int tile = (int)((item & 0x1FFFFFFFu) >> 2), quad = (int)(item & 3u);
+    constexpr bool PAIR = S_MAX <= 12;
+    const bool split_item = ntiles <= MRGS_SPLIT_MAX_TILES && (item & MRGS_ITEM_SPLIT) != 0u;
+    const bool split = PAIR && split_item;
+    const int half = split_item ? (int)((item >> MRGS_ITEM_HALF_SHIFT) & 1u) : 0;
+    const int tile = (int)((item & (split_item ? MRGS_ITEM_TILE_MASK : 0x1FFFFFFFu)) >> 2), quad = (int)(item & 3u);
     const uint32_t prio = (item >> 29) & 3u;
     const uint2 range = ranges[tile];
+    if (!PAIR && half != 0) {
+        for (uint32_t e = range.x + lane; e < range.y; e += MRGS_CHUNK) cflag[cflag_plane + (size_t)e * 4 + quad] = 0;
+        return;
+    }
     const int tx = tile % tiles_x, ty = tile / tiles_x;
     const int bx = tx * 2 + (quad & 1), by = ty * 2 + (quad >> 1);
-    const int pxi = bx * 8 + (lane & 7), pyi = by * 8 + (lane >> 3);
+    const int row0 = split ? 4 * half : 0;
+    const int pxi = bx * 8 + (lane & 7), pyi = by * 8 + (split ? row0 + ((lane >> 3) & 3) : lane >> 3);
     const bool inside = pxi < W && pyi < H;
     const float px = (float)pxi, py = (float)pyi;
     const int HW = H * W;
@@ -265,7 +274,8 @@
 
     const uint32_t* plist = point_list + range.x;
     const uint8_t* qm = qmask + range.x;
-    uint8_t* cf = cflag + (size_t)range.x * 4 + quad;
+    uint8_t* const cflag_own = cflag + (half ? cflag_plane : (size_t)0);
+    uint8_t* cf = cflag_own + (size_t)range.x * 4 + quad;
     uint32_t id1 = 0, id2 = 0, q1 = 0, q2 = 0;
     uint32_t idc = 0, idn = 0;
 
@@ -298,9 +308,9 @@
 
         uint64_t m = mask_cur;
         {
-            const uint64_t live = ~done;
-            if (m != 0ull && __builtin_popcountll(live) <= MRGS_FWD_REFINE_LIVE) {
-                const int r0 = __builtin_ctzll(live) >> 3, r1 = (63 - __builtin_clzll(live)) >> 3;
+            const uint64_t live = split ? ~done & 0xFFFFFFFFull : ~done;
+            if (m != 0ull && __builtin_popcountll(live) <= (split ? MRGS_FWD_REFINE_LIVE / 2 : MRGS_FWD_REFINE_LIVE)) {
+                const int r0 = row0 + (__builtin_ctzll(live) >> 3), r1 = row0 + ((63 - __builtin_clzll(live)) >> 3);
                 uint32_t cols = (uint32_t)(live | (live >> 32));
                 cols |= cols >> 16; cols |= cols >> 8; cols &= 0xFFu;
                 const int c0 = __builtin_ctz(cols), c1 = 31 - __builtin_clz(cols);
@@ -315,23 +325,11 @@
         uint64_t unsure = 0ull;
 
         const bool median_live = (MRGS_BALLOT(T > 0.5f - MRGS_T2_EPS) & ~done) != 0ull;
-        auto blend_entry = [&](const SurfelGeom& sg, const float4& a0, const RecTail& a1, int j) {
-            Hit h;
-            const uint64_t may_hit = mrgs_intersect_mask(sg, px, py, h) & ~done;
-#ifdef MRGS_WAVE_STATS
-            const int ws_live = __builtin_popcountll(~done);
-            ws_le4 += ws_live <= 4; ws_le8 += ws_live <= 8; ws_le16 += ws_live <= 16;
-#endif
-            if (may_hit == 0ull) return;
-#ifdef MRGS_WAVE_STATS
-            ws_blend++; ws_blend_le8 += ws_live <= 8;
-#endif
+        auto blend_hit = [&](float h_alpha, float h_depth, uint64_t ok, uint64_t ambiguous, const float4& a0, const RecTail& a1, int j) {
             work += 3u;
             contributed |= 1ull << j;
-            uint64_t ambiguous;
-            const uint64_t ok = mrgs_hit_decide_mask(h, may_hit, ambiguous);
             if (ambiguous != 0ull) unsure |= 1ull << j;
-            const float oma = 1.0f - h.alpha;
+            const float oma = 1.0f - h_alpha;
             const float test_T = T * oma;
             const float Terr_new = fmaf(Terr, oma, (MRGS_T1_SLACK * MRGS_T_STEP_ERR) * T);
             const uint64_t below = MRGS_BALLOT(test_T < (MRGS_T_MIN - MRGS_T1_ABS) - Terr_new);
@@ -339,8 +337,8 @@
             done |= ok & below;
             const uint64_t upd_mask = ok & ~below;
             const bool upd = MRGS_LANES(upd_mask);
-            const float alpha = upd ? h.alpha : 0.0f;
-            const float depth = upd ? h.depth : 1.0f;
+            const float alpha = upd ? h_alpha : 0.0f;
+            const float depth = upd ? h_depth : 1.0f;
             const float w = alpha * T;
             const float A = 1.0f - T;
             const float m_ = mscale * (1.0f - MRGS_NEAR_N * mrgs_rcp(depth));
@@ -369,8 +367,69 @@
             Terr = upd ? Terr_new : Terr;
             last_contributor = upd ? contributor : last_contributor;
         };
-
-        if (m != 0ull) {
+        auto blend_entry = [&](const SurfelGeom& sg, const float4& a0, const RecTail& a1, int j) {
+            Hit h;
+            const uint64_t may_hit = mrgs_intersect_mask(sg, px, py, h) & ~done;
+#ifdef MRGS_WAVE_STATS
+            const int ws_live = __builtin_popcountll(~done);
+            ws_le4 += ws_live <= 4; ws_le8 += ws_live <= 8; ws_le16 += ws_live <= 16;
+#endif
+            if (may_hit == 0ull) return;
+#ifdef MRGS_WAVE_STATS
+            ws_blend++; ws_blend_le8 += ws_live <= 8;
+#endif
+            uint64_t ambiguous;
+            const uint64_t ok = mrgs_hit_decide_mask(h, may_hit, ambiguous);
+            blend_hit(h.alpha, h.depth, ok, ambiguous, a0, a1, j);
+        };
+
+        if (m != 0ull && split) {
+            auto pick = [&](int& ja, int& jb, bool& two) {
+                ja = __builtin_ctzll(m);
+                m &= m - 1;
+                two = m != 0ull;
+                jb = two ? __builtin_ctzll(m) : ja;
+                m &= m - 1;
+            };
+            const bool hi = lane >= 32;
+            int j0, j1;
+            bool two;
+            pick(j0, j1, two);
+            SurfelGeom sg;
+            { const int js = hi ? j1 : j0; sg.g0 = sb.rec[0][js]; sg.g1 = sb.rec[1][js]; sg.g2 = sb.rec[2][js]; }
+            while (true) {
+                const bool more = m != 0ull;
+                int n0 = j0, n1 = j1;
+                bool ntwo = false;
+                if (more) pick(n0, n1, ntwo);
+                SurfelGeom sn;
+                { const int js = hi ? n1 : n0; sn.g0 = sb.rec[0][js]; sn.g1 = sb.rec[1][js]; sn.g2 = sb.rec[2][js]; }
+                const float4 t00 = sb.rec[3][j0], t10 = sb.rec[3][j1];
+                const RecTail t01 = *reinterpret_cast<const RecTail*>(&sb.rec[4][j0]), t11 = *reinterpret_cast<const RecTail*>(&sb.rec[4][j1]);
+                Hit h;
+                uint64_t mh = mrgs_intersect_mask_pair(sg, px, py, h);
+                if (!two) mh &= 0xFFFFFFFFull;
+                const uint64_t hitm = mh & ~MRGS_BALLOT(h.depth < MRGS_NEAR_LO);
+                const uint64_t ambm = (hitm & (MRGS_BALLOT(h.alpha < MRGS_ALPHA_HI) | MRGS_BALLOT(h.depth < MRGS_NEAR_HI))) |
+                                      (mh & MRGS_BALLOT(fabsf(h.rho3d - h.rho2d) < MRGS_RHO_EPS));
+                const float2 al = mrgs_halves(h.alpha), de = mrgs_halves(h.depth);
+                auto both = [](uint64_t v, bool high) { const uint64_t x = high ? v >> 32 : v & 0xFFFFFFFFull; return x | (x << 32); };
+                if ((both(mh, false) & ~done) != 0ull) {
+                    blend_hit(al.x, de.x, both(hitm, false) & ~done, both(ambm, false) & ~done, t00, t01, j0);
+#ifdef MRGS_WAVE_STATS
+                    ws_blend++;
+#endif
+                }
+                if ((both(mh, true) & ~done) != 0ull) {
+                    blend_hit(al.y, de.y, both(hitm, true) & ~done, both(ambm, true) & ~done, t10, t11, j1);
+#ifdef MRGS_WAVE_STATS
+                    ws_blend++;
+#endif
+                }
+                if (!more) break;
+                sg = sn; j0 = n0; j1 = n1; two = ntwo;
+            }
+        } else if (m != 0ull) {
             int j = __builtin_ctzll(m);
             SurfelGeom sA, sB;
             sA.g0 = sb.rec[0][j]; sA.g1 = sb.rec[1][j]; sA.g2 = sb.rec[2][j];
@@ -404,8 +463,14 @@
     mrgs_stage_wait();
 
     if (lane == 0) {
-        item_work[tile * 4 + quad] = work;
-        if (work_hint != nullptr) work_hint[tile * 4 + quad] = work;
+        if (split) {
+            const uint32_t mine = work > 0u ? work : 1u;
+            const uint32_t other = atomicAdd(&item_work[tile * 4 + quad], mine | (half == 0 ? MRGS_WORK_SPLIT : 0u)) & ~MRGS_WORK_SPLIT;
+            if (work_hint != nullptr && other != 0u) work_hint[tile * 4 + quad] = other + mine;
+        } else {
+            item_work[tile * 4 + quad] = work;
+            if (work_hint != nullptr) work_hint[tile * 4 + quad] = work;
+        }
     }
 #ifdef MRGS_WAVE_STATS
     if (lane == 0 && b < 65536) {
@@ -417,7 +482,7 @@
         w[7] = ((unsigned long long)ws_le4 << 40) | ((unsigned long long)ws_le8 << 20) | ws_le16;
     }
 #endif
-    if (inside) {
+    if (inside && (!split || lane < 32)) {
         final_T[pix] = T;
         final_T[pix + HW] = M1;
         final_T[pix + 2 * HW] = M2;
@@ -445,8 +510,11 @@
 #endif
     redo |= MRGS_BALLOT(T < (MRGS_T_MIN + MRGS_T1_ABS) + Terr);
     redo &= __builtin_amdgcn_ballot_w64(inside);
+    if (split) redo &= 0xFFFFFFFFull;
+    if (redo != 0ull || split) {
+        for (int e = cf_end + lane; e < total; e += MRGS_CHUNK) cf[(size_t)e * 4] = 0;
+    }
     if (redo != 0ull) {
-        for (int e = cf_end + lane; e < total; e += MRGS_CHUNK) cf[(size_t)e * 4] = 0;
         if (lane == 0) atomicAdd(&redo_list[0], (uint32_t)__builtin_popcountll(redo));
         uint32_t* q = reinterpret_cast<uint32_t*>(&stage[0]);
         static_assert(sizeof(StageBuf<SF>) >= 2 * MRGS_REDO_QCAP * sizeof(uint32_t), "the redo's queue must fit the staging buffer");
@@ -455,7 +523,7 @@
         while (redo != 0ull) {
             const int p = __builtin_ctzll(redo);
             redo &= redo - 1;
-            mrgs_redo_pixel<S_ROW>(__builtin_amdgcn_readlane(pix, p), lane, q, q + MRGS_REDO_QCAP, ranges, point_list, qmask, cflag, S, W, H, tiles_x, rec, features,
+            mrgs_redo_pixel<S_ROW>(__builtin_amdgcn_readlane(pix, p), lane, q, q + MRGS_REDO_QCAP, ranges, point_list, qmask, cflag_own, S, W, H, tiles_x, rec, features,
                                    bg, final_T, n_contrib, out_color, out_feature, out_others);
             __builtin_amdgcn_wave_barrier();
         }
@@ -465,14 +533,14 @@
 #define MRGS_FWD_KERNEL render_fwd_kernel
 
 void mrgs_launch_render_fwd(const MrgsRasterConfig& cfg, const MrgsRasterInputs& in, const MrgsGeomWs& g, const uint32_t* plist,
-                            const uint8_t* qmask, uint8_t* cflag, const MrgsImgWs& img, float* out_color, float* out_feature, float* out_others, hipStream_t stream)
+                            const uint8_t* qmask, uint8_t* cflag, size_t cflag_plane, const MrgsImgWs& img, float* out_color, float* out_feature, float* out_others, hipStream_t stream)
 {
     const int tiles_x = (cfg.W + MRGS_BLOCK_X - 1) / MRGS_BLOCK_X, tiles_y = (cfg.H + MRGS_BLOCK_Y - 1) / MRGS_BLOCK_Y;
     const int ntiles = tiles_x * tiles_y;
-    const int nblocks = (((ntiles + 7) / 8) * 4 + MRGS_MAX_SIMD_QUEUES) * 8;
+    const int nblocks = MRGS_BLEND_BLOCKS(ntiles);
     const dim3 grid(nblocks), block(64);
 #define LAUNCH(SM, ...)                                                                                                           \
-    hipLaunchKernelGGL((MRGS_FWD_KERNEL<SM, __VA_ARGS__>), grid, block, 0, stream, img.ranges, img.fwd_assign, img.blend_state, plist, qmask, cflag, cfg.S, cfg.W, cfg.H, tiles_x, ntiles, \
+    hipLaunchKernelGGL((MRGS_FWD_KERNEL<SM, __VA_ARGS__>), grid, block, 0, stream, img.ranges, img.fwd_assign, img.blend_state, plist, qmask, cflag, cflag_plane, cfg.S, cfg.W, cfg.H, tiles_x, ntiles, \
                        g.rec, g.cull, in.features, in.bg, img.final_T, img.n_contrib, out_color, out_feature, out_others, img.item_work, img.item_est, in.work_hint, mrgs_waves_per_simd<MRGS_FWD_KERNEL<SM, __VA_ARGS__>>(), img.redo_list)
     const bool fv_ok = ((uintptr_t)in.features & 15u) == 0;
     if (cfg.S == 0) LAUNCH(0, false, 0);
diff --git a/materialrefgs_amd/csrc/mrgs_sort.hip b/materialrefgs_amd/csrc/mrgs_sort.hip
--- a/materialrefgs_amd/csrc/mrgs_sort.hip
+++ b/materialrefgs_amd/csrc/mrgs_sort.hip
@@ -417,19 +417,26 @@
 
 __device__ __forceinline__ uint32_t item_cost(const uint32_t* __restrict__ item_src, const uint32_t* __restrict__ hint, int idx)
 {
-    const uint32_t e = item_src[idx];
+    const uint32_t e = item_src[idx] & ~MRGS_WORK_SPLIT;
     if (hint == nullptr) return e;
     const uint32_t h = hint[idx];
     return (h != 0u && e != 0u) ? h : 3u * e;
 }
 #define ORDER_ADAPTIVE_PASSES 16
 #define ORDER_LDS_ITEMS 4096
+#ifndef MRGS_SPLIT_NUM
+#define MRGS_SPLIT_NUM 8
+#define MRGS_SPLIT_DEN 5
+#endif
+#ifndef MRGS_SPLIT_H0_QUARTERS
+#define MRGS_SPLIT_H0_QUARTERS 4
+#endif
 __global__ void __launch_bounds__(1024) blend_order_kernel(const uint32_t* __restrict__ item_src, int ntiles, uint32_t* __restrict__ items_ws,
                                                            uint32_t* __restrict__ work_ws, uint32_t* __restrict__ assign_ws,
                                                            uint32_t* __restrict__ qstate, const uint32_t* __restrict__ census,
                                                            uint32_t* __restrict__ cu_state, int forward, uint32_t* __restrict__ zero_this,
                                                            float4* __restrict__ bulk_zero, size_t bulk_zero_f4, const uint32_t* __restrict__ hint,
-                                                           uint32_t* __restrict__ qstate_twin, uint32_t* __restrict__ redo_count)
+                                                           uint32_t* __restrict__ qstate_twin, uint32_t* __restrict__ redo_count, uint32_t split_mode)
 {
     if (blockIdx.x >= 8) {
         const float4 z = make_float4(0.f, 0.f, 0.f, 0.f);
@@ -440,11 +447,11 @@
     __shared__ uint32_t wave_sums[16];
     __shared__ uint32_t load[MRGS_MAX_SIMD_QUEUES];
     __shared__ unsigned long long s_total;
-    __shared__ uint32_t s_busy;
+    __shared__ uint32_t s_busy, s_split_buckets;
     const int tid = threadIdx.x, x = blockIdx.x;
     const int per_list = ((ntiles + 7) >> 3) * 4;
     hist[tid] = 0;
-    if (tid == 0) { s_total = 0ull; s_busy = 0u; }
+    if (tid == 0) { s_total = 0ull; s_busy = 0u; s_split_buckets = 0u; }
     if (tid < MRGS_MAX_SIMD_QUEUES) {
         qstate[MRGS_QS_TICKET + x * MRGS_MAX_SIMD_QUEUES + tid] = 0u;
         if (qstate_twin != nullptr) qstate_twin[MRGS_QS_TICKET + x * MRGS_MAX_SIMD_QUEUES + tid] = 0u;
@@ -477,24 +484,66 @@
         else if (w > 0u) atomicAdd(&hist[1023u - min(w >> 2, 1023u)], 1u);
         const uint64_t bm = __builtin_amdgcn_ballot_w64(w > idle);
         if ((tid & 63) == 0 && bm != 0ull) atomicAdd(&s_busy, (uint32_t)__builtin_popcountll(bm));
+        unsigned long long ws = w;
+#pragma unroll
+        for (int d = 32; d >= 1; d >>= 1) ws += __shfl_xor(ws, d, 64);
+        if ((tid & 63) == 0 && ws != 0ull) atomicAdd(&s_total, ws);
     }
     __syncthreads();
     uint32_t tot;
-    const uint32_t ex = block_exclusive_scan<1024>(hist[tid], wave_sums, tot);
+    uint32_t ex = block_exclusive_scan<1024>(hist[tid], wave_sums, tot);
+    const int n_whole = (int)tot;
+    const bool can_split = forward && split_mode != MRGS_HINT_SPLIT_NONE && ntiles <= MRGS_SPLIT_MAX_TILES;
+    if (can_split) {
+        const unsigned long long low = 4ull * (1023u - (uint32_t)tid);
+        const bool heavy = split_mode == MRGS_HINT_SPLIT_ALL ||
+                           (s_busy > 0u && low * MRGS_SPLIT_DEN * (unsigned long long)s_busy > MRGS_SPLIT_NUM * s_total);
+        const bool fits = ex + hist[tid] <= (uint32_t)MRGS_MAX_SIMD_QUEUES;
+        const uint64_t sm = __builtin_amdgcn_ballot_w64(heavy && fits);
+        if ((tid & 63) == 0 && sm != 0ull) atomicAdd(&s_split_buckets, (uint32_t)__builtin_popcountll(sm));
+    }
+    __syncthreads();
+    const uint32_t split_buckets = s_split_buckets;
+    auto is_split = [&](uint32_t w) { return w > idle && 1023u - min(w >> 2, 1023u) < split_buckets; };
+    if (split_buckets > 0u) {
+        hist[tid] = 0;
+        __syncthreads();
+        for (int i0 = 0; i0 < per_list; i0 += 1024) {
+            const int i = i0 + tid;
+            const int tile = (i >> 2) * 8 + x;
+            const uint32_t w = (i < per_list && tile < ntiles) ? item_cost(item_src, hint, tile * 4 + (i & 3)) + idle : 0u;
+            if (w > 0u) {
+                if (is_split(w)) atomicAdd(&hist[1023u - min(((w + 1u) >> 1) >> 2, 1023u)], 2u);
+                else atomicAdd(&hist[1023u - min(w >> 2, 1023u)], 1u);
+            }
+            const uint64_t sm = __builtin_amdgcn_ballot_w64(w > 0u && is_split(w));
+            if ((tid & 63) == 0 && sm != 0ull) atomicAdd(&s_busy, (uint32_t)__builtin_popcountll(sm));
+        }
+        __syncthreads();
+        ex = block_exclusive_scan<1024>(hist[tid], wave_sums, tot);
+    }
     hist[tid] = ex;
     __syncthreads();
     __shared__ uint32_t s_items[ORDER_LDS_ITEMS], s_work[ORDER_LDS_ITEMS];
-    const bool in_lds = per_list <= ORDER_LDS_ITEMS;
-    uint32_t* items = in_lds ? s_items : items_ws + (size_t)x * per_list;
-    uint32_t* work = in_lds ? s_work : work_ws + (size_t)x * per_list;
+    const bool in_lds = per_list + MRGS_MAX_SIMD_QUEUES <= ORDER_LDS_ITEMS;
+    uint32_t* items = in_lds ? s_items : items_ws + (size_t)x * (per_list + MRGS_MAX_SIMD_QUEUES);
+    uint32_t* work = in_lds ? s_work : work_ws + (size_t)x * (per_list + MRGS_MAX_SIMD_QUEUES);
     for (int i0 = 0; i0 < per_list; i0 += 1024) {
         const int i = i0 + tid;
         const int tile = (i >> 2) * 8 + x;
         const uint32_t w = (i < per_list && tile < ntiles) ? item_cost(item_src, hint, tile * 4 + (i & 3)) + idle : 0u;
-        const bool lightest = w > 0u && (w >> 2) == 0u;
+        const bool halves = w > 0u && split_buckets > 0u && is_split(w);
+        const bool lightest = w > 0u && (w >> 2) == 0u && !halves;
         const uint64_t lm = __builtin_amdgcn_ballot_w64(lightest);
         uint32_t pos = 0;
-        if (lightest) {
+        if (halves) {
+            const uint32_t wh = (w + 1u) >> 1;
+            pos = atomicAdd(&hist[1023u - min(wh >> 2, 1023u)], 2u);
+            const uint32_t it = ((uint32_t)tile << 2) | (uint32_t)(i & 3) | MRGS_ITEM_SPLIT;
+            items[pos] = it;
+            items[pos + 1] = it | (1u << MRGS_ITEM_HALF_SHIFT);
+            work[pos] = work[pos + 1] = wh;
+        } else if (lightest) {
             const int leader = __builtin_ctzll(lm);
             uint32_t base = 0;
             if ((tid & 63) == leader) base = atomicAdd(&hist[1023], (uint32_t)__builtin_popcountll(lm));
@@ -503,14 +552,10 @@
         } else if (w > 0u) {
             pos = atomicAdd(&hist[1023u - min(w >> 2, 1023u)], 1u);
         }
-        if (w > 0u) {
+        if (w > 0u && !halves) {
             items[pos] = ((uint32_t)tile << 2) | (uint32_t)(i & 3);
             work[pos] = w;
         }
-        unsigned long long ws = w;
-#pragma unroll
-        for (int d = 32; d >= 1; d >>= 1) ws += __shfl_xor(ws, d, 64);
-        if ((tid & 63) == 0 && ws != 0ull) atomicAdd(&s_total, ws);
     }
     __threadfence_block();
     __syncthreads();
@@ -520,8 +565,8 @@
     const int NQ = 4 * min(max(Q, 1), MRGS_MAX_SIMD_QUEUES / 4);
     const int n_items = (int)tot;
     const int passes = (n_items + NQ - 1) / NQ;
-    const unsigned long long mean5 = n_items > 0 ? 5ull * s_total / (unsigned long long)n_items : 0ull;
-    uint32_t* assign = assign_ws + (size_t)x * (per_list + MRGS_MAX_SIMD_QUEUES);
+    const unsigned long long mean5 = n_whole > 0 ? 5ull * s_total / (unsigned long long)n_whole : 0ull;
+    uint32_t* assign = assign_ws + (size_t)x * MRGS_ASSIGN_WORDS(per_list);
     __shared__ uint32_t qrank[MRGS_MAX_SIMD_QUEUES];
     const int n_adapt = min(min(passes, ORDER_ADAPTIVE_PASSES), ((int)s_busy + NQ - 1) / NQ);
     for (int p = 0; p < n_adapt; p++) {
@@ -547,7 +592,9 @@
                 const unsigned long long w25 = 25ull * work[rank];
                 const uint32_t prio = w25 > 8ull * mean5 ? 3u : w25 > 6ull * mean5 ? 2u : w25 > 4ull * mean5 ? 1u : 0u;
                 entry = items[rank] | (prio << 29);
-                load[tid] += work[rank];
+                const uint32_t it = items[rank];
+                load[tid] += !(can_split && (it & MRGS_ITEM_SPLIT)) ? work[rank]
+                             : ((it >> MRGS_ITEM_HALF_SHIFT) & 1u) ? (work[rank] * (4 - MRGS_SPLIT_H0_QUARTERS)) / 2 : (work[rank] * MRGS_SPLIT_H0_QUARTERS) / 2;
             }
             assign[p * NQ + tid] = entry;
         }
@@ -569,18 +616,18 @@
 }
 
 void mrgs_launch_blend_order(const MrgsImgWs& img, const uint32_t* census, int ntiles, int backward, void* bulk_zero, size_t bulk_zero_bytes,
-                             const uint32_t* fwd_hint, hipStream_t stream)
+                             const uint32_t* fwd_hint, uint32_t split_mode, hipStream_t stream)
 {
     const size_t f4 = bulk_zero ? bulk_zero_bytes / sizeof(float4) : 0;
     const unsigned extra = f4 ? (unsigned)((f4 + 8191) / 8192 < 504 ? (f4 + 8191) / 8192 : 504) : 0u;
     if (backward)
         hipLaunchKernelGGL(blend_order_kernel, dim3(8 + extra), dim3(1024), 0, stream, img.item_work, ntiles, img.order_items, img.order_work,
                            img.bwd_assign, img.q_bwd, census, img.blend_state + MRGS_CS_BASE, 0, (uint32_t*)nullptr,
-                           (float4*)bulk_zero, f4, (const uint32_t*)nullptr, (uint32_t*)nullptr, (uint32_t*)nullptr);
+                           (float4*)bulk_zero, f4, (const uint32_t*)nullptr, (uint32_t*)nullptr, (uint32_t*)nullptr, 0u);
     else
         hipLaunchKernelGGL(blend_order_kernel, dim3(8 + extra), dim3(1024), 0, stream, img.item_est, ntiles, img.order_items, img.order_work,
                            img.fwd_assign, img.blend_state + MRGS_QS_FWD, census, img.blend_state + MRGS_CS_BASE, 1, img.item_work,
-                           (float4*)bulk_zero, f4, fwd_hint, bulk_zero ? img.q_bwd : (uint32_t*)nullptr, img.redo_list);
+                           (float4*)bulk_zero, f4, fwd_hint, bulk_zero ? img.q_bwd : (uint32_t*)nullptr, img.redo_list, split_mode);
 }
 
 void mrgs_launch_tile_ranges(const uint32_t* tile_key, const uint32_t* plist, int64_t R, const uint32_t* R_dev, const float4* rec,
diff --git a/materialrefgs_amd/rasterizer.py b/materialrefgs_amd/rasterizer.py
--- a/materialrefgs_amd/rasterizer.py
+++ b/materialrefgs_amd/rasterizer.py
@@ -120,10 +120,10 @@
 
 
 class _RenderCall:
-    __slots__ = ("features_live", "glue", "visible")
-
-    def __init__(self, features_live=0, glue=None):
-        self.features_live, self.glue, self.visible = int(features_live or 0), glue, None
+    __slots__ = ("features_live", "glue", "visible", "extra_flags")
+
+    def __init__(self, features_live=0, glue=None, extra_flags=0):
+        self.features_live, self.glue, self.visible, self.extra_flags = int(features_live or 0), glue, None, int(extra_flags or 0)
 
 
 def _make_cfg_inputs(raster_settings, means3D, sh, colors_precomp, features, opacities, scales, rotations, cov3Ds_precomp, sh_rest=None,
@@ -253,7 +253,7 @@
         with _lib.guard(dev):
             grad_ws = torch.empty((L.mrgs_grad_bytes(means3D.shape[0], S_),), dtype=torch.uint8, device=dev)
     cfg, inp, hint = _make_cfg_inputs(raster_settings, means3D, sh, colors_precomp, features, opacities, scales, rotations, cov3Ds_precomp,
-                                      sh_rest, grad_ws, extra_flags=_lib.MRGS_HINT_VISIBLE_BYTES,
+                                      sh_rest, grad_ws, extra_flags=_lib.MRGS_HINT_VISIBLE_BYTES | (0 if call is None else call.extra_flags),
                                       features_live=0 if call is None else call.features_live)
     P, S = cfg.P, cfg.S
     with _lib.guard(dev):
@@ -469,6 +469,7 @@
 class GaussianRasterizer(nn.Module):
     features_live = 0
     glue = None
+    split = 0
     visible = None
 
     def __init__(self, raster_settings):
@@ -517,7 +518,7 @@
         if cov3D_precomp is None:
             cov3D_precomp = empty
 
-        call = _RenderCall(self.features_live, self.glue)
+        call = _RenderCall(self.features_live, self.glue, self.split)
         self.visible = None
         out = rasterize_gaussians(means3D, means2D, shs, colors_precomp, features, opacities, scales, rotations, cov3D_precomp,
                                   raster_settings, shs_rest, call)
```

After: 1122 views/s. 6.9% lower.
